# ZYM-PKU/UDiffText

Measured on AMD Instinct MI355X. Metric: 512x512 50-step denoised images/sec (UDiffText hot path: conditioner + 50 CFG Euler steps + VAE decode), higher is better.
Workload: dtype bf16; 1 GPU; 512x512, 50 Euler/DDIM(eta 0) steps, CFG 5.0, 9-char labels, noise_iters 0; global batch 4 per step sharded over 1 GPU(s) = 4 images per GPU in micro-batches of 4: every UNet call runs ONE batch of 4 (8 samples with CFG); 3 such batch(es) in flight per GPU on separate launch streams; BASELINE.json configs[1]; global_batch=4, weights=synthetic (name-keyed recipe), 1361.2 M parameters, launch=hipGraph replay of the sampler steps, in_flight=3, batches_per_unet_call=1

## Files before the change

include/udt_kernels.h:

```cpp
#ifndef UDT_KERNELS_H
#define UDT_KERNELS_H

#include <stddef.h>
#include <stdint.h>

#ifdef __cplusplus
extern "C" {
#endif

typedef enum {
  UDT_OK = 0,
  UDT_ERR_BAD_SHAPE = -1,
  UDT_ERR_BAD_ARG = -2,
  UDT_ERR_WORKSPACE = -3,
  UDT_ERR_HIP = -4,
  UDT_ERR_NO_DEVICE = -5,
  UDT_ERR_ASYNC = -6
} udt_status;

typedef enum {
  UDT_DTYPE_F32 = 0,
  UDT_DTYPE_BF16 = 1,
  UDT_DTYPE_FP8_E4M3 = 2
} udt_dtype;

#define UDT_GEMM_OUT_F32     (1 << 0)
#define UDT_GEMM_GEGLU       (1 << 1)
#define UDT_GEMM_RELU        (1 << 2)
#define UDT_GEMM_TRANSPOSED  (1 << 3)
#define UDT_GEMM_CONV        (1 << 4)
#define UDT_GEMM_SILU_OUT    (1 << 5)
#define UDT_GEMM_MX8         (1 << 7)

typedef struct {
  const void* a;
  const void* a2;
  const void* w;
  const float* bias;
  const void* residual;
  const float* rowvec;
  void* out;
  int32_t M, N, K;
  int32_t lda, ldo, ldr;
  int32_t ldw;
  int32_t batch;
  int64_t stride_a, stride_w, stride_out, stride_res;
  int32_t Hin, Win, C1, C2, Hout, Wout;
  int32_t ksize;
  int32_t stride;
  int32_t pad_t, pad_l;
  int32_t upsample;
  int32_t rows_per_batch;
  int32_t ld_rowvec;
  int32_t flags;
  float alpha;
  const float* colscale;
  const float* in_scsh;
  int32_t in_act;
  float* colstats;
  int32_t cu_share;
  const float* ln_colsum;
  float ln_eps;
  const void* a_scale;
  void* q8_out;
  void* q8_scale;
  int32_t ld_q8;
  int32_t q8_fixed_col;
  float q8_fixed_mul;
  float* rowstat_out;
  const float* rowstat_in;
  int32_t rowstat_in_parts;
} udt_gemm_desc;

size_t udt_gemm_workspace_bytes(const udt_gemm_desc* d);
int udt_gemm(const udt_gemm_desc* d, void* workspace, size_t workspace_bytes, void* stream);
int32_t udt_gemm_colstats_rows(const udt_gemm_desc* d);
int32_t udt_gemm_rowstat_parts(const udt_gemm_desc* d);
int32_t udt_gemm_q8_ok(const udt_gemm_desc* d);
int32_t udt_gemm_colstats_slots(const udt_gemm_desc* d);
int32_t udt_gemm_in_scsh_ok(const udt_gemm_desc* d);
int32_t udt_gemm_up4_ok(const udt_gemm_desc* d);
int udt_gn_silu_conv3x3_fwd(const udt_gemm_desc* d, void* workspace, size_t workspace_bytes, void* stream);
int udt_ln_gemm_fwd(const udt_gemm_desc* d, void* workspace, size_t workspace_bytes, void* stream);
int udt_check_async_error(void* workspace, size_t workspace_bytes, void* stream);

int udt_attn_fwd(const void* q, const void* k, const void* vt, void* o,
                 int32_t batch, int32_t heads, int32_t nq, int32_t nk,
                 int32_t ldq, int32_t ldk, int32_t ldvt, int32_t ldo,
                 int64_t q_bstride, int64_t k_bstride, int64_t vt_bstride, int64_t o_bstride,
                 float scale, void* stream);

int udt_xattn_fwd(const void* q, const void* k, const void* v, void* o, float* probs,
                  int32_t batch, int32_t heads, int32_t head_dim, int32_t nq, int32_t L,
                  int32_t ldq, int32_t ldkv, int32_t ldo, float scale, void* stream);

int udt_attn_rowv_fwd(const void* q, const void* k, const void* v, void* o,
                      int32_t batch, int32_t heads, int32_t nq, int32_t nk,
                      int32_t ldq, int32_t ldk, int32_t ldv, int32_t ldo,
                      int64_t q_bstride, int64_t k_bstride, int64_t v_bstride, int64_t o_bstride,
                      float scale, void* stream);
int udt_attn_rowv_q8_fwd(const void* q, const void* k, const void* v, void* o,
                         int32_t batch, int32_t heads, int32_t nq, int32_t nk,
                         int32_t ldq, int32_t ldk, int32_t ldv, int32_t ldo,
                         int64_t q_bstride, int64_t k_bstride, int64_t v_bstride, int64_t o_bstride,
                         float scale, void* q8_out, void* q8_scale, int32_t ld_q8, void* stream);

int udt_attn_mx8_fwd(const void* qkv8, const void* qkv_scale, void* o, int32_t batch, int32_t heads, int32_t n,
                     int32_t ld8, int32_t ldo, float scale, float v_inv, void* q8_out, void* q8_scale, int32_t ld_q8,
                     void* stream);

int udt_attn512_fwd(const void* q, const void* k, const void* v, void* o,
                    int32_t batch, int32_t nq, int32_t nk,
                    int32_t ldq, int32_t ldk, int32_t ldv, int32_t ldo,
                    int64_t q_bstride, int64_t k_bstride, int64_t v_bstride, int64_t o_bstride,
                    float scale, void* stream);

size_t udt_attn512_workspace_bytes(int32_t batch, int32_t nq, int32_t nk);
int udt_attn512_split_fwd(const void* q, const void* k, const void* v, void* o,
                          int32_t batch, int32_t nq, int32_t nk,
                          int32_t ldq, int32_t ldk, int32_t ldv, int32_t ldo,
                          int64_t q_bstride, int64_t k_bstride, int64_t v_bstride, int64_t o_bstride,
                          float scale, void* workspace, size_t workspace_bytes, void* stream);

int udt_mattn_fwd(const void* q, const void* k, const void* v, void* o, const float* mask, const uint8_t* kpm,
                  int32_t batch, int32_t heads, int32_t head_dim, int32_t nq, int32_t lk,
                  int32_t ldq, int32_t ldk, int32_t ldv, int32_t ldo, int32_t ldmask,
                  int64_t q_bstride, int64_t k_bstride, int64_t v_bstride, int64_t o_bstride, float scale, void* stream);

int32_t udt_tattn_hp(int32_t heads);
int udt_tattn_prepare(const void* kv, int32_t ldkv, const void* wq, int32_t ldwq, const void* wo, int32_t ldwo,
                      const float* gamma, const float* beta, void* A, float* sc, void* BmT, int32_t B, int32_t L,
                      int32_t C, int32_t heads, float scale, void* stream);
int udt_tattn_fused(const void* x, void* out, const void* A, const float* sc, const void* BmT, const float* bias,
                    int32_t B, int32_t n_tok, int32_t C, int32_t heads, int32_t zero_samples, float eps, void* stream);
int32_t udt_tattn_rowstat_parts(int32_t B, int32_t n_tok, int32_t C);
int udt_tattn_fused_q8(const void* x, void* out, const void* A, const float* sc, const void* BmT, const float* bias,
                       int32_t B, int32_t n_tok, int32_t C, int32_t heads, int32_t zero_samples, float eps, void* q8_out,
                       void* q8_scale, float* rowstat_out, void* stream);

int udt_softmax_rows(void* x, int64_t rows, int32_t cols, int32_t ld, void* stream);

int32_t udt_gn_nchunks(int64_t HW, int32_t C);
int udt_gn_stats(const void* x, const void* x2, float* partials, int32_t B, int64_t HW, int32_t C, int32_t C2,
                 int32_t G, void* stream);
int udt_gn_apply(const void* x, const void* x2, void* y, const float* partials, const float* gamma,
                 const float* beta, int32_t B, int64_t HW, int32_t C, int32_t C2, int32_t G, float eps, int32_t act,
                 void* stream);
int32_t udt_gn_strip_ok(int32_t B, int64_t HW, int32_t C1, int32_t C2, int32_t G);
int udt_gn_strip(const void* x, const void* x2, void* y, const float* gamma, const float* beta, int32_t B, int64_t HW,
                 int32_t C1, int32_t C2, int32_t G, float eps, int32_t act, void* stream);

int udt_gn_finalize(const float* stats1, int32_t slots1, int32_t C1, const float* stats2, int32_t slots2, int32_t C2,
                    const float* gamma, const float* beta, float* scsh, int32_t B, int64_t HW, int32_t G, float eps,
                    void* stream);

int udt_gn_apply_scsh(const void* x, const void* x2, void* y, const float* scsh, int32_t B, int64_t HW, int32_t C1,
                      int32_t C2, int32_t act, void* stream);

int udt_gn_strip_stats(const void* x, const void* x2, void* y, const float* stats1, int32_t slots1, const float* stats2,
                       int32_t slots2, const float* gamma, const float* beta, int32_t B, int64_t HW, int32_t C1, int32_t C2,
                       int32_t G, float eps, int32_t act, void* stream);

int udt_layernorm(const void* x, void* y, const float* gamma, const float* beta,
                  int64_t rows, int32_t C, float eps, void* stream);
int udt_unet_input(const float* x, void* xin, int32_t B, int32_t hw, int32_t cpad, float c_in, void* stream);
int udt_unet_input_churn(float* x, const float* noise, void* xin, int32_t B, int32_t hw, int32_t cpad, float c_in, float kn,
                         void* stream);
int udt_cfg_euler_step(float* x, const float* eps, float* denoised_out, int32_t B, int32_t hw, int32_t ld_eps,
                       float c_out, float sigma, float sigma_next, float cfg_scale, void* stream);
typedef struct {
  float kx, kd, ka, kp, kn;
  float c_out, scale;
} udt_sampler_coefs;
int udt_cfg_sampler_step(const float* xin, const float* eps, const float* aux, const float* prev, const float* noise,
                         float* xout, float* denoised_out, int32_t B, int32_t hw, int32_t ld_eps, udt_sampler_coefs k,
                         void* stream);
#define UDT_MULTISTEP_MAX 8
typedef struct {
  float c_out, scale, sigma;
  int32_t n;
  float k[UDT_MULTISTEP_MAX];
  const float* hist[UDT_MULTISTEP_MAX];
} udt_multistep_coefs;
int udt_cfg_multistep_step(const float* xin, const float* eps, float* xout, float* d_out, int32_t B, int32_t hw,
                           int32_t ld_eps, udt_multistep_coefs k, void* stream);
int udt_posterior_sample(const float* moments, const float* noise, float* z, int32_t B, int32_t hw, int32_t ldm,
                         float scale, void* stream);
int udt_nchw_to_nhwc(const float* x, void* y, int32_t B, int32_t C, int64_t HW, int32_t cpad, float scale,
                     void* stream);
int udt_nhwc_to_nchw(const void* x, float* y, int32_t B, int32_t C, int64_t HW, int32_t ld, int32_t src_is_f32,
                     void* stream);
int udt_nhwc_set_channels(const float* src, void* dst, int32_t B, int32_t C, int64_t HW, int32_t cpad, int32_t c0,
                          void* stream);
int udt_embed_tokens(const int32_t* idx, const float* table, const float* pe, void* out, int32_t n_tok, int32_t L,
                     int32_t D, void* stream);
int udt_timestep_embedding(const float* t, void* out, int32_t n, int32_t dim, void* stream);
int udt_mask_downsample(const float* mask, float* out, int32_t B, int32_t H, int32_t W, void* stream);
int udt_local_loss(const float* probs, const float* mask, const float* seg_mask, const float* gkernel9,
                   float* loss_accum, int32_t B, int32_t heads, int32_t size, int32_t L, int32_t seg_l,
                   int32_t Hm, int32_t Wm, void* stream);
int udt_local_loss_tiled(const float* probs, const float* mask, const float* seg_mask, const float* gkernel9,
                         float* loss_accum, int32_t n_samples, int32_t mask_batch, int32_t heads, int32_t size, int32_t L,
                         int32_t seg_l, int32_t Hm, int32_t Wm, void* stream);
int udt_attn_bwd(const void* q, const void* k, const void* v, const void* o, const void* d_o, void* dq, void* dk, void* dv,
                 float* lse_ws, float* dsum_ws, int32_t batch, int32_t heads, int32_t n, int32_t ldq, int32_t ldo, int32_t ldd,
                 float scale, void* stream);
int udt_xattn_bwd(const void* k, const void* v, const float* probs, const float* d_probs, const void* d_o, void* dq, int32_t batch,
                  int32_t heads, int32_t head_dim, int32_t nq, int32_t L, int32_t ldkv, int32_t ldo, int32_t lddq, float scale,
                  void* stream);
int udt_local_loss_bwd(const float* probs, const float* mask, const float* seg_mask, const float* gkernel9, float* d_probs,
                       float* loss_accum, float* scratch , int32_t n_samples,
                       int32_t mask_batch, int32_t heads, int32_t size, int32_t L, int32_t seg_l, int32_t Hm, int32_t Wm, float weight,
                       void* stream);
int udt_local_loss_bwd_hw(const float* probs, const float* mask, const float* seg_mask, const float* gkernel9, float* d_probs,
                          float* loss_accum, float* scratch , int32_t n_samples, int32_t mask_batch,
                          int32_t heads, int32_t h, int32_t w, int32_t L, int32_t seg_l, int32_t Hm, int32_t Wm, float weight,
                          void* stream);
int udt_local_loss_tiled_hw(const float* probs, const float* mask, const float* seg_mask, const float* gkernel9, float* loss_accum,
                            float* scratch , int32_t n_samples, int32_t mask_batch, int32_t heads,
                            int32_t h, int32_t w, int32_t L, int32_t seg_l, int32_t Hm, int32_t Wm, void* stream);
int udt_layernorm_bwd(const void* x, const void* dy, const float* gamma, const void* add, void* dx, int64_t rows, int32_t C, float eps,
                      void* stream);
int udt_gn_bwd(const void* x, const void* dy, const float* gamma, const float* beta, const void* add, void* dx, float* partials, int32_t B,
               int32_t HW, int32_t C, int32_t groups, float eps, int32_t silu, void* stream);
int udt_geglu_fwd(const void* ag, void* out, int64_t rows, int32_t inner, void* stream);
int udt_geglu_bwd(const void* ag, const void* dy, void* dag, int64_t rows, int32_t inner, void* stream);
int udt_sum2x2_bf16(const void* dy, void* dx, int32_t B, int32_t H, int32_t W, int32_t C, void* stream);
int udt_center_tokens(const float* x, void* out, int32_t B, int32_t L, int32_t D, void* stream);
int udt_transpose_bf16(const void* in, void* out, int32_t R, int32_t C, int32_t ld, int32_t Rp, void* stream);
int udt_reduce_rows_f32(const float* in, float* out, int32_t P, int64_t n, int32_t accumulate, void* stream);
int32_t udt_colparts(int64_t rows);
int udt_colsum_bf16(const void* x, float* partials, float* out, int64_t rows, int32_t C, void* stream);
int udt_ln_param_grad(const void* x, const void* dy, float* partials, float* dgamma_dbeta, int64_t rows, int32_t C, float eps, void* stream);
// ... 58 lines not shown
```

udifftext_amd/csrc/common.h:

```cpp
#pragma once
#include <hip/hip_runtime.h>
#include <stdint.h>
#include "../../include/udt_kernels.h"

typedef __attribute__((ext_vector_type(8))) __bf16 bf16x8_t;
typedef __attribute__((ext_vector_type(2))) __bf16 bf16x2_t;
typedef __attribute__((ext_vector_type(2))) float f32x2;
typedef __attribute__((ext_vector_type(4))) float f32x4;
typedef __attribute__((ext_vector_type(16))) float f32x16;
typedef __attribute__((ext_vector_type(2))) uint32_t u32x2;
typedef __attribute__((ext_vector_type(4))) uint32_t u32x4;

#define UDT_DEVINL __device__ __forceinline__

#ifdef UDT_MEASURE
#define UDT_DBG(flags, bit) ((((flags) >> (bit)) & 1) != 0)
#else
#define UDT_DBG(flags, bit) false
#endif

UDT_DEVINL float bf16_bits_to_f32(uint32_t v) { return __uint_as_float(v << 16); }
UDT_DEVINL float bf16_lo(uint32_t packed) { return __uint_as_float(packed << 16); }
UDT_DEVINL float bf16_hi(uint32_t packed) { return __uint_as_float(packed & 0xffff0000u); }

UDT_DEVINL uint32_t pack_bf16x2(float lo, float hi) {
  f32x2 v = {lo, hi};
  bf16x2_t b = __builtin_convertvector(v, bf16x2_t);
  return __builtin_bit_cast(uint32_t, b);
}

UDT_DEVINL float fast_exp2(float x) { return __builtin_amdgcn_exp2f(x); }
UDT_DEVINL float silu_f(float x) {
  return x * __builtin_amdgcn_rcpf(1.0f + __builtin_amdgcn_exp2f(-x * 1.4426950408889634f));
}
UDT_DEVINL float gelu_erf_f(float x) {
  const float z = fabsf(x) * 0.70710678118654752f;
  const float t = __builtin_amdgcn_rcpf(1.0f + 0.3275911f * z);
  float poly = 1.061405429f;
  poly = poly * t - 1.453152027f;
  poly = poly * t + 1.421413741f;
  poly = poly * t - 0.284496736f;
  poly = poly * t + 0.254829592f;
  poly = poly * t;
  const float e = __builtin_amdgcn_exp2f(-z * z * 1.4426950408889634f);
  const float erf_abs = 1.0f - poly * e;
  const float erf = __builtin_copysignf(erf_abs, x);
  return 0.5f * x * (1.0f + erf);
}

constexpr float GEGLU_GS = 0.70710678118654752f * 1.2011224087864498f;
constexpr float GEGLU_XS = 0.5f / GEGLU_GS;
UDT_DEVINL float geglu_scaled(float xs, float gs) {
  const float t = fminf(fabsf(gs), 7.2067347f);
  float P = 5.1346913e-05f;
  P = P * t - 0.001489955f;
  P = P * t + 0.014895574f;
  P = P * t - 0.086436f;
  P = P * t - 0.636406f;
  P = P * t - 1.3553386f;
  P = P * t;
  const float e = __builtin_amdgcn_exp2f(P);
  const float ha = xs * fabsf(gs);
  const float hs = __builtin_fmaf(xs, gs, ha);
  return __builtin_fmaf(-ha, e, hs);
}

UDT_DEVINL void glds16(const void* gsrc, void* lds_wave_base) {
  __builtin_amdgcn_global_load_lds((const __attribute__((address_space(1))) void*)gsrc,
                                   (__attribute__((address_space(3))) void*)lds_wave_base, 16, 0, 0);
}

UDT_DEVINL void store16_sc1(void* p, f32x4 v) {
  asm volatile("global_store_dwordx4 %0, %1, off sc1\n\ts_nop 1" ::"v"(p), "v"(v) : "memory");
}

UDT_DEVINL void wait_vmcnt0() { asm volatile("s_waitcnt vmcnt(0)" ::: "memory"); }

UDT_DEVINL bf16x8_t lds_read_frag(const char* p) { return *reinterpret_cast<const bf16x8_t*>(p); }

UDT_DEVINL f32x16 mfma32(bf16x8_t a, bf16x8_t b, f32x16 c) {
  return __builtin_amdgcn_mfma_f32_32x32x16_bf16(a, b, c, 0, 0, 0);
}

typedef __attribute__((ext_vector_type(8))) int i32x8_t;
UDT_DEVINL i32x8_t lds_read_frag32(const char* p0, const char* p1) {
  const u32x4 a = *reinterpret_cast<const u32x4*>(p0);
  const u32x4 b = *reinterpret_cast<const u32x4*>(p1);
  i32x8_t r = {(int)a[0], (int)a[1], (int)a[2], (int)a[3], (int)b[0], (int)b[1], (int)b[2], (int)b[3]};
  return r;
}

template <int OPSEL>
UDT_DEVINL f32x16 mfma32_mx8(i32x8_t w, i32x8_t x, f32x16 c, int scale) {
  return __builtin_amdgcn_mfma_scale_f32_32x32x64_f8f6f4(w, x, c, 0, 0, 0, 127, OPSEL, scale);
}

UDT_DEVINL uint32_t mx8_scale_byte(float amax) {
  const uint32_t e = (__float_as_uint(amax * 0.57142866f) >> 23) & 0xffu;
  return e > 7u ? e - 7u : 0u;
}
UDT_DEVINL float mx8_inv_scale(uint32_t s) { return __uint_as_float((254u - s) << 23); }
UDT_DEVINL uint32_t mx8_pack4(float a, float b, float c, float d) {
  int r = 0;
  r = __builtin_amdgcn_cvt_pk_fp8_f32(a, b, r, false);
  r = __builtin_amdgcn_cvt_pk_fp8_f32(c, d, r, true);
  return (uint32_t)r;
}
template <int CTRL>
UDT_DEVINL float dpp_max(float v) {
  const int t = __builtin_amdgcn_update_dpp(0, __builtin_bit_cast(int, v), CTRL, 0xF, 0xF, false);
  return fmaxf(v, __builtin_bit_cast(float, t));
}
UDT_DEVINL u32x2 mx8_quant_row8(const float (&o)[8], uint32_t& sbyte) {
  float a = fmaxf(fmaxf(fmaxf(fabsf(o[0]), fabsf(o[1])), fmaxf(fabsf(o[2]), fabsf(o[3]))),
                  fmaxf(fmaxf(fabsf(o[4]), fabsf(o[5])), fmaxf(fabsf(o[6]), fabsf(o[7]))));
  a = dpp_max<0xB1>(a);
  a = dpp_max<0x4E>(a);
  sbyte = mx8_scale_byte(a);
  const float m = mx8_inv_scale(sbyte);
  u32x2 r = {mx8_pack4(o[0] * m, o[1] * m, o[2] * m, o[3] * m), mx8_pack4(o[4] * m, o[5] * m, o[6] * m, o[7] * m)};
  return r;
}
UDT_DEVINL u32x2 e4m3_fixed_row8(const float (&o)[8], float m) {
  float c[8];
#pragma unroll
  for (int j = 0; j < 8; ++j) c[j] = fminf(fmaxf(o[j] * m, -448.f), 448.f);
  u32x2 r = {mx8_pack4(c[0], c[1], c[2], c[3]), mx8_pack4(c[4], c[5], c[6], c[7])};
  return r;
}
UDT_DEVINL void mx8_quant_acc16(const float (&v)[16], uint32_t (&out)[4], uint32_t& sbyte) {
  float a = 0.f;
#pragma unroll
  for (int r = 0; r < 16; ++r) a = fmaxf(a, fabsf(v[r]));
  const auto sw = __builtin_amdgcn_permlane32_swap(__builtin_bit_cast(unsigned, a), __builtin_bit_cast(unsigned, a), false, false);
  a = fmaxf(__builtin_bit_cast(float, (unsigned)sw[0]), __builtin_bit_cast(float, (unsigned)sw[1]));
  sbyte = mx8_scale_byte(a);
  const float m = mx8_inv_scale(sbyte);
#pragma unroll
  for (int q = 0; q < 4; ++q) out[q] = mx8_pack4(v[q * 4] * m, v[q * 4 + 1] * m, v[q * 4 + 2] * m, v[q * 4 + 3] * m);
}

UDT_DEVINL int range_index(int g, int G) {
  if ((G & 7) != 0) return g;
  return (g & 7) * (G >> 3) + (g >> 3);
}

UDT_DEVINL unsigned lds_offset(const void* p) { return (unsigned)(uintptr_t)p; }
UDT_DEVINL u32x2 lds_tr16_b64(unsigned addr, int off) {
  u32x2 r;
  asm volatile("ds_read_b64_tr_b16 %0, %1 offset:%2" : "=v"(r) : "v"(addr), "i"(off) : "memory");
  return r;
}
UDT_DEVINL u32x2 lds_tr8_b64(unsigned addr, int off) {
  u32x2 r;
  asm volatile("ds_read_b64_tr_b8 %0, %1 offset:%2" : "=v"(r) : "v"(addr), "i"(off) : "memory");
  return r;
}
UDT_DEVINL void lds_tr_wait(u32x2& a, u32x2& b) { asm volatile("s_waitcnt lgkmcnt(0)" : "+v"(a), "+v"(b) : : "memory"); }
UDT_DEVINL void lds_tr_wait(u32x2& a, u32x2& b, u32x2& c, u32x2& d) {
  asm volatile("s_waitcnt lgkmcnt(0)" : "+v"(a), "+v"(b), "+v"(c), "+v"(d) : : "memory");
}
UDT_DEVINL float half_swap_max(float v) {
  const auto sw = __builtin_amdgcn_permlane32_swap(__builtin_bit_cast(unsigned, v), __builtin_bit_cast(unsigned, v), false, false);
  return fmaxf(__builtin_bit_cast(float, (unsigned)sw[0]), __builtin_bit_cast(float, (unsigned)sw[1]));
}
UDT_DEVINL float half_swap_sum(float v) {
  const auto sw = __builtin_amdgcn_permlane32_swap(__builtin_bit_cast(unsigned, v), __builtin_bit_cast(unsigned, v), false, false);
  return __builtin_bit_cast(float, (unsigned)sw[0]) + __builtin_bit_cast(float, (unsigned)sw[1]);
}

template <int CTRL>
UDT_DEVINL float dpp_add(float v) {
  const int t = __builtin_amdgcn_update_dpp(0, __builtin_bit_cast(int, v), CTRL, 0xF, 0xF, false);
  return v + __builtin_bit_cast(float, t);
}
UDT_DEVINL float row16_sum(float v) {
  v = dpp_add<0xB1>(v);
  v = dpp_add<0x4E>(v);
  v = dpp_add<0x124>(v);
  v = dpp_add<0x128>(v);
  return v;
}
UDT_DEVINL float xor16_sum(float v) {
  const auto r = __builtin_amdgcn_permlane16_swap(__builtin_bit_cast(unsigned, v), __builtin_bit_cast(unsigned, v), false, false);
  return __builtin_bit_cast(float, (unsigned)r[0]) + __builtin_bit_cast(float, (unsigned)r[1]);
}
// ... 22 lines not shown
```

udifftext_amd/csrc/gemm.hip:

```cpp
#include "common.h"
#include <stdio.h>
#include <stdlib.h>
#include <string.h>
#include <atomic>
#include <cmath>

hipError_t udt_lean_launch_gemm(int cfg, const void* lparams, int smem, int G, int geglu, int ln, hipStream_t s);
hipError_t udt_lean_launch_conv3(const void* c3params, hipStream_t s);

namespace {
#include "tile_common.h"

struct GemmParams {
  const uint16_t* a;
  const uint16_t* a2;
  const uint16_t* w;
  const uint16_t* zero;
  const float* bias;
  const uint16_t* res;
  const float* rowvec;
  void* out;
  const float* colscale;
  const float* in_scsh;
  float* colstats;
// ... 725 lines not shown
  const bool geglu = (d->flags & UDT_GEMM_GEGLU) != 0;
  const bool ln = d->ln_colsum != nullptr;
  if (want_stats && (geglu || ln || !lean_stats_enabled())) return false;
  if (mx8 || emit) {
    if (conv1 || d->rowvec || mode == 0 || (mode > 0 && mode != 1)) return false;
    if (mx8 && (!d->a_scale || d->K % 128 != 0 || d->lda % 16 != 0 || (d->ldw > 0 && d->ldw % 16 != 0))) return false;
    if (mx8 && ln && (!d->rowstat_in || d->rowstat_in_parts <= 0)) return false;
    if (!mx8 && geglu) return false;
    if (mx8 && geglu && !(ln && emit)) return false;
    if (mx8 && !geglu && ln && emit && d->rowstat_out) return false;
    if (emit && (want_stats || !d->q8_scale || d->ld_q8 % 8 != 0 || d->N % (geglu ? 64 : 32) != 0)) return false;
    if (d->rowstat_out && (!emit || geglu)) return false;
    if (d->q8_fixed_col > 0 && (!emit || geglu || d->q8_fixed_col % 32 != 0 || !(d->q8_fixed_mul > 0.f))) return false;
    if ((reinterpret_cast<uintptr_t>(d->q8_out) | reinterpret_cast<uintptr_t>(d->colscale)) & 15) return false;
  } else if (d->rowstat_out || d->rowstat_in) {
    return false;
  }
  const int KT = mx8 ? 128 : BK;
  if (d->N <= 64 || d->N % 8 != 0 || d->K % KT != 0 || (!conv1 && d->lda % 8 != 0) || (d->ldo % 8 != 0 && d->out)) return false;
  if (d->residual && d->ldr % 8 != 0) return false;
  if (geglu && (d->N % 64 != 0 || d->residual || d->rowvec)) return false;
  const long long ldw = d->ldw > 0 ? d->ldw : d->K;
  const long long lda_eff = conv1 ? (d->C1 > d->C2 ? d->C1 : d->C2) : d->lda;
  if ((long long)d->M * lda_eff * 2 >= (1LL << 31) || (long long)d->N * ldw * 2 >= (1LL << 31)) return false;
  if (d->M >= (1 << 28)) return false;
  if ((reinterpret_cast<uintptr_t>(d->out) | reinterpret_cast<uintptr_t>(d->residual) | reinterpret_cast<uintptr_t>(d->bias) |
       reinterpret_cast<uintptr_t>(d->rowvec) | reinterpret_cast<uintptr_t>(d->ln_colsum)) & 15) return false;
  if (d->rowvec && ((d->ld_rowvec > 0 ? d->ld_rowvec : d->N) % 4 != 0)) return false;
  if (mode > 0 && mode != 1 && mode != 6 && mode != 7) return false;
  if (!mx8 && (!emit || (ln && !geglu && !d->rowstat_out)) && (mode == 7 || (mode < 0 && rowres_on()))) {
    const bool emit_fits = !emit || ((d->q8_fixed_col <= 0 || d->q8_fixed_col % 64 == 0) && (long long)d->M * d->ld_q8 < (1LL << 31) &&
                                     (long long)d->M * (d->out ? d->ldo : 0) * 2 < (1LL << 31) && (long long)((d->N + 127) / 128) * d->M * 4 < (1LL << 31));
    if (ln && !want_stats && d->K == 320 && d->N % 64 == 0 && !d->residual && !d->rowvec && !conv1 && emit_fits &&
        (reinterpret_cast<uintptr_t>(d->a) & 15) == 0) {
      const int tiles_m = (d->M + 255) / 256, chunks = d->N / 64;
      int ns = (device_cus() + tiles_m - 1) / tiles_m;
      if (ns > chunks / 4) ns = chunks / 4;
      const int cmax = geglu ? 20 : 16;
      const int ns_min = (chunks + cmax - 1) / cmax;
      if (ns < ns_min) ns = ns_min;
      const long long wgs = (long long)tiles_m * ns;
      if (ns >= 1 && (mode == 7 || emit || (geglu ? wgs * 4 >= 3LL * device_cus() : wgs >= device_cus()))) {
        t.cfg = 7; t.stats_rows = 0; t.nw = 4; t.bm = 256; t.bn = 64; t.smem = 0;
        t.tiles_m = tiles_m; t.kt_per = (chunks + ns - 1) / ns; t.tiles_n = (chunks + t.kt_per - 1) / t.kt_per;
        t.tiles = t.tiles_m * t.tiles_n; t.nkt = d->K / BK; t.splitk = 1; t.n_block = 1;
        t.G = round_workgroups(t.tiles);
        return true;
      }
    }
    if (mode == 7 || (emit && ln)) return false;
  }
  t.cfg = (mode > 0) ? mode : 1;
  if (!mx8 && !emit) {
  if (!geglu && d->N % 160 == 0 && d->N % 128 != 0 && t.cfg == 1) t.cfg = 5;
  if (mode <= 0 && d->N >= 768 && (long long)((d->M + 255) / 256) * ((d->N + 255) / 256) >= 2LL * device_cus() &&
      (d->cu_share <= 1 || lean256_under_lanes())) t.cfg = 6;
  }
  t.stats_rows = 0;
  if (want_stats) {
    if (t.cfg != 1 && t.cfg != 5) {
      if (mode > 0) return false;
      t.cfg = (d->N % 160 == 0 && d->N % 128 != 0) ? 5 : 1;
    }
    if (mx8) t.cfg = 1;
    t.stats_rows = t.cfg == 1 ? 64 : 32;
    const int rpb = d->rows_per_batch > 0 ? d->rows_per_batch : d->M;
    if (rpb % t.stats_rows != 0) return false;
  }
  switch (t.cfg) {
    case 1: t.nw = 4; t.bm = 128; t.bn = 128; t.smem = 2 * (128 + 128) * ROW_BYTES; break;
    case 5: t.nw = 4; t.bm = 128; t.bn = 160; t.smem = 128 * 160 * 4; break;
    case 6: t.nw = 8; t.bm = 256; t.bn = 256; t.smem = 2 * (256 + 256) * ROW_BYTES; break;
    default: return false;
  }
  {
    const int epi = (t.cfg == 6 ? t.bm * t.bn : t.bm * t.bn * 4) + ((ln && t.cfg != 5) ? t.bm * 8 : 0);
    if (t.smem < epi) t.smem = epi;
  }
  t.tiles_m = (d->M + t.bm - 1) / t.bm;
  t.tiles_n = (d->N + t.bn - 1) / t.bn;
  t.tiles = t.tiles_m * t.tiles_n;
  t.nkt = d->K / KT;
  int slots = device_cus() * ((t.cfg == 1 || t.cfg == 5) ? 2 : 1) / share_of(d);
  if (slots < 1) slots = 1;
  int sk = 1;
  const int knob = lean_splitk_knob();
  if (!ln && t.tiles <= 1023) {
    if (knob > 1) sk = knob;
    else if (knob < 0 && t.tiles * 2 <= slots && t.nkt >= (mx8 ? 20 : 40)) { sk = slots / t.tiles; if (sk > t.nkt / (mx8 ? 8 : 16)) sk = t.nkt / (mx8 ? 8 : 16); }
    if (sk > t.nkt / 4) sk = t.nkt / 4;
    while (sk > 1 && (long long)t.tiles * sk * t.bm * t.bn * 4 > (64LL << 20)) --sk;
    if (sk < 1) sk = 1;
  }
  t.kt_per = (t.nkt + sk - 1) / sk;
  t.splitk = (t.nkt + t.kt_per - 1) / t.kt_per;
  const int units = t.tiles * t.splitk;
  t.G = round_workgroups(units);
  int nb = g_n_block.load(std::memory_order_relaxed);
  if (nb <= 0) nb = (t.tiles_m <= 8) ? t.tiles_n : 8;
  if (nb > t.tiles_n) nb = t.tiles_n;
  t.n_block = nb;
  return true;
}

size_t lean_workspace(const LeanPlan& t) {
  return t.splitk > 1 ? G8_HEADER_BYTES + (size_t)t.tiles * t.splitk * t.bm * t.bn * sizeof(float) : 0;
}

std::atomic<int> g_lean_conv{-1};
std::atomic<int> g_wide_conv{-2};
int wide_conv_mode() {
  int v = g_wide_conv.load(std::memory_order_relaxed);
  if (v == -2) {
    const char* e = getenv("UDT_WIDE_CONV");
    v = e ? atoi(e) : -1;
    g_wide_conv.store(v, std::memory_order_relaxed);
  }
  return v;
}
#ifdef UDT_MEASURE
std::atomic<int> g_lconv_dbg{0};
#endif

std::atomic<int> g_wide_lanes_eff{-2};
double wide_lanes_eff() {
  int v = g_wide_lanes_eff.load(std::memory_order_relaxed);
  if (v == -2) {
    const char* e = getenv("UDT_WIDE_LANES_EFF");
    v = e ? atoi(e) : 70;
    g_wide_lanes_eff.store(v, std::memory_order_relaxed);
  }
  return v / 100.0;
}

int conv_chunk_slices(long long tiles, int slots, int chunks, int knob) {
  long long sk = 1;
  if (tiles <= 1023) {
    if (knob > 1) { sk = knob; if (sk > chunks) sk = chunks; }
    else if (knob < 0 && tiles * 2 <= slots && chunks >= 10) { sk = slots / tiles; if (sk > chunks / 4) sk = chunks / 4; }
    if (sk < 1) sk = 1;
  }
  return (int)sk;
}

bool lean_conv_plan(const udt_gemm_desc* d, lg::C3Params& c, bool want_stats) {
  int on = g_lean_conv.load(std::memory_order_relaxed);
  if (on < 0) {
    const char* e = getenv("UDT_LEAN_CONV");
    on = (e && e[0] == '0') ? 0 : 1;
    g_lean_conv.store(on, std::memory_order_relaxed);
  }
  if (!on || lean_mode() == 0) return false;
  if (d->flags != UDT_GEMM_CONV || d->ksize != 3 || d->stride != 1 || d->pad_t != 1 || d->pad_l != 1) return false;
  if (d->C2 != 0 || d->in_scsh || d->colscale || d->batch > 1) return false;
  if (want_stats && !lean_stats_enabled()) return false;
  if (d->N < 128 || d->N % 8 != 0 || d->C1 <= 0 || d->C1 % 64 != 0) return false;
  if (d->upsample != 0 && d->upsample != 1 && d->upsample != 2) return false;
  const bool phase = d->upsample == 2, ups = d->upsample == 1;
  const int nph = phase ? 4 : 1;
  if (d->Hout != (d->Hin << (d->upsample ? 1 : 0)) || d->Wout != (d->Win << (d->upsample ? 1 : 0))) return false;
  if (phase && d->ldw > 0 && d->ldw < 4 * d->C1) return false;
  const int Ht = phase ? d->Hin : d->Hout, Wt = phase ? d->Win : d->Wout;
  c.bn = 128; c.wgm = 2;
  bool wide = false;
  int wide_slots = device_cus();
  {
    const int wm = wide_conv_mode();
    if (wm != 0 && !ups && d->N % 160 == 0 && Wt % 16 == 0 && Ht % 16 == 0) {
      const int cus = device_cus(), share = d->cu_share > 1 ? d->cu_share : 1;
      wide_slots = cus / share > 0 ? cus / share : 1;
      const long long wt = (long long)(d->M / 256) * (d->N / 160);
      const long long sk = conv_chunk_slices(wt, wide_slots, d->C1 / 64, lean_splitk_knob());
      const long long units = wt * sk;
      const long long rounds = (units + cus - 1) / cus;
      const double eff = units > cus ? (double)units / (double)(rounds * cus) : ((double)units * share >= cus ? 1.0 : (double)units * share / cus);
      wide = (wm > 0) || (sk <= 2 && eff >= ((share >= 3 && share_of(d) >= 3) ? wide_lanes_eff() : 0.85));
    }
  }
  if (wide) { c.geo = phase ? 6 : 3; c.tw = 16; c.th = 16; c.bn = 160; c.wgm = 4; }
  else if (Wt % 16 == 0 && Ht % 8 == 0) { c.geo = ups ? 2 : phase ? 4 : 0; c.tw = 16; c.th = 8; }
  else if (!ups && Wt % 8 == 0 && Ht % 8 == 0) { c.geo = phase ? 5 : 1; c.tw = 8; c.th = 8; }
  else return false;
  if (d->ldo % 8 != 0 || (d->residual && d->ldr % 8 != 0)) return false;
  const long long ldw = d->ldw > 0 ? d->ldw : (phase ? 4LL * d->C1 : (long long)d->K);
  if (ldw % 8 != 0) return false;
  c.w_phase = phase ? (d->stride_w > 0 ? d->stride_w : (long long)d->N * ldw) : 0;
  if (phase && (c.w_phase < (long long)d->N * ldw || c.w_phase % 8 != 0)) return false;
  if ((long long)d->M * d->C1 * 2 >= (1LL << 31) || (long long)d->N * ldw * 2 >= (1LL << 31)) return false;
  if ((reinterpret_cast<uintptr_t>(d->out) | reinterpret_cast<uintptr_t>(d->residual) | reinterpret_cast<uintptr_t>(d->bias) |
       reinterpret_cast<uintptr_t>(d->rowvec)) & 15) return false;
  if (d->rowvec && ((d->ld_rowvec > 0 ? d->ld_rowvec : d->N) % 4 != 0)) return false;
  c.dbg = 0;
#ifdef UDT_MEASURE
  c.dbg = g_lconv_dbg.load(std::memory_order_relaxed);
#endif
  c.N = d->N; c.C = d->C1; c.H = d->Hin; c.W = d->Win; c.B = d->M / (d->Hout * d->Wout);
  c.ldw = (int)ldw; c.ldo = d->ldo; c.ldr = d->ldr; c.ldrv = d->ld_rowvec > 0 ? d->ld_rowvec : d->N;
  c.alpha = d->alpha;
  c.tiles_x = Wt / c.tw; c.tiles_y = Ht / c.th;
  c.tiles_m = c.B * c.tiles_x * c.tiles_y;
  c.tiles_n = (d->N + c.bn - 1) / c.bn;
  c.tiles = c.tiles_m * c.tiles_n;
  c.chunks = c.C / 64;
  const int slots = wide ? wide_slots : (2 * device_cus() / share_of(d) > 0 ? 2 * device_cus() / share_of(d) : 1);
  int sk = conv_chunk_slices((long long)c.tiles * nph, slots, c.chunks, lean_splitk_knob());
  while (sk > 1 && (long long)c.tiles * nph * sk * c.tw * c.th * c.bn * 4 > (64LL << 20)) --sk;
  c.ch_per = (c.chunks + sk - 1) / sk;
  c.splitk = (c.chunks + c.ch_per - 1) / c.ch_per;
  c.G = round_workgroups(c.tiles * nph * c.splitk);
  {
    const double patch = (double)((ups ? c.tw / 2 : c.tw) + 2) * ((ups ? c.th / 2 : c.th) + 2) * c.C * 2.0, wtile = (phase ? 4.0 : 9.0) * c.bn * c.C * 2.0;
    int nb = g_n_block.load(std::memory_order_relaxed);
    if (nb <= 0) nb = (int)(std::sqrt(64.0 * patch / wtile) + 0.5);
    if (nb < 1) nb = 1;
    if (nb > c.tiles_n) nb = c.tiles_n;
    c.n_block = nb;
  }
  c.a_bytes = (unsigned)((long long)c.B * d->Hin * d->Win * d->C1 * 2);
  c.w_bytes = (unsigned)((long long)d->N * ldw * 2);
  c.counters = nullptr; c.slabs = nullptr;
  return true;
}

int lean_conv_phases(const lg::C3Params& c) { return c.geo >= 4 ? 4 : 1; }

size_t lean_conv_workspace(const lg::C3Params& c) {
  return c.splitk > 1 ? G8_HEADER_BYTES + (size_t)c.tiles * lean_conv_phases(c) * c.splitk * c.tw * c.th * c.bn * sizeof(float) : 0;
}

bool lean_stats_probe(const udt_gemm_desc* d, int& rows, int& slots) {
  if (d->in_scsh) return false;
  {
    lg::C3Params c3;
    if (lean_conv_plan(d, c3, true)) {
      rows = c3.tw * c3.th / c3.wgm;
      slots = c3.tiles_m * c3.wgm * lean_conv_phases(c3);
      return true;
    }
  }
  if ((d->flags & UDT_GEMM_CONV) && d->ksize == 3) return false;
  LeanPlan lt;
  if (lean_plan(d, lt, true)) {
    rows = lt.stats_rows;
    slots = lt.tiles_m * (lt.bm / lt.stats_rows);
    return true;
  }
  return false;
}
}

extern "C" int udt_debug_set(const char* key, int32_t value) {
  if (!key) return UDT_ERR_BAD_ARG;
  if (!strcmp(key, "n_block")) { g_n_block.store(value); return UDT_OK; }
  if (!strcmp(key, "rows_epi")) { g_rows_epi.store(value ? 1 : 0); return UDT_OK; }
  if (!strcmp(key, "lean")) { g_lean.store(value < 0 ? -2 : value); return UDT_OK; }
  if (!strcmp(key, "rowres")) { g_rowres.store(value < 0 ? 1 : (value ? 1 : 0)); return UDT_OK; }
  if (!strcmp(key, "wide_lanes_eff")) { g_wide_lanes_eff.store(value < 0 ? -2 : value); return UDT_OK; }
  if (!strcmp(key, "conv_n4")) { g_conv_n4.store(value < 0 ? -2 : (value ? 1 : 0)); return UDT_OK; }
  if (!strcmp(key, "lean256_lanes")) { g_lean256_lanes.store(value < 0 ? -2 : (value ? 1 : 0)); return UDT_OK; }
  if (!strcmp(key, "lean_splitk")) { g_lean_splitk.store(value); return UDT_OK; }
  if (!strcmp(key, "share_splitk")) { g_share_splitk.store(value < 0 ? -2 : (value ? 1 : 0)); return UDT_OK; }
  if (!strcmp(key, "lean_conv")) { g_lean_conv.store(value < 0 ? -1 : (value ? 1 : 0)); return UDT_OK; }
  if (!strcmp(key, "wide_conv")) { g_wide_conv.store(value < 0 ? -1 : (value ? 1 : 0)); return UDT_OK; }
#ifdef UDT_MEASURE
  if (!strcmp(key, "lconv_dbg")) { g_lconv_dbg.store(value); return UDT_OK; }
  static const struct { const char* k; int bit; } bits[] = {{"no_xchg", 28}, {"no_epi", 27}, {"no_store", 26}, {"no_res", 25},
                                                            {"no_bias", 24}, {"no_fast", 22}};
  for (const auto& b : bits)
    if (!strcmp(key, b.k)) {
      int cur = g_dbg_bits.load();
      g_dbg_bits.store((cur & ~(1 << b.bit)) | (value ? (1 << b.bit) : 0));
      return UDT_OK;
    }
#endif
  return UDT_ERR_BAD_ARG;
}

extern "C" int udt_check_async_error(void* workspace, size_t workspace_bytes, void* stream) {
  if (!workspace || workspace_bytes < G8_HEADER_BYTES) return UDT_ERR_BAD_ARG;
  hipStream_t s = reinterpret_cast<hipStream_t>(stream);
  int err = 0;
  hipError_t e = hipMemcpyAsync(&err, reinterpret_cast<int*>(workspace) + 1023, sizeof(int), hipMemcpyDeviceToHost, s);
  if (e == hipSuccess) e = hipStreamSynchronize(s);
  if (e != hipSuccess) return udt_set_hip_error(e);
  if (err == 0) return UDT_OK;
  e = hipMemsetAsync(workspace, 0, G8_HEADER_BYTES, s);
  if (e == hipSuccess) e = hipStreamSynchronize(s);
  if (e != hipSuccess) return udt_set_hip_error(e);
  return UDT_ERR_ASYNC;
}

extern "C" int32_t udt_gemm_colstats_rows(const udt_gemm_desc* d) { return d ? colstats_rows(d) : 0; }
extern "C" int32_t udt_gemm_colstats_slots(const udt_gemm_desc* d) { return d ? colstats_slots(d) : 0; }
extern "C" int32_t udt_gemm_q8_ok(const udt_gemm_desc* d) {
  if (!d || !d->q8_out || d->M <= 0 || d->N <= 0 || d->K <= 0) return 0;
  LeanPlan lt;
  return lean_plan(d, lt, d->colstats != nullptr) ? 1 : 0;
}

extern "C" int32_t udt_gemm_rowstat_parts(const udt_gemm_desc* d) {
  if (!d || d->M <= 0 || d->N <= 0 || d->K <= 0) return 0;
  udt_gemm_desc t = *d;
  alignas(16) static const uint64_t probe_dst[2] = {0, 0};
  if (!t.q8_out) { t.q8_out = const_cast<uint64_t*>(probe_dst); t.q8_scale = const_cast<uint64_t*>(probe_dst); if (t.ld_q8 <= 0) t.ld_q8 = (t.N + 15) / 16 * 16; }
  LeanPlan lt;
  if (!lean_plan(&t, lt, false) || lt.cfg != 1 || (d->flags & UDT_GEMM_GEGLU)) return 0;
  return (d->N + 63) / 64;
}
extern "C" int32_t udt_gemm_in_scsh_ok(const udt_gemm_desc* d) {
  if (!d || d->K <= 0 || d->K % BK != 0) return 0;
  c3p::Geo ge;
  return conv3p_geometry(d, ge, true) ? 1 : 0;
}

extern "C" int32_t udt_gemm_up4_ok(const udt_gemm_desc* d) {
  if (!d || d->upsample != 2) return 0;
  lg::C3Params c3;
  return lean_conv_plan(d, c3, d->colstats != nullptr) ? 1 : 0;
}

extern "C" int udt_gn_silu_conv3x3_fwd(const udt_gemm_desc* d, void* workspace, size_t workspace_bytes, void* stream) {
  if (!d || !(d->flags & UDT_GEMM_CONV) || d->ksize != 3 || d->stride != 1 || d->pad_t != 1 || d->pad_l != 1 || !d->in_scsh)
    return UDT_ERR_BAD_ARG;
  return udt_gemm(d, workspace, workspace_bytes, stream);
}

extern "C" int udt_ln_gemm_fwd(const udt_gemm_desc* d, void* workspace, size_t workspace_bytes, void* stream) {
  if (!d || !d->ln_colsum || !d->bias || !(d->ln_eps > 0.f)) return UDT_ERR_BAD_ARG;
  LeanPlan lt;
  if (!lean_plan(d, lt, false)) return UDT_ERR_BAD_SHAPE;
  return udt_gemm(d, workspace, workspace_bytes, stream);
}

extern "C" size_t udt_gemm_workspace_bytes(const udt_gemm_desc* d) {
  if (!d || d->K <= 0 || d->M <= 0 || d->N <= 0 || d->K % k_tile(d) != 0) return 0;
  if (conv_n4_applies(d)) return 0;
  {
    LeanPlan lt;
    if (lean_plan(d, lt, d->colstats != nullptr)) return lean_workspace(lt);
    lg::C3Params c3;
    if (lean_conv_plan(d, c3, d->colstats != nullptr)) return lean_conv_workspace(c3);
  }
  {
    c3p::Geo ge;
    if (conv3p_geometry(d, ge, d->in_scsh != nullptr)) {
      TilePlan t3 = plan_tiles3p(d, ge);
      if (!t3.fixup) return 0;
      return G8_HEADER_BYTES + (size_t)t3.G * t3.bm * t3.bn * sizeof(float);
    }
  }
  if (use_gemm8(d)) {
    TilePlan t8 = plan_tiles8(d);
    if (!t8.fixup) return 0;
    return G8_HEADER_BYTES + (size_t)t8.G * t8.bm * t8.bn * sizeof(float);
  }
  TilePlan t = plan_tiles(d);
  if (t.bm != 256 || !t.fixup) return 0;
  return G8_HEADER_BYTES + (size_t)t.G * 2 * SLAB_FLOATS * sizeof(float);
}

extern "C" int udt_gemm(const udt_gemm_desc* d, void* workspace, size_t workspace_bytes, void* stream) {
  if (!d || !d->a || !d->w) return UDT_ERR_BAD_ARG;
  if (d->M <= 0 || d->N <= 0 || d->K <= 0) return UDT_ERR_BAD_SHAPE;
  if (d->K % k_tile(d) != 0) return UDT_ERR_BAD_SHAPE;
  if (d->N % 4 != 0) return UDT_ERR_BAD_SHAPE;
  const bool mx8 = (d->flags & UDT_GEMM_MX8) != 0;
  if (mx8 || d->q8_out || d->rowstat_out || d->rowstat_in) {
    LeanPlan lt8;
    if (!lean_plan(d, lt8, d->colstats != nullptr)) return UDT_ERR_BAD_ARG;
  } else if (d->colscale) {
    return UDT_ERR_BAD_ARG;
  }
  const bool conv = (d->flags & UDT_GEMM_CONV) != 0;
  const bool trans = (d->flags & UDT_GEMM_TRANSPOSED) != 0;
  const int batch = d->batch > 0 ? d->batch : 1;
  if (conv) {
    if (d->ksize != 1 && d->ksize != 3) return UDT_ERR_BAD_SHAPE;
    if (d->C1 <= 0 || d->C1 % BK != 0 || d->C2 % BK != 0) return UDT_ERR_BAD_SHAPE;
    if (d->C2 > 0 && !d->a2) return UDT_ERR_BAD_ARG;
    if (d->K != d->ksize * d->ksize * (d->C1 + d->C2)) return UDT_ERR_BAD_SHAPE;
    if (d->Hout <= 0 || d->Wout <= 0 || d->M % (d->Hout * d->Wout) != 0) return UDT_ERR_BAD_SHAPE;
    if (d->stride != 1 && d->stride != 2) return UDT_ERR_BAD_SHAPE;
    if (trans || batch != 1) return UDT_ERR_BAD_ARG;
  } else {
    if (d->lda < d->K || d->lda % 8 != 0) return UDT_ERR_BAD_SHAPE;
  }
  if (!d->out && !d->q8_out) return UDT_ERR_BAD_ARG;
  if (trans) {
    if (d->rows_per_batch <= 0 || d->rows_per_batch % 4 != 0 || d->M % d->rows_per_batch != 0)
      return UDT_ERR_BAD_SHAPE;
    if (d->flags & (UDT_GEMM_OUT_F32 | UDT_GEMM_GEGLU | UDT_GEMM_RELU | UDT_GEMM_SILU_OUT)) return UDT_ERR_BAD_ARG;
    if (d->residual || d->rowvec || batch != 1) return UDT_ERR_BAD_ARG;
  } else {
    if (d->ldo % 4 != 0) return UDT_ERR_BAD_SHAPE;
    if (d->residual && d->ldr % 4 != 0) return UDT_ERR_BAD_SHAPE;
  }
  if (d->flags & UDT_GEMM_GEGLU) {
    if (d->N % 64 != 0 || (d->flags & UDT_GEMM_OUT_F32) || d->residual || d->rowvec) return UDT_ERR_BAD_ARG;
  }
  if (d->rowvec && d->rows_per_batch <= 0) return UDT_ERR_BAD_ARG;

  hipStream_t s = reinterpret_cast<hipStream_t>(stream);
  if (conv_n4_applies(d)) {
    cn4::Params cp;
    cp.a = reinterpret_cast<const uint16_t*>(d->a); cp.w = reinterpret_cast<const uint16_t*>(d->w); cp.bias = d->bias;
    cp.out = reinterpret_cast<float*>(d->out);
    cp.B = d->M / (d->Hout * d->Wout); cp.H = d->Hin; cp.W = d->Win; cp.C = d->C1;
    cp.ldw = d->ldw > 0 ? d->ldw : d->K; cp.ldo = d->ldo;
    cp.tiles_x = (d->Win + 7) / 8; cp.tiles_y = (d->Hin + 7) / 8;
    const size_t smem = (size_t)100 * (d->C1 + 8) * 2 + (size_t)4 * 9 * d->C1 * 2;
    static AttrOnce once;
    hipError_t ea = once.ensure(reinterpret_cast<const void*>(cn4::conv3x3_n4_kernel), 100 * (512 + 8) * 2 + 4 * 9 * 512 * 2);
    if (ea != hipSuccess) return udt_set_hip_error(ea);
    UdtProfScope profn(0, s);
    if (profn.rec) {
      char tag[96];
      snprintf(tag, sizeof(tag), "conv_n4 M=%d N=%d K=%d %dx%d", d->M, d->N, d->K, d->Hin, d->Win);
      udt_prof_tag(profn.rec, tag);
    }
    hipLaunchKernelGGL(cn4::conv3x3_n4_kernel, dim3((unsigned)(cp.B * cp.tiles_x * cp.tiles_y)), dim3(256), smem, s, cp);
    UDT_CHECK_LAUNCH();
    return UDT_OK;
  }
  TilePlan t = plan_tiles(d);

  GemmParams p;
  p.a = reinterpret_cast<const uint16_t*>(d->a);
  p.a2 = reinterpret_cast<const uint16_t*>(d->a2);
  p.w = reinterpret_cast<const uint16_t*>(d->w);
  p.zero = udt_zero_page();
  if (!p.zero) return UDT_ERR_HIP;
  p.bias = d->bias;
  p.res = reinterpret_cast<const uint16_t*>(d->residual);
  p.rowvec = d->rowvec;
  p.out = d->out;
  p.colscale = d->colscale;
  p.in_scsh = d->in_scsh;
  p.in_act = d->in_act;
  p.colstats = d->colstats;
  p.slabs = nullptr;
  if (d->colstats && colstats_rows(d) == 0) return UDT_ERR_BAD_ARG;
  if (d->in_scsh && !udt_gemm_in_scsh_ok(d)) return UDT_ERR_BAD_ARG;
  if (d->in_act != 0 && d->in_act != 1) return UDT_ERR_BAD_ARG;
  p.M = d->M; p.N = d->N; p.K = d->K;
  p.lda = d->lda; p.ldo = d->ldo; p.ldr = d->ldr;
  p.ldw = d->ldw > 0 ? d->ldw : d->K;
  if (d->upsample == 2) {
    if (!udt_gemm_up4_ok(d)) return UDT_ERR_BAD_SHAPE;
  } else if (p.ldw < d->K || p.ldw % 8 != 0) return UDT_ERR_BAD_SHAPE;
  if (mx8 && d->lda < d->K) return UDT_ERR_BAD_SHAPE;
  p.sA = d->stride_a; p.sW = d->stride_w; p.sO = d->stride_out; p.sR = d->stride_res;
  p.Hin = d->Hin; p.Win = d->Win; p.C1 = d->C1; p.C2 = d->C2; p.Hout = d->Hout; p.Wout = d->Wout;
  p.ksz = d->ksize; p.stride = d->stride; p.pad_t = d->pad_t; p.pad_l = d->pad_l; p.ups = d->upsample ? 1 : 0;
  p.rows_per_batch = d->rows_per_batch > 0 ? d->rows_per_batch : d->M;
  p.ldrv = d->ld_rowvec > 0 ? d->ld_rowvec : d->N;
  if (d->flags & ~PUBLIC_FLAGS) return UDT_ERR_BAD_ARG;
  p.flags = d->flags | (g_rows_epi.load(std::memory_order_relaxed) ? 0 : INTERNAL_DIRECT_EPI);
#ifdef UDT_MEASURE
  p.flags |= g_dbg_bits.load(std::memory_order_relaxed);
#endif
  p.n_block = 1;
  p.alpha = d->alpha;
  const int cls = (conv && d->ksize == 3) ? 0 : 1;
  {
    LeanPlan lt;
    if (lean_plan(d, lt, d->colstats != nullptr)) {
      lg::LParams lp;
      lp.colstats = d->colstats;
      const bool conv1 = (d->flags & UDT_GEMM_CONV) != 0;
      lp.a = p.a; lp.a2 = (conv1 && d->C2 > 0) ? p.a2 : nullptr; lp.w = p.w; lp.bias = p.bias; lp.res = p.res; lp.rowvec = p.rowvec;
      lp.ln_s = d->ln_colsum;
      lp.out = reinterpret_cast<uint16_t*>(d->out);
      lp.M = d->M; lp.N = d->N; lp.K = d->K;
      lp.lda = conv1 ? d->C1 : p.lda; lp.ldw = p.ldw; lp.ldo = p.ldo; lp.ldr = p.ldr; lp.ldrv = p.ldrv; lp.rows_per_batch = p.rows_per_batch;
      lp.lda2 = conv1 ? d->C2 : 0;
      lp.kt_split = (conv1 && d->C2 > 0) ? d->C1 / BK : lt.nkt;
      lp.a2_bytes = (unsigned)((long long)d->M * (conv1 ? d->C2 : 0) * 2);
      lp.alpha = d->alpha; lp.ln_eps = d->ln_eps;
      lp.tiles_m = lt.tiles_m; lp.tiles_n = lt.tiles_n; lp.n_block = lt.n_block; lp.tiles = lt.tiles;
      lp.nkt = lt.nkt; lp.splitk = lt.splitk; lp.kt_per = lt.kt_per;
      lp.a_bytes = (unsigned)((long long)d->M * lp.lda * elem_bytes(d));
      lp.w_bytes = (unsigned)((long long)d->N * p.ldw * elem_bytes(d));
      lp.a_scale = mx8 ? reinterpret_cast<const uint32_t*>(d->a_scale) : nullptr;
      lp.colscale = d->colscale;
      lp.rowstat_in = d->rowstat_in; lp.rowstat_in_parts = d->rowstat_in_parts;
      lp.q8_out = reinterpret_cast<uint8_t*>(d->q8_out); lp.q8_scale = reinterpret_cast<uint32_t*>(d->q8_scale); lp.ld_q8 = d->ld_q8;
      lp.rowstat_out = d->rowstat_out;
      lp.q8_fixed_col = d->q8_fixed_col > 0 ? d->q8_fixed_col : 0x7fffffff;
      lp.q8_fixed_mul = d->q8_fixed_mul;
      lp.G = lt.G;
      lp.counters = nullptr; lp.slabs = nullptr;
      if (lt.splitk > 1) {
        if (!workspace || workspace_bytes < lean_workspace(lt)) return UDT_ERR_WORKSPACE;
        lp.counters = reinterpret_cast<int*>(workspace);
        lp.slabs = reinterpret_cast<float*>(reinterpret_cast<char*>(workspace) + G8_HEADER_BYTES);
      }
      UdtProfScope profl(cls, s);
      if (profl.rec) {
        char tag[96];
        snprintf(tag, sizeof(tag), "lean%d%s%s M=%d N=%d K=%d fl=0x%x ln=%d tile=%dx%d units=%d splitk=%d", lt.cfg, mx8 ? "-mx8" : "", d->q8_out ? "+q8" : "",
                 d->M, d->N, d->K, d->flags, d->ln_colsum ? 1 : 0, lt.bm, lt.bn, lt.tiles * lt.splitk, lt.splitk);
        udt_prof_tag(profl.rec, tag);
      }
      const bool geglu = (d->flags & UDT_GEMM_GEGLU) != 0, ln = d->ln_colsum != nullptr;
      hipError_t el;
      el = udt_lean_launch_gemm(lt.cfg, &lp, lt.smem, lt.G, geglu ? 1 : 0, ln ? 1 : 0, s);
      if (el != hipSuccess) return udt_set_hip_error(el);
      return UDT_OK;
    }
  }
  if (d->ln_colsum) return UDT_ERR_BAD_ARG;
  {
    lg::C3Params c3;
    if (lean_conv_plan(d, c3, d->colstats != nullptr)) {
      c3.colstats = d->colstats;
      c3.a = p.a; c3.w = p.w; c3.bias = p.bias; c3.res = p.res; c3.rowvec = p.rowvec; c3.out = reinterpret_cast<uint16_t*>(d->out);
      if (c3.splitk > 1) {
        if (!workspace || workspace_bytes < lean_conv_workspace(c3)) return UDT_ERR_WORKSPACE;
        c3.counters = reinterpret_cast<int*>(workspace);
        c3.slabs = reinterpret_cast<float*>(reinterpret_cast<char*>(workspace) + G8_HEADER_BYTES);
      }
      UdtProfScope profc(cls, s);
      if (profc.rec) {
        char tag[96];
        snprintf(tag, sizeof(tag), "%s%s M=%d N=%d K=%d %dx%d tile=%dx%d units=%d splitk=%d nb=%d%s", (c3.geo == 3 || c3.geo == 6) ? "wconv3" : "lconv3",
                 (d->upsample && c3.geo != 6) ? "+up" : "", d->M, d->N, d->K,
                 d->Hin, d->Win, c3.tw, c3.th, c3.tiles * lean_conv_phases(c3) * c3.splitk, c3.splitk, c3.n_block,
                 d->upsample == 2 ? " up4" : "");
        udt_prof_tag(profc.rec, tag);
      }
      const hipError_t ec = udt_lean_launch_conv3(&c3, s);
      if (ec != hipSuccess) return udt_set_hip_error(ec);
      return UDT_OK;
    }
  }
  {
    c3p::CParams cp;
    if (conv3p_geometry(d, cp.geo, d->in_scsh != nullptr)) {
      const TilePlan t3 = plan_tiles3p(d, cp.geo);
      p.tiles_m = t3.tiles_m; p.tiles_n = t3.tiles_n; p.tiles_per_batch = t3.tiles_m * t3.tiles_n;
      {
        const double patch = (double)cp.geo.prows_img * cp.geo.NI * cp.geo.C * 2.0;
        const double wtile = 9.0 * t3.bn * cp.geo.C * 2.0;
        const double S = (double)(t3.tiles < t3.G ? t3.tiles : t3.G) / 8.0;
        int nb = (int)(std::sqrt((S < 1.0 ? 1.0 : S) * patch / wtile) + 0.5);
        if (nb < 1) nb = 1;
        if (nb > t3.tiles_n) nb = t3.tiles_n;
        p.n_block = nb;
      }
      p.n_ktiles = t3.nkt;
      p.total_iters = t3.total;
      p.iters_per_wg = t3.ipw;
      p.G = t3.G;
      const long long in_px = (long long)cp.geo.B * d->Hin * d->Win;
      cp.base.a_bytes = (unsigned)(in_px * d->C1 * 2);
      cp.a2_bytes = (unsigned)((long long)d->M * d->C2 * 2);
      cp.scsh_bytes = (unsigned)((long long)cp.geo.B * cp.geo.chunks * 512);
      cp.base.w_bytes = (unsigned)((long long)d->N * p.ldw * 2);
      cp.base.g = p;
      cp.base.flags = nullptr; cp.base.err = nullptr; cp.base.slab_base = nullptr;
      if (t3.fixup) {
        const size_t need = G8_HEADER_BYTES + (size_t)t3.G * t3.bm * t3.bn * sizeof(float);
        if (!workspace || workspace_bytes < need) return UDT_ERR_WORKSPACE;
        cp.base.flags = reinterpret_cast<int*>(workspace);
        cp.base.err = cp.base.flags + 1023;
        cp.base.slab_base = reinterpret_cast<float*>(reinterpret_cast<char*>(workspace) + G8_HEADER_BYTES);
      }
      UdtProfScope prof3(cls, s);
      if (prof3.rec) {
        char tag[96];
        snprintf(tag, sizeof(tag), "conv3p%s%s M=%d N=%d K=%d %dx%d tile=%dx%dx%d bn=%d G=%d ipw=%d", d->in_scsh ? "+gn" : "", d->upsample ? "+up" : "", d->M,
                 d->N, d->K, d->Hin, d->Win, cp.geo.TW, cp.geo.TH, cp.geo.NI, t3.bn, t3.G, t3.ipw);
        udt_prof_tag(prof3.rec, tag);
      }
      hipError_t e3;
      const bool st3 = d->colstats != nullptr;
      if (t3.bn == 160) e3 = st3 ? launch3p<8, 1, 1, 5, true, true>(cp, t3, s) : launch3p<8, 1, 1, 5, true, false>(cp, t3, s);
      else e3 = st3 ? launch3p<4, 2, 2, 2, true, true>(cp, t3, s) : launch3p<4, 2, 2, 2, true, false>(cp, t3, s);
      if (e3 != hipSuccess) return udt_set_hip_error(e3);
      return UDT_OK;
    }
  }
  if (use_gemm8(d)) {
    const TilePlan t8 = plan_tiles8(d);
    p.tiles_m = t8.tiles_m; p.tiles_n = t8.tiles_n; p.tiles_per_batch = t8.tiles_m * t8.tiles_n;
    const int n_block_knob = g_n_block.load(std::memory_order_relaxed);
    if (n_block_knob != 0 && !conv) {
      const long long wt = (long long)t8.bn * d->K * elem_bytes(d);
      long long nb = 1;
      if (n_block_knob > 0) nb = n_block_knob;
      else if (t8.tiles_m <= 8 || trans) nb = t8.tiles_n;
      else if (t8.tiles_n >= 8) nb = (4LL << 20) / (wt > 0 ? wt : 1);
      if (nb < 1) nb = 1;
      if (nb > t8.tiles_n) nb = t8.tiles_n;
      p.n_block = (int)nb;
    }
    p.n_ktiles = t8.nkt;
    p.total_iters = t8.total;
    p.iters_per_wg = t8.ipw;
    p.G = t8.G;
    g8::Params pp;
    pp.g = p;
    pp.flags = nullptr; pp.err = nullptr; pp.slab_base = nullptr;
    pp.a_bytes = conv ? 0u : (unsigned)((long long)d->M * d->lda * elem_bytes(d));
    pp.w_bytes = (unsigned)((long long)d->N * p.ldw * elem_bytes(d));
    if (t8.fixup) {
      const size_t need = G8_HEADER_BYTES + (size_t)t8.G * t8.bm * t8.bn * sizeof(float);
      if (!workspace || workspace_bytes < need) return UDT_ERR_WORKSPACE;
      pp.flags = reinterpret_cast<int*>(workspace);
      pp.err = pp.flags + 1023;
      pp.slab_base = reinterpret_cast<float*>(reinterpret_cast<char*>(workspace) + G8_HEADER_BYTES);
    }
    UdtProfScope prof8(cls, s);
    if (prof8.rec) {
      char tag[96];
      snprintf(tag, sizeof(tag), "gemm8 M=%d N=%d K=%d conv=%d ks=%d fl=0x%x tile=%dx%d G=%d ipw=%d b=%d",
               d->M, d->N, d->K, conv ? 1 : 0, d->ksize, d->flags, t8.bm, t8.bn, t8.G, t8.ipw, batch);
      udt_prof_tag(prof8.rec, tag);
    }
    hipError_t e8;
    const bool st = d->colstats != nullptr;
    if (t8.bn == 160) {
      if (st) e8 = conv ? launch8<8, 1, 1, 5, true, false, true>(pp, t8, s) : launch8<8, 1, 1, 5, false, false, true>(pp, t8, s);
      else e8 = conv ? launch8<8, 1, 1, 5, true, false>(pp, t8, s) : launch8<8, 1, 1, 5, false, false>(pp, t8, s);
    } else if (trans) {
      e8 = launch8<4, 2, 2, 2, false, true>(pp, t8, s);
    } else if (st) {
      e8 = conv ? launch8<4, 2, 2, 2, true, false, true>(pp, t8, s) : launch8<4, 2, 2, 2, false, false, true>(pp, t8, s);
    } else {
      e8 = conv ? launch8<4, 2, 2, 2, true, false>(pp, t8, s) : launch8<4, 2, 2, 2, false, false>(pp, t8, s);
    }
    if (e8 != hipSuccess) return udt_set_hip_error(e8);
    return UDT_OK;
  }

  p.tiles_m = t.tiles_m; p.tiles_n = t.tiles_n; p.tiles_per_batch = t.tiles_m * t.tiles_n;
  p.n_ktiles = t.nkt;
  p.total_iters = t.total;
  p.iters_per_wg = t.ipw;
  p.G = t.G;

  if (t.fixup) {
    const size_t need = G8_HEADER_BYTES + (size_t)t.G * 2 * SLAB_FLOATS * sizeof(float);
    if (!workspace || workspace_bytes < need) return UDT_ERR_WORKSPACE;
    p.slabs = reinterpret_cast<float*>(reinterpret_cast<char*>(workspace) + G8_HEADER_BYTES);
  }

  UdtProfScope prof(cls, s);
  if (prof.rec) {
    char tag[96];
    snprintf(tag, sizeof(tag), "gemm M=%d N=%d K=%d conv=%d ks=%d fl=0x%x tile=%dx%d G=%d ipw=%d b=%d", d->M, d->N, d->K,
             conv ? 1 : 0, d->ksize, d->flags, t.bm, t.bn, t.G, t.ipw, batch);
    udt_prof_tag(prof.rec, tag);
  }

  if (t.bm != 256) return UDT_ERR_BAD_SHAPE;
  const hipError_t e = conv ? launch_cfg<256, 64, 4, 1, true, false>(p, t, s) : launch_cfg<256, 64, 4, 1, false, false>(p, t, s);
  if (e != hipSuccess) return udt_set_hip_error(e);
  return UDT_OK;
}
```

udifftext_amd/csrc/lean.hip:

```cpp
#include "common.h"
#include <stdio.h>
#include <stdlib.h>
#include <atomic>

namespace {
#include "tile_common.h"
#include "lean_params.h"
#include "lean.h"
#include "wide.h"
#include "rowres.h"

template <int NW, int WGM, int WGN, int TM, int TN, int NST, int TMB = TM>
hipError_t launch_lean(const lg::LParams& lp, int smem, int G, bool geglu, bool ln, hipStream_t s) {
  static AttrOnce once[5];
  const void* fn;
  const bool stats = lp.colstats != nullptr;
  if constexpr (NW == 4 && NST == 2) {
    if (stats) {
      fn = (const void*)lg::lgemm_kernel<NW, WGM, WGN, TM, TN, NST, false, false, TMB, true>;
      hipError_t e = once[4].ensure(fn, smem);
      if (e != hipSuccess) return e;
      void* args[] = {const_cast<lg::LParams*>(&lp)};
      return hipLaunchKernel(fn, dim3(G), dim3(NW * 64), args, smem, s);
    }
  }
  if (stats) return hipErrorInvalidValue;
  if constexpr (TN == 2) {
    fn = geglu ? (ln ? (const void*)lg::lgemm_kernel<NW, WGM, WGN, TM, TN, NST, true, true, TMB> : (const void*)lg::lgemm_kernel<NW, WGM, WGN, TM, TN, NST, true, false, TMB>)
               : (ln ? (const void*)lg::lgemm_kernel<NW, WGM, WGN, TM, TN, NST, false, true, TMB> : (const void*)lg::lgemm_kernel<NW, WGM, WGN, TM, TN, NST, false, false, TMB>);
  } else {
    fn = ln ? (const void*)lg::lgemm_kernel<NW, WGM, WGN, TM, TN, NST, false, true, TMB> : (const void*)lg::lgemm_kernel<NW, WGM, WGN, TM, TN, NST, false, false, TMB>;
  }
  hipError_t e = once[(geglu ? 2 : 0) + (ln ? 1 : 0)].ensure(fn, smem);
  if (e != hipSuccess) return e;
  void* args[] = {const_cast<lg::LParams*>(&lp)};
  return hipLaunchKernel(fn, dim3(G), dim3(NW * 64), args, smem, s);
}

template <bool GEGLU, bool LN, bool STATS, bool FP8, bool EMIT>
hipError_t launch_lean_mx8_k(const lg::LParams& lp, int smem, int G, hipStream_t s) {
  static AttrOnce once;
  const void* fn = (const void*)lg::lgemm_kernel<4, 2, 2, 2, 2, 2, GEGLU, LN, 2, STATS, FP8, EMIT>;
  hipError_t e = once.ensure(fn, smem);
  if (e != hipSuccess) return e;
  void* args[] = {const_cast<lg::LParams*>(&lp)};
  return hipLaunchKernel(fn, dim3(G), dim3(256), args, smem, s);
}
hipError_t launch_lean_mx8(const lg::LParams& lp, int smem, int G, bool geglu, bool ln, bool fp8, bool emit, hipStream_t s) {
  const bool stats = lp.colstats != nullptr;
  if (!fp8) {
    if (emit && !geglu && !ln && !stats) return launch_lean_mx8_k<false, false, false, false, true>(lp, smem, G, s);
    return hipErrorInvalidValue;
  }
  if (geglu) return (ln && emit && !stats) ? launch_lean_mx8_k<true, true, false, true, true>(lp, smem, G, s) : hipErrorInvalidValue;
  if (ln) return stats ? hipErrorInvalidValue
                 : emit ? launch_lean_mx8_k<false, true, false, true, true>(lp, smem, G, s)
                        : launch_lean_mx8_k<false, true, false, true, false>(lp, smem, G, s);
  if (stats) return emit ? hipErrorInvalidValue : launch_lean_mx8_k<false, false, true, true, false>(lp, smem, G, s);
  return emit ? launch_lean_mx8_k<false, false, false, true, true>(lp, smem, G, s) : launch_lean_mx8_k<false, false, false, true, false>(lp, smem, G, s);
}

template <int TW, int TH, bool UPS, bool STATS, bool PHASE>
hipError_t launch_lconv3s(const lg::C3Params& c3, hipStream_t s) {
  static AttrOnce once;
  constexpr int smem = lg::C3Geo<TW, TH, UPS>::SMEM;
  hipError_t e = once.ensure(reinterpret_cast<const void*>(lg::lconv3_kernel<TW, TH, UPS, STATS, PHASE>), smem);
  if (e != hipSuccess) return e;
  hipLaunchKernelGGL((lg::lconv3_kernel<TW, TH, UPS, STATS, PHASE>), dim3(c3.G), dim3(256), smem, s, c3);
  return hipGetLastError();
}
template <int TW, int TH, bool UPS, bool PHASE = false>
hipError_t launch_lconv3(const lg::C3Params& c3, hipStream_t s) {
  return c3.colstats ? launch_lconv3s<TW, TH, UPS, true, PHASE>(c3, s) : launch_lconv3s<TW, TH, UPS, false, PHASE>(c3, s);
}

template <bool STATS, bool PHASE>
hipError_t launch_wconv3s(const lg::C3Params& c3, hipStream_t s) {
  static AttrOnce once;
  constexpr int smem = wd::WGeo::SMEM;
  hipError_t e = once.ensure(reinterpret_cast<const void*>(wd::wconv3_kernel<STATS, PHASE>), smem);
  if (e != hipSuccess) return e;
  hipLaunchKernelGGL((wd::wconv3_kernel<STATS, PHASE>), dim3(c3.G), dim3(256), smem, s, c3);
  return hipGetLastError();
}
template <int KT, bool GEGLU, bool EMIT = false>
hipError_t launch_rowres(const lg::LParams& lp, int G, hipStream_t s) {
  static AttrOnce once;
  constexpr int smem = rr::RGeo<KT, GEGLU>::SMEM;
  hipError_t e = once.ensure(reinterpret_cast<const void*>(rr::rgemm_kernel<KT, GEGLU, EMIT>), smem);
  if (e != hipSuccess) return e;
  hipLaunchKernelGGL((rr::rgemm_kernel<KT, GEGLU, EMIT>), dim3(G), dim3(256), smem, s, lp);
  return hipGetLastError();
}

template <bool PHASE>
hipError_t launch_wconv3(const lg::C3Params& c3, hipStream_t s) {
  return c3.colstats ? launch_wconv3s<true, PHASE>(c3, s) : launch_wconv3s<false, PHASE>(c3, s);
}

}

hipError_t udt_lean_launch_gemm(int cfg, const void* lparams, int smem, int G, int geglu, int ln, hipStream_t s) {
  const lg::LParams& lp = *static_cast<const lg::LParams*>(lparams);
  const bool fp8 = lp.a_scale != nullptr, emit = lp.q8_out != nullptr;
  if (cfg == 7 && emit && !fp8 && !geglu && ln && lp.K == 320) return launch_rowres<5, false, true>(lp, G, s);
  if (fp8 || emit) return cfg == 1 ? launch_lean_mx8(lp, smem, G, geglu != 0, ln != 0, fp8, emit, s) : hipErrorInvalidValue;
  switch (cfg) {
    case 1: return launch_lean<4, 2, 2, 2, 2, 2>(lp, smem, G, geglu != 0, ln != 0, s);
    case 6: return launch_lean<8, 2, 4, 4, 2, 2, 1>(lp, smem, G, geglu != 0, ln != 0, s);
    case 5: return geglu ? hipErrorInvalidValue : launch_lean<4, 4, 1, 1, 5, 2>(lp, smem, G, false, ln != 0, s);
    case 7:
      if (!ln || lp.K != 320) return hipErrorInvalidValue;
      return geglu ? launch_rowres<5, true>(lp, G, s) : launch_rowres<5, false>(lp, G, s);
    default: return hipErrorInvalidValue;
  }
}

hipError_t udt_lean_launch_conv3(const void* c3params, hipStream_t s) {
  const lg::C3Params& c3 = *static_cast<const lg::C3Params*>(c3params);
  return c3.geo == 3 ? launch_wconv3<false>(c3, s) : c3.geo == 6 ? launch_wconv3<true>(c3, s) : c3.geo == 2 ? launch_lconv3<16, 8, true>(c3, s)
         : c3.geo == 4 ? launch_lconv3<16, 8, false, true>(c3, s) : c3.geo == 5 ? launch_lconv3<8, 8, false, true>(c3, s)
         : c3.geo == 1 ? launch_lconv3<8, 8, false>(c3, s) : launch_lconv3<16, 8, false>(c3, s);
}
```

udifftext_amd/csrc/lean_params.h:

```cpp
#pragma once

namespace lg {

struct LParams {
  const uint16_t* a;
  const uint16_t* a2;
  const uint16_t* w;
  const float* bias;
  const uint16_t* res;
  const float* rowvec;
  const float* ln_s;
  uint16_t* out;
  int M, N, K;
  int lda, ldw, ldo, ldr, ldrv, rows_per_batch;
  float alpha, ln_eps;
  int tiles_m, tiles_n, n_block, tiles;
  int nkt;
  int splitk, kt_per;
  unsigned a_bytes, w_bytes;
  int kt_split, lda2;
  unsigned a2_bytes;
  int G;
  int* counters;
  float* slabs;
  float* colstats;
  const uint32_t* a_scale;
  const float* colscale;
  const float* rowstat_in;
  int rowstat_in_parts;
  uint8_t* q8_out;
  uint32_t* q8_scale;
  int ld_q8;
  int q8_fixed_col;
  float q8_fixed_mul;
  float* rowstat_out;
};

struct C3Params {
  const uint16_t* a;
  const uint16_t* w;
  const float* bias;
  const uint16_t* res;
  const float* rowvec;
  uint16_t* out;
  int N, C;
  int B, H, W;
  int ldw, ldo, ldr, ldrv;
  float alpha;
  int tiles_x, tiles_y, tiles_m, tiles_n, n_block, tiles;
  int chunks, splitk, ch_per;
  unsigned a_bytes, w_bytes;
  int G;
  int* counters;
  float* slabs;
  float* colstats;
  int geo, tw, th;
  int bn, wgm;
  long long w_phase;
  int dbg;
};

}
```

udifftext_amd/csrc/norm.hip:

```cpp
#include "common.h"
#include <stdio.h>
#include <stdlib.h>

namespace {

constexpr int GN_MAX_C = 4096;

__global__ void __launch_bounds__(256) gn_stats_kernel(const uint16_t* __restrict__ x, const uint16_t* __restrict__ x2,
                                                       float* __restrict__ partials, long long HW, int C1, int C2,
                                                       int G, int nchunks) {
  const int C = C1 + C2;
  extern __shared__ __attribute__((aligned(16))) float gsm[];
  const int t = threadIdx.x;
  const int c8 = C >> 3;
  const int chunk = blockIdx.x;
  const int b = blockIdx.y;
  const long long rows_per_chunk = (HW + nchunks - 1) / nchunks;
  const long long p0 = chunk * rows_per_chunk;
  long long p1 = p0 + rows_per_chunk;
  if (p1 > HW) p1 = HW;

  int R, rg, cc0, cstep;
  if (c8 <= 256) {
    R = 256 / c8;
    rg = t / c8;
    cc0 = t - rg * c8;
    cstep = c8;
    if (rg >= R) cc0 = c8;
  } else {
    R = 1; rg = 0; cc0 = t; cstep = 256;
  }
  float* ssum = gsm;
  float* ssq = gsm + R * C;
  for (int cc = cc0; cc < c8; cc += cstep) {
    float s[8], q[8];
#pragma unroll
    for (int j = 0; j < 8; ++j) s[j] = q[j] = 0.f;
    const bool second = cc * 8 >= C1;
    const int cs = second ? C2 : C1;
    const uint16_t* xb = (second ? x2 : x) + (long long)b * HW * cs + (second ? cc * 8 - C1 : cc * 8);
    auto acc8 = [&](const u32x4 v) {
#pragma unroll
      for (int j = 0; j < 4; ++j) {
        const float a = bf16_lo(v[j]), bb = bf16_hi(v[j]);
        s[2 * j] += a; q[2 * j] += a * a;
        s[2 * j + 1] += bb; q[2 * j + 1] += bb * bb;
      }
    };
    long long pix = p0 + rg;
    for (; pix + 3LL * R < p1; pix += 4LL * R) {
      const u32x4 v0 = *reinterpret_cast<const u32x4*>(xb + pix * cs);
      const u32x4 v1 = *reinterpret_cast<const u32x4*>(xb + (pix + R) * cs);
      const u32x4 v2 = *reinterpret_cast<const u32x4*>(xb + (pix + 2LL * R) * cs);
      const u32x4 v3 = *reinterpret_cast<const u32x4*>(xb + (pix + 3LL * R) * cs);
      acc8(v0); acc8(v1); acc8(v2); acc8(v3);
    }
    for (; pix < p1; pix += R) acc8(*reinterpret_cast<const u32x4*>(xb + pix * cs));
#pragma unroll
    for (int j = 0; j < 8; ++j) {
      ssum[rg * C + cc * 8 + j] = s[j];
      ssq[rg * C + cc * 8 + j] = q[j];
    }
  }
  __syncthreads();
  if (t < G) {
    const int cpg = C / G;
    float a = 0.f, q = 0.f;
    for (int r = 0; r < R; ++r)
      for (int c = t * cpg; c < (t + 1) * cpg; ++c) {
        a += ssum[r * C + c];
        q += ssq[r * C + c];
      }
    float* dst = partials + (((long long)b * nchunks + chunk) * G + t) * 2;
    dst[0] = a;
    dst[1] = q;
  }
}

__global__ void __launch_bounds__(256) gn_apply_kernel(const uint16_t* __restrict__ x, const uint16_t* __restrict__ x2,
                                                       uint16_t* __restrict__ y, const float* __restrict__ partials,
                                                       const float* __restrict__ gamma,
                                                       const float* __restrict__ beta, long long HW, int C1, int C2,
                                                       int G, int nchunks, float eps, int act,
                                                       long long chunks_per_wg, const float* __restrict__ scsh) {
  const int C = C1 + C2;
  extern __shared__ __attribute__((aligned(16))) float asm_[];
  float* sc = asm_;
  float* sh = asm_ + C;
  float* gm = asm_ + 2 * C;
  float* gr = gm + G;
  const int t = threadIdx.x;
  const int b = blockIdx.y;
  const int cpg = C / G;
  const int c8 = C >> 3;
  const long long total = HW * c8;
  const long long begin = (long long)blockIdx.x * chunks_per_wg;
  long long end = begin + chunks_per_wg;
  if (end > total) end = total;
  const uint16_t* xb1 = x + (long long)b * HW * C1;
  const uint16_t* xb2 = x2 ? (x2 + (long long)b * HW * C2) : nullptr;
  uint16_t* yb = y + (long long)b * HW * C;
  auto src_of = [&](long long i, int& cc) -> const uint16_t* {
    const long long pix = i / c8;
    cc = (int)(i - pix * c8);
    return (cc * 8 < C1) ? (xb1 + pix * C1 + cc * 8) : (xb2 + pix * C2 + (cc * 8 - C1));
  };
  long long i = begin + t;
  u32x4 v0 = {0u, 0u, 0u, 0u}, v1 = v0, v2 = v0, v3 = v0;
  int c0 = 0, c1 = 0, c2 = 0, c3 = 0;
  const bool full = i + 768 < end;
  if (full) {
    v0 = *reinterpret_cast<const u32x4*>(src_of(i, c0));
    v1 = *reinterpret_cast<const u32x4*>(src_of(i + 256, c1));
    v2 = *reinterpret_cast<const u32x4*>(src_of(i + 512, c2));
    v3 = *reinterpret_cast<const u32x4*>(src_of(i + 768, c3));
  }
  if (scsh) {
    for (int c = t; c < C; c += 256) {
      const float* src = scsh + (((long long)b * (C >> 6) + (c >> 6)) * 2) * 64 + (c & 63);
      sc[c] = src[0];
      sh[c] = src[64];
    }
  } else {
    double* red = reinterpret_cast<double*>(gr + G);
    const int lanes = 256 / G;
    const int g = t % G, ln = t / G;
    double a = 0.0, q = 0.0;
    if (ln < lanes)
      for (int k = ln; k < nchunks; k += lanes) {
        const float* src = partials + (((long long)b * nchunks + k) * G + g) * 2;
        a += (double)src[0];
        q += (double)src[1];
      }
    red[t] = a;
    red[256 + t] = q;
    __syncthreads();
    if (t < G) {
      a = 0.0; q = 0.0;
      for (int l = 0; l < lanes; ++l) { a += red[l * G + t]; q += red[256 + l * G + t]; }
      const double n = (double)HW * (double)cpg;
      const double mean = a / n;
      double var = q / n - mean * mean;
      if (var < 0.0) var = 0.0;
      gm[t] = (float)mean;
      gr[t] = (float)(1.0 / sqrt(var + (double)eps));
    }
    __syncthreads();
    for (int c = t; c < C; c += 256) {
      const int g = c / cpg;
      const float a = gr[g] * gamma[c];
      sc[c] = a;
      sh[c] = beta[c] - gm[g] * a;
    }
  }
  __syncthreads();
  auto norm8 = [&](const u32x4 v, int cc) {
    u32x4 o;
#pragma unroll
    for (int j = 0; j < 4; ++j) {
      const int c = cc * 8 + 2 * j;
      float a = bf16_lo(v[j]) * sc[c] + sh[c];
      float bb = bf16_hi(v[j]) * sc[c + 1] + sh[c + 1];
      if (act == 1) {
        a = silu_f(a);
        bb = silu_f(bb);
      }
      o[j] = pack_bf16x2(a, bb);
    }
    return o;
  };
  if (full) {
    *reinterpret_cast<u32x4*>(yb + i * 8) = norm8(v0, c0);
    *reinterpret_cast<u32x4*>(yb + (i + 256) * 8) = norm8(v1, c1);
    *reinterpret_cast<u32x4*>(yb + (i + 512) * 8) = norm8(v2, c2);
    *reinterpret_cast<u32x4*>(yb + (i + 768) * 8) = norm8(v3, c3);
    i += 1024;
  }
  for (; i + 768 < end; i += 1024) {
    v0 = *reinterpret_cast<const u32x4*>(src_of(i, c0));
    v1 = *reinterpret_cast<const u32x4*>(src_of(i + 256, c1));
    v2 = *reinterpret_cast<const u32x4*>(src_of(i + 512, c2));
    v3 = *reinterpret_cast<const u32x4*>(src_of(i + 768, c3));
    *reinterpret_cast<u32x4*>(yb + i * 8) = norm8(v0, c0);
    *reinterpret_cast<u32x4*>(yb + (i + 256) * 8) = norm8(v1, c1);
    *reinterpret_cast<u32x4*>(yb + (i + 512) * 8) = norm8(v2, c2);
    *reinterpret_cast<u32x4*>(yb + (i + 768) * 8) = norm8(v3, c3);
  }
  for (; i < end; i += 256) {
    int cc;
    const u32x4 v = *reinterpret_cast<const u32x4*>(src_of(i, cc));
    *reinterpret_cast<u32x4*>(yb + i * 8) = norm8(v, cc);
  }
}

template <int NCH>
__global__ void __launch_bounds__(256) layernorm_kernel(const uint16_t* __restrict__ x, uint16_t* __restrict__ y,
                                                        const float* __restrict__ gamma,
                                                        const float* __restrict__ beta, long long rows, int C,
                                                        float eps) {
  const int lane = threadIdx.x & 63;
  const long long row = (long long)blockIdx.x * 4 + (threadIdx.x >> 6);
  if (row >= rows) return;
  const int c8 = C >> 3;
  const uint16_t* xr = x + row * C;
  float v[NCH][8];
  float s = 0.f;
#pragma unroll
  for (int i = 0; i < NCH; ++i) {
    const int ch = lane + i * 64;
    if (ch < c8) {
      const u32x4 u = *reinterpret_cast<const u32x4*>(xr + ch * 8);
#pragma unroll
      for (int j = 0; j < 4; ++j) {
        v[i][2 * j] = bf16_lo(u[j]);
        v[i][2 * j + 1] = bf16_hi(u[j]);
      }
    } else {
#pragma unroll
      for (int j = 0; j < 8; ++j) v[i][j] = 0.f;
    }
#pragma unroll
    for (int j = 0; j < 8; ++j) s += v[i][j];
  }
#pragma unroll
  for (int off = 32; off > 0; off >>= 1) s += __shfl_xor(s, off);
  const float mean = s / (float)C;
  float q = 0.f;
#pragma unroll
  for (int i = 0; i < NCH; ++i) {
    const int ch = lane + i * 64;
    if (ch < c8) {
#pragma unroll
      for (int j = 0; j < 8; ++j) {
        const float d = v[i][j] - mean;
        q += d * d;
      }
    }
  }
#pragma unroll
  for (int off = 32; off > 0; off >>= 1) q += __shfl_xor(q, off);
  const float rstd = rsqrtf(q / (float)C + eps);
  uint16_t* yr = y + row * C;
#pragma unroll
  for (int i = 0; i < NCH; ++i) {
    const int ch = lane + i * 64;
    if (ch < c8) {
      const f32x4 g0 = *reinterpret_cast<const f32x4*>(gamma + ch * 8);
      const f32x4 g1 = *reinterpret_cast<const f32x4*>(gamma + ch * 8 + 4);
      const f32x4 b0 = *reinterpret_cast<const f32x4*>(beta + ch * 8);
      const f32x4 b1 = *reinterpret_cast<const f32x4*>(beta + ch * 8 + 4);
      float o[8];
#pragma unroll
      for (int j = 0; j < 4; ++j) {
        o[j] = (v[i][j] - mean) * rstd * g0[j] + b0[j];
        o[4 + j] = (v[i][4 + j] - mean) * rstd * g1[j] + b1[j];
      }
      u32x4 pk = {pack_bf16x2(o[0], o[1]), pack_bf16x2(o[2], o[3]), pack_bf16x2(o[4], o[5]),
                  pack_bf16x2(o[6], o[7])};
      *reinterpret_cast<u32x4*>(yr + ch * 8) = pk;
    }
  }
}


constexpr int GNS_THREADS = 512;

__global__ void __launch_bounds__(GNS_THREADS) gn_strip_kernel(const uint16_t* __restrict__ x, const uint16_t* __restrict__ x2,
                                                               uint16_t* __restrict__ y, const float* __restrict__ gamma,
                                                               const float* __restrict__ beta, long long HW, int C1, int C2, int G,
                                                               int gw, float eps, int act, const float* __restrict__ st1,
                                                               int slots1, const float* __restrict__ st2, int slots2) {
  extern __shared__ __attribute__((aligned(16))) float gss[];
  const int C = C1 + C2;
  const int cpg = C / G;
  const int cw = gw * cpg;
  const int nch = cw >> 3;
  const int pstep = GNS_THREADS / nch;
  float* psum = gss;
  float* psq = gss + pstep * cw;
  float* scl = psq + pstep * cw;
  float* shf = scl + cw;
  double* csum = reinterpret_cast<double*>(shf + cw + (cw & 1));
  double* csq = csum + cw;
  const int t = threadIdx.x;
  const int b = blockIdx.y;
  const int c_base = blockIdx.x * cw;
  const int j = t % nch, pl = t / nch;
  const bool active = pl < pstep;
  const int c = c_base + 8 * j;
  const bool second = c >= C1;
  const int cs = second ? C2 : C1;
  const uint16_t* src = (second ? x2 : x) + (long long)b * HW * cs + (second ? c - C1 : c);
  if (st1) {
    if (t < cw) {
      const int cc = c_base + t;
      const bool sec = cc >= C1;
      const float* sp = sec ? st2 + ((long long)b * slots2 * C2 + (cc - C1)) * 2 : st1 + ((long long)b * slots1 * C1 + cc) * 2;
      const int n = sec ? slots2 : slots1;
      const long long stride = (long long)(sec ? C2 : C1) * 2;
      double a = 0.0, qq = 0.0;
      for (int k = 0; k < n; ++k) {
        const f32x2 v = *reinterpret_cast<const f32x2*>(sp + k * stride);
        a += (double)v[0];
        qq += (double)v[1];
      }
      csum[t] = a;
      csq[t] = qq;
    }
  }
  float s[8], q[8];
#pragma unroll
  for (int i = 0; i < 8; ++i) s[i] = q[i] = 0.f;
  auto acc8 = [&](const u32x4 v) {
#pragma unroll
    for (int i = 0; i < 4; ++i) {
      const float a = bf16_lo(v[i]), bb = bf16_hi(v[i]);
      s[2 * i] += a; q[2 * i] += a * a;
      s[2 * i + 1] += bb; q[2 * i + 1] += bb * bb;
    }
  };
  if (active && !st1) {
    long long p = pl;
    for (; p + 3LL * pstep < HW; p += 4LL * pstep) {
// ... 321 lines not shown
```

udifftext_amd/csrc/wide.h:

```cpp
#pragma once
#include <type_traits>

namespace wd {

using g8::buf_lds16;
using g8::OOB;
using g8::wait_vm;
using lg::C3Params;
using lg::raw_barrier;
using lg::wait_vm_upto;
using lg::wave_colstats;

struct WGeo {
  static constexpr int TW = 16, TH = 16, NW = 4;
  static constexpr int TM = 2, TN = 5, BN = TN * 32;
  static constexpr int PW = TW + 2, PH = TH + 2, PROWS = PW * PH;
  static constexpr int PIECES = (PROWS + 7) / 8;
  static constexpr int PATCH_BYTES = PIECES * 1024;
  static constexpr int W_BYTES = BN * ROW_BYTES;
  static constexpr int NRING = 3;
  static constexpr int RING = NRING * W_BYTES + 2 * PATCH_BYTES;
  static constexpr int EROW = BN * 4;
  static constexpr int STAGING = NW * 32 * EROW;
  static constexpr int SMEM = RING > STAGING ? RING : STAGING;
  static_assert(SMEM <= 160 * 1024, "one workgroup per CU");
};

template <bool STATS, bool PHASE = false>
__global__ void __launch_bounds__(256, 1) wconv3_kernel(const C3Params p) {
  using G = WGeo;
  constexpr int NT = PHASE ? 4 : 9;
  constexpr int NW = G::NW, TM = G::TM, TN = G::TN, BN = G::BN, PW = G::PW, NR = G::NRING;
  constexpr int WP = (BN / 8) / NW;
  constexpr int PP = (G::PIECES + NW - 1) / NW;
  constexpr int EROW = G::EROW;
  static_assert((BN / 8) % NW == 0, "weight pieces split evenly over the waves");
  extern __shared__ __attribute__((aligned(16))) char smem[];
  char* const wring = smem;
  char* const patches = smem + NR * G::W_BYTES;

  const int tid = threadIdx.x;
  const int wave = __builtin_amdgcn_readfirstlane(tid >> 6);
  const int lane = tid & 63;
  const int l31 = lane & 31;
  const int hi = lane >> 5;
  const int l3 = lane >> 3;
  const int pslot = lane & 7;
  const int row0 = wave * (TM * 32);
  const int swz_w = (l31 >> 1) & 7;
  const int w_frag_row = l31 * ROW_BYTES;

  const int unit = range_index(blockIdx.x, p.G);
  if (unit >= p.tiles * p.splitk * (PHASE ? 4 : 1)) return;
  const int phase = PHASE ? unit / (p.tiles * p.splitk) : 0;
  const int pha = phase >> 1, phb = phase & 1;
  const int ptile = unit / p.splitk;
  const int slice = unit - ptile * p.splitk;
  const int tile = ptile - phase * p.tiles;
  int tile_m, n0;
  {
    const int per_block = p.tiles_m * p.n_block;
    const int blk = tile / per_block;
    const int r = tile - blk * per_block;
    int nbw = p.tiles_n - blk * p.n_block;
    if (nbw > p.n_block) nbw = p.n_block;
    tile_m = r / nbw;
    n0 = (blk * p.n_block + (r - tile_m * nbw)) * BN;
  }
  const int per_img = p.tiles_x * p.tiles_y;
  const int b = tile_m / per_img;
  const int rt = tile_m - b * per_img;
  const int ty = rt / p.tiles_x;
  const int y0 = ty * G::TH, x0 = (rt - ty * p.tiles_x) * G::TW;
  const int c0 = slice * p.ch_per;
  int c1 = c0 + p.ch_per;
  if (c1 > p.chunks) c1 = p.chunks;

  const __amdgpu_buffer_rsrc_t rsrc_a = __builtin_amdgcn_make_buffer_rsrc(const_cast<uint16_t*>(p.a), 0, p.a_bytes, 0x00020000);
  const __amdgpu_buffer_rsrc_t rsrc_w =
      __builtin_amdgcn_make_buffer_rsrc(const_cast<uint16_t*>(p.w) + (PHASE ? (long long)phase * p.w_phase : 0LL), 0, p.w_bytes, 0x00020000);
  auto patch_swz = [](int prow, int yy) { return ((prow - 2 * yy) >> 1) & 7; };
  unsigned w_voff[WP], p_voff[PP];
  int p_piece[PP];
#pragma unroll
  for (int i = 0; i < WP; ++i) {
    const int row = (wave + NW * i) * 8 + l3;
    const int kw = (pslot ^ ((row >> 1) & 7)) * 8;
    const int n = n0 + row;
    w_voff[i] = (n < p.N) ? (unsigned)(((long long)n * p.ldw + kw) * 2) : OOB;
  }
#pragma unroll
  for (int i = 0; i < PP; ++i) {
    int idx = wave + NW * i;
    while (idx >= G::PIECES) idx -= NW;
    p_piece[i] = idx;
    const int prow = idx * 8 + l3;
    const int yy = prow / PW;
    const int xx = prow - yy * PW;
    const int gy = y0 + yy - 1, gx = x0 + xx - 1;
    const bool ok = (prow < G::PROWS) && ((unsigned)gy < (unsigned)p.H) && ((unsigned)gx < (unsigned)p.W);
    const int koff = (pslot ^ patch_swz(prow, yy)) * 8;
    p_voff[i] = ok ? (unsigned)(((((long long)b * p.H + gy) * p.W + gx) * p.C + koff) * 2) : OOB;
  }
  int a_prow[TM], a_py[TM];
#pragma unroll
  for (int tm = 0; tm < TM; ++tm) {
    const int ml = row0 + tm * 32 + l31;
    const int py = ml / G::TW, px = ml - py * G::TW;
    a_py[tm] = PHASE ? py + pha : py;
    a_prow[tm] = PHASE ? (py + pha) * PW + px + phb : py * PW + px;
  }
  auto issue_w = [&](int st, int c, int tap) {
    const int soff = (tap * p.C + c * 64) * 2;
    char* wbuf = wring + st * G::W_BYTES;
#pragma unroll
    for (int i = 0; i < WP; ++i) buf_lds16(rsrc_w, wbuf + (wave + NW * i) * 1024, w_voff[i], soff);
  };
  auto issue_patch = [&](int buf, int c) {
    char* pbuf = patches + buf * G::PATCH_BYTES;
#pragma unroll
    for (int i = 0; i < PP; ++i) buf_lds16(rsrc_a, pbuf + p_piece[i] * 1024, p_voff[i], c * 128);
  };

  f32x16 acc[TM][TN];
#pragma unroll
  for (int i = 0; i < TM; ++i)
#pragma unroll
    for (int j = 0; j < TN; ++j)
#pragma unroll
      for (int r = 0; r < 16; ++r) acc[i][j][r] = 0.f;

  constexpr int PPT = PHASE ? 6 : 2, PTAPS = (PP + PPT - 1) / PPT;
  static_assert(PTAPS <= NT - 2, "the next patch is complete two taps before its chunk starts");
  static_assert(NR - 1 < NT, "the ring's prologue stays inside the first chunk");
  auto issue_patch_part = [&](int buf, int c, int part) {
    char* pbuf = patches + buf * G::PATCH_BYTES;
#pragma unroll
    for (int j = 0; j < PPT; ++j) {
      const int i = part * PPT + j;
      if (i < PP) buf_lds16(rsrc_a, pbuf + p_piece[i] * 1024, p_voff[i], c * 128);
    }
  };
  issue_patch(c0 & 1, c0);
#pragma unroll
  for (int j = 0; j < NR - 1; ++j) issue_w(j, c0, j);
  int st = 0;
  for (int c = c0; c < c1; ++c) {
    const int cn = (c + 1 < c1) ? c + 1 : c;
    const char* pbuf = patches + (c & 1) * G::PATCH_BYTES;
    auto tap_body = [&](auto tap_c) {
      constexpr int tap = decltype(tap_c)::value;
      constexpr auto pcount = [](int t) { const int tt = (t + NT) % NT; return tt < PTAPS ? ((tt + 1) * PPT <= PP ? PPT : PP - tt * PPT) : 0; };
      wait_vm<pcount(tap - 2) + WP + pcount(tap - 1)>();
      raw_barrier();
      const int dy = PHASE ? tap >> 1 : tap / 3, dx = PHASE ? tap & 1 : tap - dy * 3;
      const char* wbuf = wring + st * G::W_BYTES;
      int arow[TM], aswz[TM];
#pragma unroll
      for (int t = 0; t < TM; ++t) {
        const int prow = a_prow[t] + dy * PW + dx;
        arow[t] = prow * ROW_BYTES;
        aswz[t] = patch_swz(prow, a_py[t] + dy);
      }
      bf16x8_t fx[2][TM], fw[2][TN];
      auto read_ks = [&](int ks, int slot2) {
        if (UDT_DBG(p.dbg, 3)) return;
#pragma unroll
        for (int t = 0; t < TM; ++t) fx[slot2][t] = lds_read_frag(pbuf + arow[t] + (((ks * 2 + hi) ^ aswz[t]) << 4));
        const int slot = ((ks * 2 + hi) ^ swz_w) << 4;
#pragma unroll
        for (int t = 0; t < TN; ++t) fw[slot2][t] = lds_read_frag(wbuf + w_frag_row + t * 32 * ROW_BYTES + slot);
      };
      read_ks(0, 0);
#pragma unroll
      for (int ks = 0; ks < 4; ++ks) {
        if (ks + 1 < 4) read_ks(ks + 1, (ks + 1) & 1);
        if (ks == 3) {
          const int ahead = tap + NR - 1;
          int s2 = st + NR - 1;
          if (s2 >= NR) s2 -= NR;
          if (!UDT_DBG(p.dbg, 0)) {
            if (ahead < NT) issue_w(s2, c, ahead);
            else issue_w(s2, cn, ahead - NT);
          }
          if constexpr (tap < PTAPS) {
            if (!UDT_DBG(p.dbg, 1)) issue_patch_part((c + 1) & 1, cn, tap);
          }
        }
        if (UDT_DBG(p.dbg, 2)) {
#pragma unroll
          for (int tm = 0; tm < TM; ++tm) asm volatile("" ::"v"(fx[ks & 1][tm]));
#pragma unroll
          for (int tn = 0; tn < TN; ++tn) asm volatile("" ::"v"(fw[ks & 1][tn]));
        } else {
#pragma unroll
          for (int tm = 0; tm < TM; ++tm)
#pragma unroll
            for (int tn = 0; tn < TN; ++tn) acc[tm][tn] = mfma32(fw[ks & 1][tn], fx[ks & 1][tm], acc[tm][tn]);
        }
      }
      __builtin_amdgcn_sched_group_barrier(0x100, TM + TN, 0);
#pragma unroll
      for (int ks = 0; ks < 3; ++ks) {
#pragma unroll
        for (int i = 0; i < TM + TN; ++i) {
          __builtin_amdgcn_sched_group_barrier(0x008, 1, 0);
          __builtin_amdgcn_sched_group_barrier(0x100, 1, 0);
        }
        __builtin_amdgcn_sched_group_barrier(0x008, TM * TN - (TM + TN), 0);
      }
      constexpr int NV = WP + pcount(tap), NVI = NV < TM * TN ? NV : TM * TN;
#pragma unroll
      for (int i = 0; i < NVI; ++i) {
        __builtin_amdgcn_sched_group_barrier(0x008, 1, 0);
        __builtin_amdgcn_sched_group_barrier(0x020, 1, 0);
      }
      if constexpr (NV > NVI) __builtin_amdgcn_sched_group_barrier(0x020, NV - NVI, 0);
      else __builtin_amdgcn_sched_group_barrier(0x008, TM * TN - NV, 0);
      st = (st + 1 == NR) ? 0 : st + 1;
    };
    tap_body(std::integral_constant<int, 0>{}); tap_body(std::integral_constant<int, 1>{}); tap_body(std::integral_constant<int, 2>{});
    tap_body(std::integral_constant<int, 3>{});
    if constexpr (!PHASE) {
      tap_body(std::integral_constant<int, 4>{}); tap_body(std::integral_constant<int, 5>{});
      tap_body(std::integral_constant<int, 6>{}); tap_body(std::integral_constant<int, 7>{}); tap_body(std::integral_constant<int, 8>{});
    }
  }
  constexpr int CPR = TN * 4;
  constexpr int RPI = 64 / CPR;
  constexpr int NIT = (32 + RPI - 1) / RPI;
  const int rl = lane / CPR;
  const int c8 = lane - rl * CPR;
  const int n = n0 + c8 * 8;
  const bool col_ok = (rl < RPI) && (n < p.N);
  long long mrow[TM][NIT];
  bool rok[TM][NIT];
  u32x4 rv[TM][NIT];
#pragma unroll
  for (int tm = 0; tm < TM; ++tm)
#pragma unroll
    for (int i = 0; i < NIT; ++i) {
      const int row = i * RPI + rl;
      rok[tm][i] = col_ok && row < 32;
      const int ml = row0 + tm * 32 + (row < 32 ? row : 0);
      const int py = ml / G::TW, px = ml - py * G::TW;
      mrow[tm][i] = PHASE ? ((long long)b * (2 * p.H) + (2 * (y0 + py) + pha)) * (2 * p.W) + (2 * (x0 + px) + phb)
                          : ((long long)b * p.H + (y0 + py)) * p.W + (x0 + px);
      u32x4 z = {0u, 0u, 0u, 0u};
      rv[tm][i] = z;
      if (p.res && rok[tm][i]) rv[tm][i] = *reinterpret_cast<const u32x4*>(p.res + mrow[tm][i] * p.ldr + n);
    }
  wait_vm<0>();
  raw_barrier();

  if (p.splitk > 1) {
    f32x4* slab = reinterpret_cast<f32x4*>(p.slabs + (long long)unit * (G::TW * G::TH * BN));
#pragma unroll
    for (int tm = 0; tm < TM; ++tm)
#pragma unroll
      for (int tn = 0; tn < TN; ++tn)
#pragma unroll
        for (int q = 0; q < 4; ++q) {
          f32x4 v = {acc[tm][tn][q * 4 + 0], acc[tm][tn][q * 4 + 1], acc[tm][tn][q * 4 + 2], acc[tm][tn][q * 4 + 3]};
          store16_sc1(slab + ((tm * TN + tn) * 4 + q) * 256 + tid, v);
        }
    asm volatile("s_waitcnt vmcnt(0)" ::: "memory");
    __syncthreads();
    int* const bcast = reinterpret_cast<int*>(smem);
    if (tid == 0) {
      const int t = __hip_atomic_fetch_add(p.counters + ptile, 1, __ATOMIC_RELAXED, __HIP_MEMORY_SCOPE_AGENT);
      const int last = (t == p.splitk - 1) ? 1 : 0;
      if (last) {
        __builtin_amdgcn_fence(__ATOMIC_ACQUIRE, "agent");
        __hip_atomic_store(p.counters + ptile, 0, __ATOMIC_RELAXED, __HIP_MEMORY_SCOPE_AGENT);
      }
      *bcast = last;
    }
    __syncthreads();
    const bool last = *bcast != 0;
    __syncthreads();
    if (!last) return;
#pragma unroll
    for (int i = 0; i < TM; ++i)
#pragma unroll
      for (int j = 0; j < TN; ++j)
#pragma unroll
        for (int r = 0; r < 16; ++r) acc[i][j][r] = 0.f;
    for (int s = 0; s < p.splitk; ++s) {
      const f32x4* sl = reinterpret_cast<const f32x4*>(p.slabs + ((long long)ptile * p.splitk + s) * (G::TW * G::TH * BN));
#pragma unroll
      for (int tm = 0; tm < TM; ++tm)
#pragma unroll
        for (int tn = 0; tn < TN; ++tn)
#pragma unroll
          for (int q = 0; q < 4; ++q) {
            const f32x4 v = sl[((tm * TN + tn) * 4 + q) * 256 + tid];
#pragma unroll
            for (int r = 0; r < 4; ++r) acc[tm][tn][q * 4 + r] += v[r];
          }
    }
  }

  char* const wl = smem + wave * (32 * EROW);
  f32x4 b0 = {0.f, 0.f, 0.f, 0.f}, b1 = b0;
  if (col_ok) {
    if (p.bias) {
      b0 = *reinterpret_cast<const f32x4*>(p.bias + n);
      b1 = *reinterpret_cast<const f32x4*>(p.bias + n + 4);
    }
    if (p.rowvec) {
      const float* rvp = p.rowvec + (long long)b * p.ldrv + n;
      const f32x4 r0 = *reinterpret_cast<const f32x4*>(rvp), r1 = *reinterpret_cast<const f32x4*>(rvp + 4);
#pragma unroll
      for (int j = 0; j < 4; ++j) b0[j] += r0[j], b1[j] += r1[j];
    }
  }
  float cs[8], cq[8];
#pragma unroll
  for (int j = 0; j < 8; ++j) cs[j] = cq[j] = 0.f;
#pragma unroll
  for (int tm = 0; tm < TM; ++tm) {
    {
      const int row = l31;
#pragma unroll
      for (int tn = 0; tn < TN; ++tn)
#pragma unroll
        for (int q = 0; q < 4; ++q) {
          const int chunk = (tn * 8 + q * 2 + hi) ^ (row & 7);
          f32x4 v = {acc[tm][tn][q * 4 + 0], acc[tm][tn][q * 4 + 1], acc[tm][tn][q * 4 + 2], acc[tm][tn][q * 4 + 3]};
          *reinterpret_cast<f32x4*>(wl + row * EROW + chunk * 16) = v;
        }
    }
#pragma unroll
    for (int i = 0; i < NIT; ++i) {
      const int row = i * RPI + rl;
      const int rr = row < 32 ? row : 0;
      const char* rp = wl + rr * EROW;
      const int sw = rr & 7;
      const f32x4 v0 = *reinterpret_cast<const f32x4*>(rp + (((2 * c8) ^ sw) << 4));
      const f32x4 v1 = *reinterpret_cast<const f32x4*>(rp + (((2 * c8 + 1) ^ sw) << 4));
      float o[8];
#pragma unroll
      for (int j = 0; j < 4; ++j) {
        o[j] = v0[j] * p.alpha + b0[j];
        o[4 + j] = v1[j] * p.alpha + b1[j];
      }
      if (p.res) {
#pragma unroll
        for (int j = 0; j < 4; ++j) {
          o[2 * j] += bf16_lo(rv[tm][i][j]);
          o[2 * j + 1] += bf16_hi(rv[tm][i][j]);
        }
      }
      if (rok[tm][i]) {
        u32x4 pk = {pack_bf16x2(o[0], o[1]), pack_bf16x2(o[2], o[3]), pack_bf16x2(o[4], o[5]), pack_bf16x2(o[6], o[7])};
        *reinterpret_cast<u32x4*>(p.out + mrow[tm][i] * p.ldo + n) = pk;
        if constexpr (STATS) {
#pragma unroll
          for (int j = 0; j < 4; ++j) {
            const float a = bf16_lo(pk[j]), bb = bf16_hi(pk[j]);
            cs[2 * j] += a; cq[2 * j] += a * a;
            cs[2 * j + 1] += bb; cq[2 * j + 1] += bb * bb;
          }
        }
// ... 11 lines not shown
```

udifftext_amd/lib.py:

```python
from __future__ import annotations

import ctypes as C
import os

_HERE = os.path.dirname(os.path.abspath(__file__))
LIB_PATH = os.path.join(_HERE, "libudt_kernels.so")

GEMM_OUT_F32 = 1 << 0
DTYPE_F32, DTYPE_BF16, DTYPE_FP8_E4M3 = 0, 1, 2
GEMM_GEGLU = 1 << 1
GEMM_RELU = 1 << 2
GEMM_TRANSPOSED = 1 << 3
GEMM_CONV = 1 << 4
GEMM_SILU_OUT = 1 << 5
GEMM_MX8 = 1 << 7

PROF_CONV3X3, PROF_GEMM, PROF_ATTN, PROF_XATTN, PROF_NORM, PROF_ELEMENTWISE = range(6)


class GemmDesc(C.Structure):
    _fields_ = [
        ("a", C.c_void_p), ("a2", C.c_void_p), ("w", C.c_void_p), ("bias", C.c_void_p),
        ("residual", C.c_void_p), ("rowvec", C.c_void_p), ("out", C.c_void_p),
        ("M", C.c_int32), ("N", C.c_int32), ("K", C.c_int32),
        ("lda", C.c_int32), ("ldo", C.c_int32), ("ldr", C.c_int32), ("ldw", C.c_int32),
        ("batch", C.c_int32),
        ("stride_a", C.c_int64), ("stride_w", C.c_int64), ("stride_out", C.c_int64), ("stride_res", C.c_int64),
        ("Hin", C.c_int32), ("Win", C.c_int32), ("C1", C.c_int32), ("C2", C.c_int32),
        ("Hout", C.c_int32), ("Wout", C.c_int32),
        ("ksize", C.c_int32), ("stride", C.c_int32), ("pad_t", C.c_int32), ("pad_l", C.c_int32),
        ("upsample", C.c_int32), ("rows_per_batch", C.c_int32), ("ld_rowvec", C.c_int32), ("flags", C.c_int32),
        ("alpha", C.c_float), ("colscale", C.c_void_p), ("in_scsh", C.c_void_p), ("in_act", C.c_int32), ("colstats", C.c_void_p),
        ("cu_share", C.c_int32), ("ln_colsum", C.c_void_p), ("ln_eps", C.c_float),
        ("a_scale", C.c_void_p), ("q8_out", C.c_void_p), ("q8_scale", C.c_void_p), ("ld_q8", C.c_int32),
        ("q8_fixed_col", C.c_int32), ("q8_fixed_mul", C.c_float),
        ("rowstat_out", C.c_void_p), ("rowstat_in", C.c_void_p), ("rowstat_in_parts", C.c_int32),
    ]


class SamplerCoefs(C.Structure):
    _fields_ = [("kx", C.c_float), ("kd", C.c_float), ("ka", C.c_float), ("kp", C.c_float), ("kn", C.c_float),
                ("c_out", C.c_float), ("scale", C.c_float)]


MULTISTEP_MAX = 8


class MultistepCoefs(C.Structure):
    _fields_ = [("c_out", C.c_float), ("scale", C.c_float), ("sigma", C.c_float), ("n", C.c_int32),
                ("k", C.c_float * MULTISTEP_MAX), ("hist", C.c_void_p * MULTISTEP_MAX)]


_vp, _i32, _i64, _f32, _fp = C.c_void_p, C.c_int32, C.c_int64, C.c_float, C.c_void_p
SYMBOLS = {
    "udt_gemm_workspace_bytes": (C.c_size_t, [C.POINTER(GemmDesc)]),
    "udt_gemm": (C.c_int, [C.POINTER(GemmDesc), _vp, C.c_size_t, _vp]),
    "udt_gemm_fwd": (C.c_int, [C.POINTER(GemmDesc), _vp, C.c_size_t, _vp]),
    "udt_conv1x1_fwd": (C.c_int, [C.POINTER(GemmDesc), _vp, C.c_size_t, _vp]),
    "udt_workspace_bytes": (C.c_size_t, [C.POINTER(GemmDesc)]),
    "udt_pack_linear": (C.c_int, [_fp, _fp, _i32, _i32, _i32, _i32, C.POINTER(_vp), _vp]),
    "udt_pack_conv": (C.c_int, [_fp, _fp, _i32, _i32, _i32, _i32, C.POINTER(_i32), _i32, _i32, C.POINTER(_vp), _vp]),
    "udt_packed_weight": (_vp, [_vp]),
    "udt_packed_bias": (_vp, [_vp]),
    "udt_packed_colscale": (_vp, [_vp]),
    "udt_packed_dim": (_i32, [_vp, _i32]),
    "udt_free_packed": (C.c_int, [_vp]),
    "udt_check_async_error": (C.c_int, [_vp, C.c_size_t, _vp]),
    "udt_gemm_colstats_rows": (_i32, [C.POINTER(GemmDesc)]),
    "udt_gemm_colstats_slots": (_i32, [C.POINTER(GemmDesc)]),
    "udt_gemm_rowstat_parts": (_i32, [C.POINTER(GemmDesc)]),
    "udt_gemm_q8_ok": (_i32, [C.POINTER(GemmDesc)]),
    "udt_gemm_in_scsh_ok": (_i32, [C.POINTER(GemmDesc)]),
    "udt_gemm_up4_ok": (_i32, [C.POINTER(GemmDesc)]),
    "udt_gn_silu_conv3x3_fwd": (C.c_int, [C.POINTER(GemmDesc), _vp, C.c_size_t, _vp]),
    "udt_ln_gemm_fwd": (C.c_int, [C.POINTER(GemmDesc), _vp, C.c_size_t, _vp]),
    "udt_gn_finalize": (C.c_int, [_fp, _i32, _i32, _fp, _i32, _i32, _fp, _fp, _fp, _i32, _i64, _i32, _f32, _vp]),
    "udt_gn_apply_scsh": (C.c_int, [_vp, _vp, _vp, _fp, _i32, _i64, _i32, _i32, _i32, _vp]),
    "udt_gn_strip_stats": (C.c_int, [_vp, _vp, _vp, _fp, _i32, _fp, _i32, _fp, _fp, _i32, _i64, _i32, _i32, _i32, _f32, _i32, _vp]),
    "udt_attn_fwd": (C.c_int, [_vp, _vp, _vp, _vp, _i32, _i32, _i32, _i32, _i32, _i32, _i32, _i32,
                               _i64, _i64, _i64, _i64, _f32, _vp]),
    "udt_attn_rowv_fwd": (C.c_int, [_vp, _vp, _vp, _vp, _i32, _i32, _i32, _i32, _i32, _i32, _i32, _i32,
                                    _i64, _i64, _i64, _i64, _f32, _vp]),
    "udt_attn_rowv_q8_fwd": (C.c_int, [_vp, _vp, _vp, _vp, _i32, _i32, _i32, _i32, _i32, _i32, _i32, _i32,
                                       _i64, _i64, _i64, _i64, _f32, _vp, _vp, _i32, _vp]),
    "udt_attn_mx8_fwd": (C.c_int, [_vp, _vp, _vp, _i32, _i32, _i32, _i32, _i32, _f32, _f32, _vp, _vp, _i32, _vp]),
    "udt_attn512_fwd": (C.c_int, [_vp, _vp, _vp, _vp, _i32, _i32, _i32, _i32, _i32, _i32, _i32, _i64, _i64, _i64, _i64, _f32, _vp]),
    "udt_attn512_workspace_bytes": (C.c_size_t, [_i32, _i32, _i32]),
    "udt_attn512_split_fwd": (C.c_int, [_vp, _vp, _vp, _vp, _i32, _i32, _i32, _i32, _i32, _i32, _i32, _i64, _i64, _i64, _i64, _f32,
                                        _vp, C.c_size_t, _vp]),
    "udt_xattn_fwd": (C.c_int, [_vp, _vp, _vp, _vp, _fp, _i32, _i32, _i32, _i32, _i32, _i32, _i32, _i32, _f32, _vp]),
    "udt_mattn_fwd": (C.c_int, [_vp, _vp, _vp, _vp, _fp, _vp, _i32, _i32, _i32, _i32, _i32, _i32, _i32, _i32, _i32, _i32,
                                _i64, _i64, _i64, _i64, _f32, _vp]),
    "udt_softmax_rows": (C.c_int, [_vp, _i64, _i32, _i32, _vp]),
    "udt_tattn_hp": (_i32, [_i32]),
    "udt_tattn_prepare": (C.c_int, [_vp, _i32, _vp, _i32, _vp, _i32, _fp, _fp, _vp, _fp, _vp, _i32, _i32, _i32, _i32, _f32, _vp]),
    "udt_tattn_fused": (C.c_int, [_vp, _vp, _vp, _fp, _vp, _fp, _i32, _i32, _i32, _i32, _i32, _f32, _vp]),
    "udt_tattn_rowstat_parts": (_i32, [_i32, _i32, _i32]),
    "udt_tattn_fused_q8": (C.c_int, [_vp, _vp, _vp, _fp, _vp, _fp, _i32, _i32, _i32, _i32, _i32, _f32, _vp, _vp, _fp, _vp]),
    "udt_gn_nchunks": (_i32, [_i64, _i32]),
    "udt_gn_stats": (C.c_int, [_vp, _vp, _fp, _i32, _i64, _i32, _i32, _i32, _vp]),
    "udt_gn_apply": (C.c_int, [_vp, _vp, _vp, _fp, _fp, _fp, _i32, _i64, _i32, _i32, _i32, _f32, _i32, _vp]),
    "udt_gn_strip_ok": (_i32, [_i32, _i64, _i32, _i32, _i32]),
    "udt_gn_strip": (C.c_int, [_vp, _vp, _vp, _fp, _fp, _i32, _i64, _i32, _i32, _i32, _f32, _i32, _vp]),
    "udt_layernorm": (C.c_int, [_vp, _vp, _fp, _fp, _i64, _i32, _f32, _vp]),
    "udt_unet_input": (C.c_int, [_fp, _vp, _i32, _i32, _i32, _f32, _vp]),
    "udt_unet_input_churn": (C.c_int, [_fp, _fp, _vp, _i32, _i32, _i32, _f32, _f32, _vp]),
    "udt_cfg_euler_step": (C.c_int, [_fp, _fp, _fp, _i32, _i32, _i32, _f32, _f32, _f32, _f32, _vp]),
    "udt_cfg_sampler_step": (C.c_int, [_fp, _fp, _fp, _fp, _fp, _fp, _fp, _i32, _i32, _i32, SamplerCoefs, _vp]),
    "udt_cfg_multistep_step": (C.c_int, [_fp, _fp, _fp, _fp, _i32, _i32, _i32, MultistepCoefs, _vp]),
    "udt_sampler_step": (C.c_int, [_fp, _fp, _fp, _i32, _i32, _i32, _f32, _f32, _f32, _f32, _vp]),
    "udt_posterior_sample": (C.c_int, [_fp, _fp, _fp, _i32, _i32, _i32, _f32, _vp]),
    "udt_nchw_to_nhwc": (C.c_int, [_fp, _vp, _i32, _i32, _i64, _i32, _f32, _vp]),
    "udt_nhwc_to_nchw": (C.c_int, [_vp, _fp, _i32, _i32, _i64, _i32, _i32, _vp]),
    "udt_nhwc_set_channels": (C.c_int, [_fp, _vp, _i32, _i32, _i64, _i32, _i32, _vp]),
    "udt_embed_tokens": (C.c_int, [_vp, _fp, _fp, _vp, _i32, _i32, _i32, _vp]),
    "udt_timestep_embedding": (C.c_int, [_fp, _vp, _i32, _i32, _vp]),
    "udt_mask_downsample": (C.c_int, [_fp, _fp, _i32, _i32, _i32, _vp]),
    "udt_local_loss": (C.c_int, [_fp, _fp, _fp, _fp, _fp, _i32, _i32, _i32, _i32, _i32, _i32, _i32, _vp]),
    "udt_local_loss_tiled": (C.c_int, [_fp, _fp, _fp, _fp, _fp, _i32, _i32, _i32, _i32, _i32, _i32, _i32, _i32, _vp]),
    "udt_attn_bwd": (C.c_int, [_vp, _vp, _vp, _vp, _vp, _vp, _vp, _vp, _fp, _fp, _i32, _i32, _i32, _i32, _i32, _i32, _f32, _vp]),
    "udt_xattn_bwd": (C.c_int, [_vp, _vp, _fp, _fp, _vp, _vp, _i32, _i32, _i32, _i32, _i32, _i32, _i32, _i32, _f32, _vp]),
    "udt_local_loss_bwd": (C.c_int, [_fp, _fp, _fp, _fp, _fp, _fp, _fp, _i32, _i32, _i32, _i32, _i32, _i32, _i32, _i32, _f32, _vp]),
    "udt_local_loss_bwd_hw": (C.c_int, [_fp, _fp, _fp, _fp, _fp, _fp, _fp, _i32, _i32, _i32, _i32, _i32, _i32, _i32, _i32, _i32, _f32,
                                        _vp]),
    "udt_local_loss_tiled_hw": (C.c_int, [_fp, _fp, _fp, _fp, _fp, _fp, _i32, _i32, _i32, _i32, _i32, _i32, _i32, _i32, _i32, _vp]),
    "udt_layernorm_bwd": (C.c_int, [_vp, _vp, _fp, _vp, _vp, _i64, _i32, _f32, _vp]),
    "udt_gn_bwd": (C.c_int, [_vp, _vp, _fp, _fp, _vp, _vp, _fp, _i32, _i32, _i32, _i32, _f32, _i32, _vp]),
    "udt_geglu_fwd": (C.c_int, [_vp, _vp, _i64, _i32, _vp]),
    "udt_geglu_bwd": (C.c_int, [_vp, _vp, _vp, _i64, _i32, _vp]),
    "udt_sum2x2_bf16": (C.c_int, [_vp, _vp, _i32, _i32, _i32, _i32, _vp]),
    "udt_axpy_f32": (C.c_int, [_fp, _fp, _f32, _i64, _vp]),
    "udt_center_tokens": (C.c_int, [_fp, _vp, _i32, _i32, _i32, _vp]),
    "udt_transpose_bf16": (C.c_int, [_vp, _vp, _i32, _i32, _i32, _i32, _vp]),
    "udt_reduce_rows_f32": (C.c_int, [_fp, _fp, _i32, _i64, _i32, _vp]),
    "udt_colparts": (_i32, [_i64]),
    "udt_colsum_bf16": (C.c_int, [_vp, _fp, _fp, _i64, _i32, _vp]),
    "udt_ln_param_grad": (C.c_int, [_vp, _vp, _fp, _fp, _i64, _i32, _f32, _vp]),
    "udt_xattn_bwd_kv": (C.c_int, [_vp, _vp, _fp, _fp, _vp, _vp, _vp, _fp, _i32, _i32, _i32, _i32, _i32, _i32, _i32, _i32, _i32, _f32, _vp]),
    "udt_xattn_kv_splits": (_i32, [_i32]),
    "udt_wgrad_splits": (_i32, [_i64, _i32, _i32]),
    "udt_wgrad_bf16": (C.c_int, [_vp, _vp, _fp, _fp, _i64, _i32, _i32, _i32, _i32, _vp]),
    "udt_local_loss_seg_bwd": (C.c_int, [_fp, _fp, _fp, _fp, _fp, _fp, _fp, _i32, _i32, _i32, _i32, _i32, _i32, _i32, _f32, _vp]),
    "udt_local_loss_seg_bwd_hw": (C.c_int, [_fp, _fp, _fp, _fp, _fp, _fp, _fp, _i32, _i32, _i32, _i32, _i32, _i32, _i32, _i32, _f32,
                                            _vp]),
    "udt_diff_loss_grad": (C.c_int, [_fp, _fp, _fp, _fp, _vp, _fp, _i32, _i32, _i32, _i32, _vp]),
    "udt_adamw_f32": (C.c_int, [_fp, _fp, _fp, _fp, _i64, _f32, _f32, _f32, _f32, _f32, _i32, _f32, _vp]),
    "udt_add_bf16": (C.c_int, [_vp, _vp, _i64, _vp]),
    "udt_debug_set": (C.c_int, [C.c_char_p, _i32]),
    "udt_bias_add_bf16": (C.c_int, [_vp, _vp, _vp, _i64, _i32, _vp]),
    "udt_version": (C.c_char_p, []),
    "udt_status_string": (C.c_char_p, [C.c_int]),
    "udt_last_hip_error": (C.c_int, []),
    "udt_device_arch_ok": (C.c_int, []),
    "udt_prof_enable": (C.c_int, [C.c_uint32]),
    "udt_prof_reset": (C.c_int, []),
    "udt_prof_trace": (C.c_int, [_i32]),
    "udt_prof_dump": (C.c_int, [C.c_char_p]),
    "udt_prof_get": (C.c_int, [_i32, C.POINTER(C.c_double), C.POINTER(C.c_int64)]),
}

_lib = None


class UdtError(RuntimeError):
    pass


def load() -> C.CDLL:
    global _lib
    if _lib is not None:
        return _lib
    if not os.path.exists(LIB_PATH):
        raise UdtError(
            f"{LIB_PATH} not found: the HIP extension is not built. Run `python -m udifftext_amd.build` "
            "(or __graft_entry__.build()). There is no CPU fallback for the product path.")
    lib = C.CDLL(LIB_PATH)
    for name, (res, args) in SYMBOLS.items():
        fn = getattr(lib, name)
        fn.restype = res
        fn.argtypes = args
    _lib = lib
    return lib


def check(status: int, what: str = "") -> None:
    if status == 0:
        return
    lib = load()
    msg = lib.udt_status_string(status).decode()
    if status == -4:
        msg += f" [hipError {lib.udt_last_hip_error()}]"
    if status in (-1, -2):
        raise ValueError(f"{what}: {msg}")
    raise UdtError(f"{what}: {msg}")
```

udifftext_amd/ops.py:

```python
from __future__ import annotations

import contextlib
import ctypes as C
import os
import threading
from typing import NamedTuple, Optional, Sequence

import torch

from . import lib as L

WORKSPACE_BYTES = 96 << 20


class Workspace:

    def __init__(self, device, nbytes: int = WORKSPACE_BYTES):
        if torch.device(device).type != "cuda":
            raise L.UdtError("udifftext_amd workspaces live on the GPU (no CPU fallback)")
        self.buf = torch.zeros(nbytes, dtype=torch.uint8, device=device)

    def check(self, stream: Optional[int] = None) -> None:
        L.check(L.load().udt_check_async_error(self.buf.data_ptr(), self.buf.numel(), _stream() if stream is None else stream),
                "udt_check_async_error")


class _Ctx(threading.local):
    cu_share = 1
    workspace: Optional[Workspace] = None


_ctx = _Ctx()
_default_ws: dict = {}


@contextlib.contextmanager
def launch_context(cu_share: Optional[int] = None, workspace: Optional[Workspace] = None):
    prev = (_ctx.cu_share, _ctx.workspace)
    if cu_share is not None:
        _ctx.cu_share = max(1, int(cu_share))
    if workspace is not None:
        _ctx.workspace = workspace
    try:
        yield
    finally:
        _ctx.cu_share, _ctx.workspace = prev


def _stream() -> int:
    return torch.cuda.current_stream().cuda_stream


def _ptr(t: Optional[torch.Tensor]) -> Optional[int]:
    if t is None:
        return None
    if not t.is_cuda:
        raise L.UdtError("udifftext_amd ops need device tensors (no CPU fallback)")
    return t.data_ptr()


def _ws(nbytes: int, device) -> torch.Tensor:
    ws = _ctx.workspace
    if ws is None:
        key = (device.type, device.index, _stream())
        ws = _default_ws.get(key)
        if ws is None:
            ws = _default_ws[key] = Workspace(device)
    if ws.buf.numel() < nbytes:
        raise L.UdtError(f"stream-K workspace of {ws.buf.numel()} bytes is too small for this launch ({nbytes})")
    return ws.buf


def check_async_errors() -> None:
    for (_, _, stream), ws in list(_default_ws.items()):
        ws.check(stream)


WORK_COUNTER: Optional[dict] = None


def count_work(kind: str, amount: float) -> None:
    if WORK_COUNTER is not None:
        WORK_COUNTER[kind] = WORK_COUNTER.get(kind, 0.0) + amount


def _bf16(t: torch.Tensor) -> None:
    if t.dtype != torch.bfloat16:
        raise ValueError(f"expected bf16 tensor, got {t.dtype}")


def gemm_desc(**kw) -> L.GemmDesc:
    d = L.GemmDesc()
    d.batch = 1
    d.alpha = 1.0
    d.cu_share = _ctx.cu_share
    for k, v in kw.items():
        setattr(d, k, v)
    return d


def run_gemm(d: L.GemmDesc, device, fused_gn: bool = False) -> None:
    lib = L.load()
    need = lib.udt_gemm_workspace_bytes(C.byref(d))
    ws_ptr, ws_bytes = None, 0
    if need:
        ws = _ws(need, device)
        ws_ptr, ws_bytes = ws.data_ptr(), ws.numel()
    if fused_gn:
        L.check(lib.udt_gn_silu_conv3x3_fwd(C.byref(d), ws_ptr, ws_bytes, _stream()), "udt_gn_silu_conv3x3_fwd")
    else:
        L.check(lib.udt_gemm(C.byref(d), ws_ptr, ws_bytes, _stream()), "udt_gemm")


GN_STRIP = True


class GnStats(NamedTuple):
    data: torch.Tensor
    slots_per_sample: int


def gn_stats_of(t: Optional[torch.Tensor]) -> Optional[GnStats]:
    return getattr(t, "gn_stats", None) if t is not None else None


def _attach_colstats(d: L.GemmDesc, out: torch.Tensor, n_cols: int, rows_per_batch: int) -> bool:
    lib = L.load()
    rows = lib.udt_gemm_colstats_rows(C.byref(d))
    if rows <= 0:
        return False
    slots = lib.udt_gemm_colstats_slots(C.byref(d))
    st = torch.empty((slots, n_cols, 2), dtype=torch.float32, device=out.device)
    d.colstats = st.data_ptr()
    out.gn_stats = GnStats(st, rows_per_batch // rows)
    return True


def _drop_stale_stats(out: Optional[torch.Tensor]) -> None:
    if out is not None and getattr(out, "gn_stats", None) is not None:
        del out.gn_stats


class Mx8Act(NamedTuple):
    data: torch.Tensor
    scale: torch.Tensor
    stats: Optional[torch.Tensor] = None


def mx8_of(t: Optional[torch.Tensor]) -> Optional[Mx8Act]:
    return getattr(t, "mx8", None) if t is not None else None


def _mx8_alloc(M: int, cols: int, device) -> Mx8Act:
    return Mx8Act(torch.empty((M, cols), dtype=torch.uint8, device=device),
                  torch.empty(((cols + 127) // 128, M), dtype=torch.int32, device=device))


def _attach_q8(d: L.GemmDesc, M: int, cols: int, device, rowstats: bool, fixed: Optional[tuple] = None) -> Optional[Mx8Act]:
    q = _mx8_alloc(M, cols, device)
    d.q8_out, d.q8_scale, d.ld_q8 = q.data.data_ptr(), q.scale.data_ptr(), cols
    if fixed is not None:
        d.q8_fixed_col, d.q8_fixed_mul = int(fixed[0]), float(fixed[1])
    lib = L.load()
    parts = lib.udt_gemm_rowstat_parts(C.byref(d)) if rowstats else 0
    if not lib.udt_gemm_q8_ok(C.byref(d)) or (rowstats and parts <= 0):
        d.q8_out, d.q8_scale, d.ld_q8, d.q8_fixed_col = None, None, 0, 0
        return None
    if rowstats:
        st = torch.empty((parts, M, 2), dtype=torch.float32, device=device)
        d.rowstat_out = st.data_ptr()
        q = Mx8Act(q.data, q.scale, st)
    return q


def linear(x: torch.Tensor, w: torch.Tensor, bias: Optional[torch.Tensor] = None, *, out: Optional[torch.Tensor] = None,
           residual: Optional[torch.Tensor] = None, rowvec: Optional[torch.Tensor] = None, rows_per_batch: int = 0,
           flags: int = 0, alpha: float = 1.0, n_out: Optional[int] = None, colstats: bool = False,
           emit_q8: bool = False, emit_rowstats: bool = False) -> torch.Tensor:
    _bf16(x); _bf16(w)
    K = x.shape[-1]
    x2 = x.reshape(-1, K) if x.is_contiguous() else x
    assert x2.dim() == 2 and x2.stride(1) == 1
    M = x2.shape[0]
    N = w.shape[0] if n_out is None else n_out
    assert w.shape[1] == K and w.is_contiguous()
    n_cols = N // 2 if (flags & L.GEMM_GEGLU) else N
    if out is None:
        dt = torch.float32 if (flags & L.GEMM_OUT_F32) else torch.bfloat16
        if flags & L.GEMM_TRANSPOSED:
            assert rows_per_batch > 0
            out = torch.empty((M // rows_per_batch, N, rows_per_batch), dtype=dt, device=x.device)
        else:
            out = torch.empty((M, n_cols), dtype=dt, device=x.device)
    ldo = out.stride(0) if not (flags & L.GEMM_TRANSPOSED) else 0
    d = gemm_desc(a=_ptr(x2), w=_ptr(w), bias=_ptr(bias), residual=_ptr(residual), rowvec=_ptr(rowvec), out=_ptr(out),
                  M=M, N=N, K=K, lda=x2.stride(0), ldo=ldo, ldr=(residual.stride(0) if residual is not None else 0),
                  rows_per_batch=rows_per_batch, ld_rowvec=(rowvec.stride(0) if rowvec is not None else 0), flags=flags,
                  alpha=alpha)
    if not (colstats and rows_per_batch > 0 and out.is_contiguous() and _attach_colstats(d, out, n_cols, rows_per_batch)):
        _drop_stale_stats(out)
    q8 = None
    if emit_q8 and not (flags & (L.GEMM_OUT_F32 | L.GEMM_TRANSPOSED | L.GEMM_GEGLU)) and d.colstats is None and rowvec is None:
        q8 = _attach_q8(d, M, n_cols, x.device, emit_rowstats)
    run_gemm(d, x.device)
    if getattr(out, "mx8", None) is not None:
        del out.mx8
    if q8 is not None:
        out.mx8 = q8
    if WORK_COUNTER is not None:
        count_work("gemm", 2.0 * M * N * K)
        count_work("gemm_bytes", 2.0 * (M * K + N * K) + out.numel() * out.element_size()
                   + (2.0 * M * n_cols if residual is not None else 0.0))
        count_work("gemm_launches", 1.0)
    return out


def linear_mx8(x: Mx8Act, wq: torch.Tensor, colscale: torch.Tensor, bias: Optional[torch.Tensor] = None, *,
               out: Optional[torch.Tensor] = None, residual: Optional[torch.Tensor] = None, rows_per_batch: int = 0,
               flags: int = 0, n_out: Optional[int] = None, colstats: bool = False, emit_q8: bool = False,
               emit_rowstats: bool = False, ln_c: Optional[torch.Tensor] = None, ln_s: Optional[torch.Tensor] = None,
               eps: float = 1e-5, want_bf16: bool = True, q8_fixed: Optional[tuple] = None):
    xq = x.data
    assert xq.dtype == torch.uint8 and wq.dtype == torch.uint8 and xq.is_contiguous() and wq.is_contiguous()
    M, K = xq.shape
    N = wq.shape[0] if n_out is None else n_out
    assert wq.shape[1] == K and K % 128 == 0 and colscale.dtype == torch.float32 and colscale.numel() >= N
    assert x.scale.dtype == torch.int32 and x.scale.shape == (K // 128, M) and x.scale.is_contiguous()
    geglu = bool(flags & L.GEMM_GEGLU)
    n_cols = N // 2 if geglu else N
    only_q8 = emit_q8 and not want_bf16
    if out is None and not only_q8:
        out = torch.empty((M, n_cols), dtype=torch.bfloat16, device=xq.device)
    d = gemm_desc(a=_ptr(xq), w=_ptr(wq), bias=_ptr(ln_c if ln_c is not None else bias), residual=_ptr(residual),
                  out=_ptr(out), M=M, N=N, K=K, lda=K, ldo=(out.stride(0) if out is not None else 0),
                  ldr=(residual.stride(0) if residual is not None else 0), rows_per_batch=rows_per_batch,
                  flags=flags | L.GEMM_MX8, colscale=_ptr(colscale), a_scale=_ptr(x.scale))
    if ln_s is not None:
        if x.stats is None:
            raise L.UdtError("linear_mx8: a LayerNorm-folded MX8 GEMM needs the row statistics of its input (Mx8Act.stats)")
        assert x.stats.dtype == torch.float32 and x.stats.is_contiguous() and x.stats.shape[1:] == (M, 2)
        d.ln_colsum, d.ln_eps = _ptr(ln_s), eps
        d.rowstat_in, d.rowstat_in_parts = _ptr(x.stats), x.stats.shape[0]
    if out is not None and not (colstats and rows_per_batch > 0 and out.is_contiguous()
                                and _attach_colstats(d, out, n_cols, rows_per_batch)):
        _drop_stale_stats(out)
    q8 = None
    if emit_q8:
        q8 = _attach_q8(d, M, n_cols, xq.device, emit_rowstats and not geglu, fixed=q8_fixed)
        if q8 is None:
            raise L.UdtError(f"udt_gemm has no MX8-emitting plan for M={M} N={N} K={K} flags={flags:#x}")
    run_gemm(d, xq.device)
    if out is not None and getattr(out, "mx8", None) is not None:
        del out.mx8
    if WORK_COUNTER is not None:
        count_work("gemm_fp8", 2.0 * M * N * K)
        count_work("gemm_fp8_launches", 1.0)
    if only_q8:
        return q8
    if q8 is not None:
        out.mx8 = q8
    return out


def ln_linear(x: torch.Tensor, w_folded: torch.Tensor, c: torch.Tensor, s: torch.Tensor, *, eps: float = 1e-5,
              out: Optional[torch.Tensor] = None, residual: Optional[torch.Tensor] = None, flags: int = 0,
              n_out: Optional[int] = None, emit_q8: bool = False, want_bf16: bool = True, q8_fixed: Optional[tuple] = None,
              q8_or_none: bool = False):
    _bf16(x); _bf16(w_folded)
    K = x.shape[-1]
    x2 = x.reshape(-1, K) if x.is_contiguous() else x
    assert x2.dim() == 2 and x2.stride(1) == 1 and w_folded.shape[1] == K and w_folded.is_contiguous()
    M = x2.shape[0]
    N = w_folded.shape[0] if n_out is None else n_out
    n_cols = N // 2 if (flags & L.GEMM_GEGLU) else N
    only_q8 = emit_q8 and not want_bf16
    if out is None and not only_q8:
        out = torch.empty((M, n_cols), dtype=torch.bfloat16, device=x.device)
    d = gemm_desc(a=_ptr(x2), w=_ptr(w_folded), bias=_ptr(c), residual=_ptr(residual), out=_ptr(out), M=M, N=N, K=K,
                  lda=x2.stride(0), ldo=(out.stride(0) if out is not None else 0),
                  ldr=(residual.stride(0) if residual is not None else 0), flags=flags, ln_colsum=_ptr(s), ln_eps=eps)
    q8 = None
    if emit_q8:
        q8 = _attach_q8(d, M, n_cols, x.device, False, fixed=q8_fixed)
        if q8 is None:
            if q8_or_none:
                return None
            raise L.UdtError(f"udt_ln_gemm_fwd has no MX8-emitting plan for M={M} N={N} K={K}")
    lib = L.load()
    need = lib.udt_gemm_workspace_bytes(C.byref(d))
    ws_ptr, ws_bytes = None, 0
    if need:
        ws = _ws(need, x.device)
        ws_ptr, ws_bytes = ws.data_ptr(), ws.numel()
    rc = lib.udt_ln_gemm_fwd(C.byref(d), ws_ptr, ws_bytes, _stream())
    if rc in (-1, -2) and x.is_cuda:
        raise L.UdtError(f"udt_ln_gemm_fwd declined M={M} N={N} K={K} flags={flags:#x} (status {rc}): the LayerNorm-folded GEMM "
                         "needs the lean kernel family (UDT_LEAN / udt_debug_set('lean') != 0) and 16-byte aligned operands; "
                         "set UDT_LN_GEMM=0 to run layernorm + GEMM instead")
    L.check(rc, "udt_ln_gemm_fwd")
    if WORK_COUNTER is not None:
        count_work("gemm", 2.0 * M * N * K)
        count_work("gemm_bytes", 2.0 * (M * K + N * K) + (2.0 if out is not None else 0.0) * M * n_cols
                   + (1.0 * M * n_cols if q8 is not None else 0.0) + (2.0 * M * n_cols if residual is not None else 0.0))
        count_work("gemm_launches", 1.0)
    if only_q8:
        return q8
    if q8 is not None:
        out.mx8 = q8
    return out


def bmm_nt(a: torch.Tensor, w: torch.Tensor, *, out: Optional[torch.Tensor] = None, alpha: float = 1.0) -> torch.Tensor:
    _bf16(a); _bf16(w)
    B, M, K = a.shape
    N = w.shape[1]
    assert a.stride(2) == 1 and w.stride(2) == 1 and w.shape[0] == B and w.shape[2] == K
    if out is None:
        out = torch.empty((B, M, N), dtype=torch.bfloat16, device=a.device)
    d = gemm_desc(a=_ptr(a), w=_ptr(w), out=_ptr(out), M=M, N=N, K=K, lda=a.stride(1), ldw=w.stride(1),
                  ldo=out.stride(1), batch=B, stride_a=a.stride(0), stride_w=w.stride(0), stride_out=out.stride(0),
                  alpha=alpha)
    run_gemm(d, a.device)
    if WORK_COUNTER is not None:
        count_work("gemm", 2.0 * B * M * N * K)
        count_work("gemm_bytes", 2.0 * B * (M * K + N * K + M * N))
        count_work("gemm_launches", 1.0)
    return out


def conv2d(x: torch.Tensor, w: torch.Tensor, bias: Optional[torch.Tensor] = None, *, ksize: int = 3, stride: int = 1,
           pad: Optional[tuple] = None, upsample: bool = False, x2: Optional[torch.Tensor] = None,
           out_hw: Optional[tuple] = None, residual: Optional[torch.Tensor] = None,
           rowvec: Optional[torch.Tensor] = None, flags: int = 0, n_out: Optional[int] = None,
           out: Optional[torch.Tensor] = None, colstats: bool = False, in_scsh: Optional[torch.Tensor] = None,
           in_act: int = 0, probe_in_scsh: bool = False, w_up4: Optional[torch.Tensor] = None):
    _bf16(x); _bf16(w)
    assert x.is_contiguous() and w.is_contiguous()
    B, H, W_, C1 = x.shape
    C2 = 0
    if x2 is not None:
        _bf16(x2)
        assert x2.is_contiguous() and x2.shape[:3] == x.shape[:3]
        C2 = x2.shape[3]
    Hv, Wv = (H * 2, W_ * 2) if upsample else (H, W_)
    if pad is None:
        pad = (ksize // 2, ksize // 2)
    if out_hw is None:
        out_hw = ((Hv + 2 * pad[0] - ksize) // stride + 1, (Wv + 2 * pad[1] - ksize) // stride + 1)
    Ho, Wo = out_hw
    N = w.shape[0] if n_out is None else n_out
    K = ksize * ksize * (C1 + C2)
    assert w.shape[1] == K, (w.shape, K)
    M = B * Ho * Wo
    if out is None and not probe_in_scsh:
        dt = torch.float32 if (flags & L.GEMM_OUT_F32) else torch.bfloat16
        out = torch.empty((B, Ho, Wo, N), dtype=dt, device=x.device)
    d = gemm_desc(a=_ptr(x), a2=_ptr(x2), w=_ptr(w), bias=_ptr(bias), residual=_ptr(residual), rowvec=_ptr(rowvec),
                  out=_ptr(out), M=M, N=N, K=K, lda=0, ldo=(out.stride(2) if out is not None else N),
                  ldr=(residual.stride(2) if residual is not None else 0),
                  Hin=H, Win=W_, C1=C1, C2=C2, Hout=Ho, Wout=Wo, ksize=ksize, stride=stride, pad_t=pad[0], pad_l=pad[1],
                  upsample=1 if upsample else 0, rows_per_batch=Ho * Wo,
                  ld_rowvec=(rowvec.stride(0) if rowvec is not None else 0), flags=flags | L.GEMM_CONV)
    if probe_in_scsh:
        return bool(L.load().udt_gemm_in_scsh_ok(C.byref(d)))
    if w_up4 is not None and upsample and ksize == 3 and x2 is None and in_scsh is None:
        _bf16(w_up4)
        assert w_up4.is_contiguous() and w_up4.dim() == 3 and w_up4.shape[0] == 4 and w_up4.shape[1] >= N and w_up4.shape[2] == 4 * C1, \
            (w_up4.shape, N, C1)
        d.upsample, d.w, d.ldw, d.stride_w = 2, _ptr(w_up4), w_up4.shape[2], w_up4.stride(0)
        if not L.load().udt_gemm_up4_ok(C.byref(d)):
            d.upsample, d.w, d.ldw, d.stride_w = 1, _ptr(w), 0, 0
    if in_scsh is not None:
        assert in_scsh.dtype == torch.float32 and in_scsh.is_contiguous() and in_scsh.numel() == B * (C1 + C2) * 2
        d.in_scsh = in_scsh.data_ptr()
        d.in_act = int(in_act)
    if not (colstats and _attach_colstats(d, out, N, Ho * Wo)):
        _drop_stale_stats(out)
    if in_scsh is not None:
        run_gemm(d, x.device, fused_gn=True)
    else:
        run_gemm(d, x.device)
    return out


def attention(q: torch.Tensor, k: torch.Tensor, vt: torch.Tensor, heads: int, scale: float,
              out: Optional[torch.Tensor] = None) -> torch.Tensor:
    _bf16(q); _bf16(k); _bf16(vt)
    B, Nq = q.shape[0], q.shape[1]
    Nk = k.shape[1]
    assert q.stride(2) == 1 and k.stride(2) == 1 and vt.stride(2) == 1
    if out is None:
        out = torch.empty((B, Nq, heads * 64), dtype=torch.bfloat16, device=q.device)
    L.check(L.load().udt_attn_fwd(_ptr(q), _ptr(k), _ptr(vt), _ptr(out), B, heads, Nq, Nk,
                                  q.stride(1), k.stride(1), vt.stride(1), out.stride(1),
                                  q.stride(0), k.stride(0), vt.stride(0), out.stride(0), scale, _stream()),
            "udt_attn_fwd")
    if WORK_COUNTER is not None:
        count_work("attn", 4.0 * B * heads * Nq * Nk * 64)
        count_work("attn_bytes", 2.0 * B * heads * 64 * (2 * Nq + 2 * Nk))
        count_work("attn_launches", 1.0)
    return out


def attention_rowv(q: torch.Tensor, k: torch.Tensor, v: torch.Tensor, heads: int, scale: float,
                   out: Optional[torch.Tensor] = None, emit_q8: bool = False) -> torch.Tensor:
    _bf16(q); _bf16(k); _bf16(v)
    B, Nq = q.shape[0], q.shape[1]
    Nk = k.shape[1]
    assert q.stride(2) == 1 and k.stride(2) == 1 and v.stride(2) == 1 and v.shape[1] == Nk
    if out is None:
        out = torch.empty((B, Nq, heads * 64), dtype=torch.bfloat16, device=q.device)
    if getattr(out, "mx8", None) is not None:
        del out.mx8
    if emit_q8 and heads % 2 == 0 and out.is_contiguous():
        q8 = _mx8_alloc(B * Nq, heads * 64, q.device)
        L.check(L.load().udt_attn_rowv_q8_fwd(_ptr(q), _ptr(k), _ptr(v), _ptr(out), B, heads, Nq, Nk,
                                              q.stride(1), k.stride(1), v.stride(1), out.stride(1),
                                              q.stride(0), k.stride(0), v.stride(0), out.stride(0), scale,
                                              _ptr(q8.data), _ptr(q8.scale), heads * 64, _stream()), "udt_attn_rowv_q8_fwd")
        out.mx8 = q8
    else:
        L.check(L.load().udt_attn_rowv_fwd(_ptr(q), _ptr(k), _ptr(v), _ptr(out), B, heads, Nq, Nk,
                                           q.stride(1), k.stride(1), v.stride(1), out.stride(1),
                                           q.stride(0), k.stride(0), v.stride(0), out.stride(0), scale, _stream()),
                "udt_attn_rowv_fwd")
    if WORK_COUNTER is not None:
        count_work("attn", 4.0 * B * heads * Nq * Nk * 64)
        count_work("attn_bytes", 2.0 * B * heads * 64 * (2 * Nq + 2 * Nk))
        count_work("attn_launches", 1.0)
    return out


def attention_mx8(qkv: Mx8Act, batch: int, heads: int, scale: float, v_mul: float, out: Optional[torch.Tensor] = None,
                  emit_q8: bool = False) -> torch.Tensor:
    C_ = heads * 64
    M, ld8 = qkv.data.shape
    assert qkv.data.dtype == torch.uint8 and qkv.data.is_contiguous() and ld8 >= 3 * C_ and M % batch == 0
    assert qkv.scale.dtype == torch.int32 and qkv.scale.is_contiguous() and qkv.scale.shape == ((ld8 + 127) // 128, M)
    N = M // batch
    if out is None:
        out = torch.empty((batch, N, C_), dtype=torch.bfloat16, device=qkv.data.device)
    assert out.is_contiguous()
    if getattr(out, "mx8", None) is not None:
        del out.mx8
    q8 = _mx8_alloc(M, C_, qkv.data.device) if emit_q8 else None
    L.check(L.load().udt_attn_mx8_fwd(_ptr(qkv.data), _ptr(qkv.scale), _ptr(out), batch, heads, N, ld8, out.stride(1), scale,
                                      1.0 / v_mul, _ptr(q8.data) if q8 else None, _ptr(q8.scale) if q8 else None, C_, _stream()),
            "udt_attn_mx8_fwd")
    if q8 is not None:
        out.mx8 = q8
    if WORK_COUNTER is not None:
        count_work("attn_fp8", 4.0 * batch * heads * N * N * 64)
        count_work("attn_fp8_bytes", 1.0 * batch * heads * 64 * 3 * N + 2.0 * batch * heads * 64 * N)
        count_work("attn_fp8_launches", 1.0)
    return out


def attention_d512(q: torch.Tensor, k: torch.Tensor, v: torch.Tensor, scale: float,
                   out: Optional[torch.Tensor] = None, key_split: bool = True) -> torch.Tensor:
    _bf16(q); _bf16(k); _bf16(v)
    B, Nq = q.shape[0], q.shape[1]
    Nk = k.shape[1]
    assert q.shape[2] == 512 and k.shape[2] == 512 and v.shape[2] == 512 and v.shape[1] == Nk
    assert q.stride(2) == 1 and k.stride(2) == 1 and v.stride(2) == 1
    if out is None:
        out = torch.empty((B, Nq, 512), dtype=torch.bfloat16, device=q.device)
    lib = L.load()
    need = int(lib.udt_attn512_workspace_bytes(B, Nq, Nk)) if key_split else 0
    if need:
        scratch = torch.empty((need,), dtype=torch.uint8, device=q.device)
        L.check(lib.udt_attn512_split_fwd(_ptr(q), _ptr(k), _ptr(v), _ptr(out), B, Nq, Nk,
                                          q.stride(1), k.stride(1), v.stride(1), out.stride(1),
                                          q.stride(0), k.stride(0), v.stride(0), out.stride(0), scale, _ptr(scratch), need, _stream()),
                "udt_attn512_split_fwd")
    else:
        L.check(lib.udt_attn512_fwd(_ptr(q), _ptr(k), _ptr(v), _ptr(out), B, Nq, Nk,
                                    q.stride(1), k.stride(1), v.stride(1), out.stride(1),
                                    q.stride(0), k.stride(0), v.stride(0), out.stride(0), scale, _stream()),
                "udt_attn512_fwd")
    if WORK_COUNTER is not None:
        count_work("attn", 4.0 * B * Nq * Nk * 512)
        count_work("attn_bytes", 2.0 * B * 512 * (2 * Nq + 2 * Nk))
        count_work("attn_launches", 1.0)
    return out


def xattention(q: torch.Tensor, k: torch.Tensor, v: torch.Tensor, heads: int, head_dim: int, scale: float,
               probs: Optional[torch.Tensor] = None, out: Optional[torch.Tensor] = None) -> torch.Tensor:
    _bf16(q); _bf16(k); _bf16(v)
    B, Nq = q.shape[0], q.shape[1]
    Lc = k.shape[1]
    assert q.is_contiguous() or (q.stride(2) == 1 and q.stride(0) == Nq * q.stride(1))
    assert k.stride(2) == 1 and v.stride(2) == 1 and k.stride(1) == v.stride(1)
    assert k.stride(0) == Lc * k.stride(1) and v.stride(0) == Lc * v.stride(1)
    if out is None:
        out = torch.empty((B, Nq, heads * head_dim), dtype=torch.bfloat16, device=q.device)
    if probs is not None:
        assert probs.dtype == torch.float32 and probs.is_contiguous() and probs.numel() == B * heads * Nq * Lc
    L.check(L.load().udt_xattn_fwd(_ptr(q), _ptr(k), _ptr(v), _ptr(out), _ptr(probs), B, heads, head_dim, Nq, Lc,
                                   q.stride(1), k.stride(1), out.stride(1), scale, _stream()), "udt_xattn_fwd")
    return out


def masked_attention(q: torch.Tensor, k: torch.Tensor, v: torch.Tensor, heads: int, scale: float,
                     mask: Optional[torch.Tensor] = None, key_padding_mask: Optional[torch.Tensor] = None,
                     out: Optional[torch.Tensor] = None) -> torch.Tensor:
    _bf16(q); _bf16(k); _bf16(v)
    B, Nq, Cq = q.shape
    Lk = k.shape[1]
    D = Cq // heads
    assert q.stride(2) == 1 and k.stride(2) == 1 and v.stride(2) == 1
    if out is None:
        out = torch.empty((B, Nq, heads * D), dtype=torch.bfloat16, device=q.device)
    if mask is not None:
        mask = mask.float().contiguous()
        assert mask.shape == (Nq, Lk)
# ... 561 lines not shown
```

udifftext_amd/sgm/modules/hipnn.py:

```python
from __future__ import annotations

import math
import os
from typing import Optional

import torch
import torch.nn as nn

from udifftext_amd import lib as L
from udifftext_amd import ops, packing

from ..util import init_skipped


def count_flops(kind: str, flops: float) -> None:
    ops.count_work(kind, flops)


FUSE_GN = os.environ.get("UDT_FUSE_GN", "0") != "0"

GN_EPI = os.environ.get("UDT_GN_EPI", "1") != "0" and os.environ.get("UDT_LEAN", "") != "0"
EMIT_STATS = FUSE_GN or GN_EPI


def want_stats(B: int, HW: int, C: int) -> bool:
    return FUSE_GN or (GN_EPI and C % 8 == 0)


FP8_LINEARS = os.environ.get("UDT_FP8", "0") != "0"


FP8_ATTENTION = os.environ.get("UDT_FP8_ATTN", "1") != "0"


def fp8_attention() -> bool:
    return FP8_LINEARS and LN_GEMM and FP8_ATTENTION


def v_fixed_mul(w_v: torch.Tensor, c_v: torch.Tensor) -> float:
    bound = 12.0 * float(w_v.float().norm(dim=1).max()) + float(c_v.float().abs().max())
    return float(2.0 ** math.floor(math.log2(448.0 / max(bound, 1e-20))))


def mx8_width(c: int) -> bool:
    return FP8_LINEARS and LN_GEMM and c % 128 == 0

LN_GEMM = os.environ.get("UDT_LN_GEMM", "1") != "0" and os.environ.get("UDT_LEAN", "") != "0"


def carry_stats(dst: torch.Tensor, src: torch.Tensor) -> torch.Tensor:
    st = ops.gn_stats_of(src)
    if st is not None:
        dst.gn_stats = st
    return dst


def carry_mx8(dst: torch.Tensor, src: torch.Tensor) -> torch.Tensor:
    q = ops.mx8_of(src)
    if q is not None:
        dst.mx8 = q
    return dst


def _init_uniform_(p: torch.Tensor, fan_in: int) -> None:
    if init_skipped():
        return
    bound = 1.0 / math.sqrt(max(fan_in, 1))
    with torch.no_grad():
        p.uniform_(-bound, bound)


class _Layouts(dict):
    frozen = False


def _layouts(mod: nn.Module) -> _Layouts:
    store = mod.__dict__.get("_layouts")
    if store is None:
        store = mod.__dict__["_layouts"] = _Layouts()
    return store


def layout(mod: nn.Module, tag: str, build, *inputs):
    store = _layouts(mod)
    hit = store.get(tag)
    if store.frozen:
        if hit is None:
            raise L.UdtError(f"{type(mod).__name__}: layout {tag!r} was not built before prepare(free_masters=True) released the "
                             "fp32 masters; reload the checkpoint into a fresh engine to change the launch path")
        return hit[1]
    key = [(t.data_ptr(), t._version, t.device) if isinstance(t, torch.Tensor) else t for t in (*mod._sources(), *inputs)]
    if hit is None or hit[0] != key:
        with torch.no_grad():
            hit = store[tag] = (key, build())
    return hit[1]


def has_layout(mod: nn.Module, tag: str) -> bool:
    return tag in mod.__dict__.get("_layouts", ())


def freeze_layouts(mod: nn.Module) -> None:
    _layouts(mod).frozen = True


def drop_layouts(root: nn.Module) -> None:
    for m in root.modules():
        store = m.__dict__.get("_layouts")
        if store is not None and not store.frozen:
            store.clear()


def nbytes(*layouts) -> int:
    ts = [t for pk in layouts for t in (pk if isinstance(pk, (tuple, list)) else (pk,))]
    return sum(t.numel() * t.element_size() for t in ts if isinstance(t, torch.Tensor))


class _Packed(nn.Module):

    def _sources(self):
        return self._parameters.values()

    def fused_children(self):
        return []

    def packed(self):
        return layout(self, "plain", self._pack)

    def packed_fp8(self):
        return layout(self, "fp8", self._pack_fp8)

    def packed_ln(self, norm):
        return layout(self, "ln", lambda: self._pack_ln(norm.weight, norm.bias), norm.weight, norm.bias)

    def packed_ln_mx8(self, norm):
        return layout(self, "ln_mx8", lambda: self._pack_ln_mx8(norm.weight, norm.bias), norm.weight, norm.bias)


class Linear(_Packed):
    def __init__(self, in_features: int, out_features: int, bias: bool = True):
        super().__init__()
        self.in_features, self.out_features = in_features, out_features
        self.weight = nn.Parameter(torch.empty(out_features, in_features))
        _init_uniform_(self.weight, in_features)
        if bias:
            self.bias = nn.Parameter(torch.empty(out_features))
            _init_uniform_(self.bias, in_features)
        else:
            self.register_parameter("bias", None)

    def _pack(self):
        return packing.pack_linear(self.weight), packing.pad_bias(self.bias)

    def _pack_fp8(self):
        wq, cs = packing.pack_linear_fp8(self.weight)
        return wq, cs, packing.pad_bias(self.bias)

    def forward(self, x, residual=None, flags: int = 0, out=None, rowvec=None, rows_per_batch: int = 0,
                colstats: bool = False, x8=None, emit_q8: bool = False, emit_rowstats: bool = False):
        if x8 is not None:
            wq, cs, b = self.packed_fp8()
            M = x8.data.shape[0]
            if colstats:
                rpb = rows_per_batch if rows_per_batch > 0 else M
                colstats = want_stats(M // rpb, rpb, wq.shape[0])
            return ops.linear_mx8(x8, wq, cs, b, residual=residual, flags=flags, out=out, rows_per_batch=rows_per_batch,
                                  colstats=bool(colstats), emit_q8=emit_q8, emit_rowstats=emit_rowstats)
        w, b = self.packed()
        if colstats:
            rpb = rows_per_batch if rows_per_batch > 0 else x.shape[0]
            colstats = want_stats(x.shape[0] // rpb, rpb, w.shape[0])
        return ops.linear(x, w, b, residual=residual, flags=flags, out=out, rowvec=rowvec, rows_per_batch=rows_per_batch,
                          colstats=bool(colstats), emit_q8=emit_q8, emit_rowstats=emit_rowstats)


class Conv2d(_Packed):

    def __init__(self, in_channels: int, out_channels: int, kernel_size: int, stride: int = 1, padding: int = 0):
        super().__init__()
        self.in_channels, self.out_channels = in_channels, out_channels
        self.kernel_size, self.stride, self.padding = kernel_size, stride, padding
        self.weight = nn.Parameter(torch.empty(out_channels, in_channels, kernel_size, kernel_size))
        self.bias = nn.Parameter(torch.empty(out_channels))
        fan_in = in_channels * kernel_size * kernel_size
        _init_uniform_(self.weight, fan_in)
        _init_uniform_(self.bias, fan_in)
        self.segments = None
        self.n_pad = 4
        self.emit_colstats = False

    def _pack(self):
        return packing.pack_conv(self.weight, self.segments, self.n_pad), packing.pad_bias(self.bias, self.n_pad)

    def packed(self):
        return layout(self, "plain", self._pack, self.segments, self.n_pad)

    def packed_up4(self):
        return layout(self, "up4", lambda: packing.pack_conv_up4(self.weight, self.n_pad), self.n_pad)

    def forward(self, x, x2=None, residual=None, rowvec=None, upsample: bool = False, flags: int = 0,
                pad: Optional[tuple] = None, out_hw: Optional[tuple] = None, norm: Optional["GroupNorm"] = None,
                norm_silu: bool = False, colstats: Optional[bool] = None):
        if x2 is not None and self.segments is None and (x.shape[-1] % 64 != 0 or x2.shape[-1] % 64 != 0):
            self.segments = (x.shape[-1], x2.shape[-1])
        w, b = self.packed()
        if pad is None:
            pad = (self.padding, self.padding)
        if colstats is None:
            colstats = self.emit_colstats
        if colstats:
            oh, ow = out_hw if out_hw is not None else ((x.shape[1] * (2 if upsample else 1) + 2 * pad[0] - self.kernel_size) // self.stride + 1,
                                                        (x.shape[2] * (2 if upsample else 1) + 2 * pad[1] - self.kernel_size) // self.stride + 1)
            colstats = want_stats(x.shape[0], oh * ow, w.shape[0])
        colstats = bool(colstats)
        kw = dict(ksize=self.kernel_size, stride=self.stride, pad=pad, upsample=upsample, out_hw=out_hw, residual=residual,
                  rowvec=rowvec, flags=flags, n_out=w.shape[0], colstats=colstats)
        if upsample and norm is None and x2 is None and self.kernel_size == 3 and self.stride == 1:
            kw["w_up4"] = self.packed_up4()
        in_scsh = None
        if norm is not None:
            st1, st2 = ops.gn_stats_of(x), ops.gn_stats_of(x2)
            if (FUSE_GN and st1 is not None and (x2 is None or st2 is not None)
                    and ops.conv2d(x, w, b, x2=x2, probe_in_scsh=True, **kw)):
                B = x.shape[0]
                in_scsh = ops.gn_finalize(st1, x.shape[-1], st2, x2.shape[-1] if x2 is not None else 0, norm.weight,
                                          norm.bias, B, x.shape[1] * x.shape[2], norm.num_groups, norm.eps)
                count_flops("fused_gn_convs", 1)
            else:
                x, x2 = norm(x, x2=x2, silu=norm_silu), None
        out = ops.conv2d(x, w, b, x2=x2, in_scsh=in_scsh, in_act=1 if norm_silu else 0, **kw)
        if ops.WORK_COUNTER is not None:
            k = self.kernel_size
            kind = "conv3x3" if k == 3 else "conv1x1"
            npix_out = out.shape[0] * out.shape[1] * out.shape[2]
            count_flops(kind, 2.0 * npix_out * self.out_channels * self.in_channels * k * k)
            nbytes = 2.0 * x.numel() / x.shape[-1] * self.in_channels + 2.0 * self.weight.numel() \
                + npix_out * self.out_channels * (4.0 if (flags & L.GEMM_OUT_F32) else 2.0)
            if residual is not None:
                nbytes += 2.0 * npix_out * self.out_channels
            count_flops(kind + "_bytes", nbytes)
            Hh, Ww = x.shape[1], x.shape[2]
            if (k == 3 and self.stride == 1 and not upsample and tuple(pad) == (1, 1)
                    and self.out_channels > 64 and not (flags & L.GEMM_OUT_F32)
                    and ((Ww % 32 == 0 and Hh % 8 == 0) or (Ww % 16 == 0 and Hh % 16 == 0) or (Ww == 8 and Hh == 8))):
                count_flops("conv3p_bytes", nbytes)
                count_flops("conv3p_launches", 1.0)
        return out


class GroupNorm(nn.Module):
    def __init__(self, num_groups: int, num_channels: int, eps: float = 1e-5):
        super().__init__()
        self.num_groups, self.num_channels, self.eps = num_groups, num_channels, eps
        self.weight = nn.Parameter(torch.ones(num_channels))
        self.bias = nn.Parameter(torch.zeros(num_channels))

    def forward(self, x, x2=None, silu: bool = False):
        if GN_EPI:
            st1, st2 = ops.gn_stats_of(x), ops.gn_stats_of(x2)
            C1, C2 = x.shape[-1], (x2.shape[-1] if x2 is not None else 0)
            HW = x.numel() // (x.shape[0] * C1)
            if (st1 is not None and (x2 is None or st2 is not None)
                    and (ops.gn_strip_ok(x.shape[0], HW, C1, C2, self.num_groups)
                         or ((C1 + C2) % 64 == 0 and (C1 + C2) // self.num_groups <= 128))):
                count_flops("gn_from_epilogue_stats", 1)
                return ops.group_norm_from_stats(x, st1, self.weight, self.bias, self.num_groups, self.eps, silu, x2=x2, st2=st2)
        return ops.group_norm(x, self.weight, self.bias, self.num_groups, self.eps, silu, x2=x2)


class LayerNorm(nn.Module):
    def __init__(self, dim: int, eps: float = 1e-5):
        super().__init__()
        self.dim, self.eps = dim, eps
        self.weight = nn.Parameter(torch.ones(dim))
        self.bias = nn.Parameter(torch.zeros(dim))

    def forward(self, x):
        return ops.layer_norm(x, self.weight, self.bias, self.eps)


def fuse_rows(*weights: torch.Tensor) -> torch.Tensor:
    return packing.pack_linear(torch.cat(list(weights), dim=0))


GEMM_GEGLU = L.GEMM_GEGLU
GEMM_OUT_F32 = L.GEMM_OUT_F32
GEMM_RELU = L.GEMM_RELU
GEMM_TRANSPOSED = L.GEMM_TRANSPOSED
GEMM_SILU_OUT = L.GEMM_SILU_OUT
```

Before: 10.74 images/s.

## Fuse GroupNorm+SiLU prologue into wide lean conv3x3 kernel and enable by default

Adds a GNIN variant of the wide conv3x3 kernel that loads input patches into registers, applies the GroupNorm scale/shift and optional SiLU, and stores the result to LDS. It also supports concatenated skip inputs (C2). This removes the standalone GroupNorm pass and its activation round-trip through memory. UDT_FUSE_GN now defaults to 'wide', so the fused path is used only where the wide plan applies and fills the CUs. The cost is register-staged patch loads in place of direct LDS DMA, plus extra VALU work interleaved with the MFMA schedule.

```diff
diff --git a/include/udt_kernels.h b/include/udt_kernels.h
--- a/include/udt_kernels.h
+++ b/include/udt_kernels.h
@@ -79,6 +79,7 @@
 int32_t udt_gemm_q8_ok(const udt_gemm_desc* d);
 int32_t udt_gemm_colstats_slots(const udt_gemm_desc* d);
 int32_t udt_gemm_in_scsh_ok(const udt_gemm_desc* d);
+int32_t udt_gemm_in_scsh_wide_ok(const udt_gemm_desc* d);
 int32_t udt_gemm_up4_ok(const udt_gemm_desc* d);
 int udt_gn_silu_conv3x3_fwd(const udt_gemm_desc* d, void* workspace, size_t workspace_bytes, void* stream);
 int udt_ln_gemm_fwd(const udt_gemm_desc* d, void* workspace, size_t workspace_bytes, void* stream);
diff --git a/udifftext_amd/csrc/common.h b/udifftext_amd/csrc/common.h
--- a/udifftext_amd/csrc/common.h
+++ b/udifftext_amd/csrc/common.h
@@ -32,6 +32,36 @@
 UDT_DEVINL float fast_exp2(float x) { return __builtin_amdgcn_exp2f(x); }
 UDT_DEVINL float silu_f(float x) {
   return x * __builtin_amdgcn_rcpf(1.0f + __builtin_amdgcn_exp2f(-x * 1.4426950408889634f));
+}
+UDT_DEVINL u32x4 gn_norm8(const u32x4 v, const float* sc, const float* sh, int act) {
+  u32x4 o;
+#pragma unroll
+  for (int j = 0; j < 4; ++j) {
+    float a = __builtin_fmaf(bf16_lo(v[j]), sc[2 * j], sh[2 * j]);
+    float bb = __builtin_fmaf(bf16_hi(v[j]), sc[2 * j + 1], sh[2 * j + 1]);
+    if (act == 1) {
+      a = silu_f(a);
+      bb = silu_f(bb);
+    }
+    o[j] = pack_bf16x2(a, bb);
+  }
+  return o;
+}
+UDT_DEVINL void gn_act_consts(int act, float& k, float& off) {
+  k = act == 1 ? -1.4426950408889634f : 0.0f;
+  off = act == 1 ? 0.0f : -200.0f;
+}
+UDT_DEVINL u32x4 gn_norm8_sel(const u32x4 v, const float* sc, const float* sh, float k, float off) {
+  u32x4 o;
+#pragma unroll
+  for (int j = 0; j < 4; ++j) {
+    float a = __builtin_fmaf(bf16_lo(v[j]), sc[2 * j], sh[2 * j]);
+    float bb = __builtin_fmaf(bf16_hi(v[j]), sc[2 * j + 1], sh[2 * j + 1]);
+    a = a * __builtin_amdgcn_rcpf(1.0f + __builtin_amdgcn_exp2f(__builtin_fmaf(a, k, off)));
+    bb = bb * __builtin_amdgcn_rcpf(1.0f + __builtin_amdgcn_exp2f(__builtin_fmaf(bb, k, off)));
+    o[j] = pack_bf16x2(a, bb);
+  }
+  return o;
 }
 UDT_DEVINL float gelu_erf_f(float x) {
   const float z = fabsf(x) * 0.70710678118654752f;
diff --git a/udifftext_amd/csrc/gemm.hip b/udifftext_amd/csrc/gemm.hip
--- a/udifftext_amd/csrc/gemm.hip
+++ b/udifftext_amd/csrc/gemm.hip
@@ -901,7 +901,10 @@
   }
   if (!on || lean_mode() == 0) return false;
   if (d->flags != UDT_GEMM_CONV || d->ksize != 3 || d->stride != 1 || d->pad_t != 1 || d->pad_l != 1) return false;
-  if (d->C2 != 0 || d->in_scsh || d->colscale || d->batch > 1) return false;
+  const bool gnin = d->in_scsh != nullptr;
+  if ((d->C2 != 0 && !gnin) || d->C2 < 0 || d->C2 % 64 != 0 || d->colscale || d->batch > 1) return false;
+  if (gnin && (d->upsample != 0 || (d->C2 > 0 && !d->a2) || (d->in_act != 0 && d->in_act != 1))) return false;
+  const int Ct = d->C1 + d->C2;
   if (want_stats && !lean_stats_enabled()) return false;
   if (d->N < 128 || d->N % 8 != 0 || d->C1 <= 0 || d->C1 % 64 != 0) return false;
   if (d->upsample != 0 && d->upsample != 1 && d->upsample != 2) return false;
@@ -919,23 +922,26 @@
       const int cus = device_cus(), share = d->cu_share > 1 ? d->cu_share : 1;
       wide_slots = cus / share > 0 ? cus / share : 1;
       const long long wt = (long long)(d->M / 256) * (d->N / 160);
-      const long long sk = conv_chunk_slices(wt, wide_slots, d->C1 / 64, lean_splitk_knob());
+      const long long sk = conv_chunk_slices(wt, wide_slots, Ct / 64, lean_splitk_knob());
       const long long units = wt * sk;
       const long long rounds = (units + cus - 1) / cus;
       const double eff = units > cus ? (double)units / (double)(rounds * cus) : ((double)units * share >= cus ? 1.0 : (double)units * share / cus);
       wide = (wm > 0) || (sk <= 2 && eff >= ((share >= 3 && share_of(d) >= 3) ? wide_lanes_eff() : 0.85));
     }
   }
+  if (gnin && !wide) return false;
   if (wide) { c.geo = phase ? 6 : 3; c.tw = 16; c.th = 16; c.bn = 160; c.wgm = 4; }
   else if (Wt % 16 == 0 && Ht % 8 == 0) { c.geo = ups ? 2 : phase ? 4 : 0; c.tw = 16; c.th = 8; }
   else if (!ups && Wt % 8 == 0 && Ht % 8 == 0) { c.geo = phase ? 5 : 1; c.tw = 8; c.th = 8; }
   else return false;
   if (d->ldo % 8 != 0 || (d->residual && d->ldr % 8 != 0)) return false;
   const long long ldw = d->ldw > 0 ? d->ldw : (phase ? 4LL * d->C1 : (long long)d->K);
+  if (gnin && ((reinterpret_cast<uintptr_t>(d->in_scsh) & 15) || (long long)d->M * d->C2 * 2 >= (1LL << 31))) return false;
   if (ldw % 8 != 0) return false;
   c.w_phase = phase ? (d->stride_w > 0 ? d->stride_w : (long long)d->N * ldw) : 0;
   if (phase && (c.w_phase < (long long)d->N * ldw || c.w_phase % 8 != 0)) return false;
   if ((long long)d->M * d->C1 * 2 >= (1LL << 31) || (long long)d->N * ldw * 2 >= (1LL << 31)) return false;
+  if (gnin && (long long)ldw < 9LL * Ct) return false;
   if ((reinterpret_cast<uintptr_t>(d->out) | reinterpret_cast<uintptr_t>(d->residual) | reinterpret_cast<uintptr_t>(d->bias) |
        reinterpret_cast<uintptr_t>(d->rowvec)) & 15) return false;
   if (d->rowvec && ((d->ld_rowvec > 0 ? d->ld_rowvec : d->N) % 4 != 0)) return false;
@@ -943,7 +949,7 @@
 #ifdef UDT_MEASURE
   c.dbg = g_lconv_dbg.load(std::memory_order_relaxed);
 #endif
-  c.N = d->N; c.C = d->C1; c.H = d->Hin; c.W = d->Win; c.B = d->M / (d->Hout * d->Wout);
+  c.N = d->N; c.C = Ct; c.H = d->Hin; c.W = d->Win; c.B = d->M / (d->Hout * d->Wout);
   c.ldw = (int)ldw; c.ldo = d->ldo; c.ldr = d->ldr; c.ldrv = d->ld_rowvec > 0 ? d->ld_rowvec : d->N;
   c.alpha = d->alpha;
   c.tiles_x = Wt / c.tw; c.tiles_y = Ht / c.th;
@@ -968,17 +974,23 @@
   c.a_bytes = (unsigned)((long long)c.B * d->Hin * d->Win * d->C1 * 2);
   c.w_bytes = (unsigned)((long long)d->N * ldw * 2);
   c.counters = nullptr; c.slabs = nullptr;
+  c.in_scsh = d->in_scsh; c.in_act = d->in_act; c.a2 = nullptr; c.C1 = d->C1; c.C2 = d->C2;
+  c.a2_bytes = (unsigned)((long long)c.B * d->Hin * d->Win * d->C2 * 2);
   return true;
 }
 
 int lean_conv_phases(const lg::C3Params& c) { return c.geo >= 4 ? 4 : 1; }
+
+bool wide_gn_pays(const udt_gemm_desc* d, const lg::C3Params& c) {
+  (void)d;
+  return wide_conv_mode() > 0 || (long long)c.tiles >= device_cus();
+}
 
 size_t lean_conv_workspace(const lg::C3Params& c) {
   return c.splitk > 1 ? G8_HEADER_BYTES + (size_t)c.tiles * lean_conv_phases(c) * c.splitk * c.tw * c.th * c.bn * sizeof(float) : 0;
 }
 
 bool lean_stats_probe(const udt_gemm_desc* d, int& rows, int& slots) {
-  if (d->in_scsh) return false;
   {
     lg::C3Params c3;
     if (lean_conv_plan(d, c3, true)) {
@@ -1056,10 +1068,23 @@
   if (!lean_plan(&t, lt, false) || lt.cfg != 1 || (d->flags & UDT_GEMM_GEGLU)) return 0;
   return (d->N + 63) / 64;
 }
+bool wide_gn_plan(const udt_gemm_desc* d, lg::C3Params& c3) {
+  alignas(16) static const float probe_table[4] = {0.f, 0.f, 0.f, 0.f};
+  udt_gemm_desc t = *d;
+  if (!t.in_scsh) { t.in_scsh = probe_table; if (t.in_act != 1) t.in_act = 0; }
+  return lean_conv_plan(&t, c3, t.colstats != nullptr) && c3.geo == 3;
+}
 extern "C" int32_t udt_gemm_in_scsh_ok(const udt_gemm_desc* d) {
   if (!d || d->K <= 0 || d->K % BK != 0) return 0;
+  lg::C3Params c3;
+  if (wide_gn_plan(d, c3)) return 1;
   c3p::Geo ge;
   return conv3p_geometry(d, ge, true) ? 1 : 0;
+}
+extern "C" int32_t udt_gemm_in_scsh_wide_ok(const udt_gemm_desc* d) {
+  if (!d || d->K <= 0 || d->K % BK != 0) return 0;
+  lg::C3Params c3;
+  return (wide_gn_plan(d, c3) && wide_gn_pays(d, c3)) ? 1 : 0;
 }
 
 extern "C" int32_t udt_gemm_up4_ok(const udt_gemm_desc* d) {
@@ -1263,7 +1288,7 @@
     lg::C3Params c3;
     if (lean_conv_plan(d, c3, d->colstats != nullptr)) {
       c3.colstats = d->colstats;
-      c3.a = p.a; c3.w = p.w; c3.bias = p.bias; c3.res = p.res; c3.rowvec = p.rowvec; c3.out = reinterpret_cast<uint16_t*>(d->out);
+      c3.a = p.a; c3.a2 = d->C2 > 0 ? p.a2 : nullptr; c3.w = p.w; c3.bias = p.bias; c3.res = p.res; c3.rowvec = p.rowvec; c3.out = reinterpret_cast<uint16_t*>(d->out);
       if (c3.splitk > 1) {
         if (!workspace || workspace_bytes < lean_conv_workspace(c3)) return UDT_ERR_WORKSPACE;
         c3.counters = reinterpret_cast<int*>(workspace);
@@ -1275,7 +1300,7 @@
         snprintf(tag, sizeof(tag), "%s%s M=%d N=%d K=%d %dx%d tile=%dx%d units=%d splitk=%d nb=%d%s", (c3.geo == 3 || c3.geo == 6) ? "wconv3" : "lconv3",
                  (d->upsample && c3.geo != 6) ? "+up" : "", d->M, d->N, d->K,
                  d->Hin, d->Win, c3.tw, c3.th, c3.tiles * lean_conv_phases(c3) * c3.splitk, c3.splitk, c3.n_block,
-                 d->upsample == 2 ? " up4" : "");
+                 d->upsample == 2 ? " up4" : d->in_scsh ? " gn" : "");
         udt_prof_tag(profc.rec, tag);
       }
       const hipError_t ec = udt_lean_launch_conv3(&c3, s);
diff --git a/udifftext_amd/csrc/lean.hip b/udifftext_amd/csrc/lean.hip
--- a/udifftext_amd/csrc/lean.hip
+++ b/udifftext_amd/csrc/lean.hip
@@ -74,13 +74,13 @@
   return c3.colstats ? launch_lconv3s<TW, TH, UPS, true, PHASE>(c3, s) : launch_lconv3s<TW, TH, UPS, false, PHASE>(c3, s);
 }
 
-template <bool STATS, bool PHASE>
+template <bool STATS, bool PHASE, bool GNIN = false>
 hipError_t launch_wconv3s(const lg::C3Params& c3, hipStream_t s) {
   static AttrOnce once;
   constexpr int smem = wd::WGeo::SMEM;
-  hipError_t e = once.ensure(reinterpret_cast<const void*>(wd::wconv3_kernel<STATS, PHASE>), smem);
+  hipError_t e = once.ensure(reinterpret_cast<const void*>(wd::wconv3_kernel<STATS, PHASE, GNIN>), smem);
   if (e != hipSuccess) return e;
-  hipLaunchKernelGGL((wd::wconv3_kernel<STATS, PHASE>), dim3(c3.G), dim3(256), smem, s, c3);
+  hipLaunchKernelGGL((wd::wconv3_kernel<STATS, PHASE, GNIN>), dim3(c3.G), dim3(256), smem, s, c3);
   return hipGetLastError();
 }
 template <int KT, bool GEGLU, bool EMIT = false>
@@ -95,6 +95,11 @@
 
 template <bool PHASE>
 hipError_t launch_wconv3(const lg::C3Params& c3, hipStream_t s) {
+  if constexpr (!PHASE) {
+    if (c3.in_scsh) return c3.colstats ? launch_wconv3s<true, false, true>(c3, s) : launch_wconv3s<false, false, true>(c3, s);
+  } else if (c3.in_scsh) {
+    return hipErrorInvalidValue;
+  }
   return c3.colstats ? launch_wconv3s<true, PHASE>(c3, s) : launch_wconv3s<false, PHASE>(c3, s);
 }
 
@@ -118,6 +123,7 @@
 
 hipError_t udt_lean_launch_conv3(const void* c3params, hipStream_t s) {
   const lg::C3Params& c3 = *static_cast<const lg::C3Params*>(c3params);
+  if (c3.in_scsh && c3.geo != 3) return hipErrorInvalidValue;
   return c3.geo == 3 ? launch_wconv3<false>(c3, s) : c3.geo == 6 ? launch_wconv3<true>(c3, s) : c3.geo == 2 ? launch_lconv3<16, 8, true>(c3, s)
          : c3.geo == 4 ? launch_lconv3<16, 8, false, true>(c3, s) : c3.geo == 5 ? launch_lconv3<8, 8, false, true>(c3, s)
          : c3.geo == 1 ? launch_lconv3<8, 8, false>(c3, s) : launch_lconv3<16, 8, false>(c3, s);
diff --git a/udifftext_amd/csrc/lean_params.h b/udifftext_amd/csrc/lean_params.h
--- a/udifftext_amd/csrc/lean_params.h
+++ b/udifftext_amd/csrc/lean_params.h
@@ -58,6 +58,11 @@
   int bn, wgm;
   long long w_phase;
   int dbg;
+  const float* in_scsh;
+  const uint16_t* a2;
+  int C1, C2;
+  unsigned a2_bytes;
+  int in_act;
 };
 
 }
diff --git a/udifftext_amd/csrc/norm.hip b/udifftext_amd/csrc/norm.hip
--- a/udifftext_amd/csrc/norm.hip
+++ b/udifftext_amd/csrc/norm.hip
@@ -154,21 +154,7 @@
     }
   }
   __syncthreads();
-  auto norm8 = [&](const u32x4 v, int cc) {
-    u32x4 o;
-#pragma unroll
-    for (int j = 0; j < 4; ++j) {
-      const int c = cc * 8 + 2 * j;
-      float a = bf16_lo(v[j]) * sc[c] + sh[c];
-      float bb = bf16_hi(v[j]) * sc[c + 1] + sh[c + 1];
-      if (act == 1) {
-        a = silu_f(a);
-        bb = silu_f(bb);
-      }
-      o[j] = pack_bf16x2(a, bb);
-    }
-    return o;
-  };
+  auto norm8 = [&](const u32x4 v, int cc) { return gn_norm8(v, sc + cc * 8, sh + cc * 8, act); };
   if (full) {
     *reinterpret_cast<u32x4*>(yb + i * 8) = norm8(v0, c0);
     *reinterpret_cast<u32x4*>(yb + (i + 256) * 8) = norm8(v1, c1);
diff --git a/udifftext_amd/csrc/wide.h b/udifftext_amd/csrc/wide.h
--- a/udifftext_amd/csrc/wide.h
+++ b/udifftext_amd/csrc/wide.h
@@ -26,8 +26,9 @@
   static_assert(SMEM <= 160 * 1024, "one workgroup per CU");
 };
 
-template <bool STATS, bool PHASE = false>
+template <bool STATS, bool PHASE = false, bool GNIN = false>
 __global__ void __launch_bounds__(256, 1) wconv3_kernel(const C3Params p) {
+  static_assert(!(GNIN && PHASE), "no norm sits in front of an upsampling convolution");
   using G = WGeo;
   constexpr int NT = PHASE ? 4 : 9;
   constexpr int NW = G::NW, TM = G::TM, TN = G::TN, BN = G::BN, PW = G::PW, NR = G::NRING;
@@ -82,6 +83,8 @@
   auto patch_swz = [](int prow, int yy) { return ((prow - 2 * yy) >> 1) & 7; };
   unsigned w_voff[WP], p_voff[PP];
   int p_piece[PP];
+  unsigned p_voff2[GNIN ? PP : 1];
+  int p_lds[GNIN ? PP : 1];
 #pragma unroll
   for (int i = 0; i < WP; ++i) {
     const int row = (wave + NW * i) * 8 + l3;
@@ -99,8 +102,15 @@
     const int xx = prow - yy * PW;
     const int gy = y0 + yy - 1, gx = x0 + xx - 1;
     const bool ok = (prow < G::PROWS) && ((unsigned)gy < (unsigned)p.H) && ((unsigned)gx < (unsigned)p.W);
-    const int koff = (pslot ^ patch_swz(prow, yy)) * 8;
-    p_voff[i] = ok ? (unsigned)(((((long long)b * p.H + gy) * p.W + gx) * p.C + koff) * 2) : OOB;
+    if constexpr (GNIN) {
+      const long long pix = ((long long)b * p.H + gy) * p.W + gx;
+      p_voff[i] = ok ? (unsigned)((pix * p.C1 + pslot * 8) * 2) : OOB;
+      p_voff2[i] = ok ? (unsigned)((pix * p.C2 + pslot * 8) * 2) : OOB;
+      p_lds[i] = idx * 1024 + l3 * ROW_BYTES + ((pslot ^ patch_swz(prow, yy)) << 4);
+    } else {
+      const int koff = (pslot ^ patch_swz(prow, yy)) * 8;
+      p_voff[i] = ok ? (unsigned)(((((long long)b * p.H + gy) * p.W + gx) * p.C + koff) * 2) : OOB;
+    }
   }
   int a_prow[TM], a_py[TM];
 #pragma unroll
@@ -141,9 +151,51 @@
       if (i < PP) buf_lds16(rsrc_a, pbuf + p_piece[i] * 1024, p_voff[i], c * 128);
     }
   };
-  issue_patch(c0 & 1, c0);
-#pragma unroll
-  for (int j = 0; j < NR - 1; ++j) issue_w(j, c0, j);
+  const int nc1 = GNIN ? p.C1 >> 6 : 0;
+  float gsc[GNIN ? 8 : 1], gsh[GNIN ? 8 : 1];
+  u32x4 ring[GNIN ? 2 * PPT : 1];
+  float act_k = 0.f, act_off = 0.f;
+  if constexpr (GNIN) gn_act_consts(p.in_act, act_k, act_off);
+  auto load_scsh = [&](int c) {
+    if constexpr (GNIN) {
+      const float* t = p.in_scsh + ((long long)b * p.chunks + c) * 128 + pslot * 8;
+      const f32x4 s0 = *reinterpret_cast<const f32x4*>(t), s1 = *reinterpret_cast<const f32x4*>(t + 4);
+      const f32x4 h0 = *reinterpret_cast<const f32x4*>(t + 64), h1 = *reinterpret_cast<const f32x4*>(t + 68);
+#pragma unroll
+      for (int j = 0; j < 4; ++j) gsc[j] = s0[j], gsc[4 + j] = s1[j], gsh[j] = h0[j], gsh[4 + j] = h1[j];
+    }
+  };
+  auto load_piece = [&](int i, int c) -> u32x4 {
+    const bool second = c >= nc1;
+    const __amdgpu_buffer_rsrc_t rs = __builtin_amdgcn_make_buffer_rsrc(const_cast<uint16_t*>(second ? p.a2 : p.a), 0,
+                                                                        second ? p.a2_bytes : p.a_bytes, 0x00020000);
+    return __builtin_bit_cast(u32x4, __builtin_amdgcn_raw_buffer_load_b128(rs, second ? p_voff2[i] : p_voff[i], (second ? c - nc1 : c) * 128, 0));
+  };
+  auto store_piece = [&](int buf, int i, const u32x4 v) {
+    const u32x4 on = gn_norm8_sel(v, gsc, gsh, act_k, act_off);
+    const uint32_t keep = ~(uint32_t)((int32_t)p_voff[i] >> 31);
+    u32x4 o;
+#pragma unroll
+    for (int j = 0; j < 4; ++j) o[j] = on[j] & keep;
+    *reinterpret_cast<u32x4*>(patches + buf * G::PATCH_BYTES + p_lds[i]) = o;
+  };
+  if constexpr (GNIN) {
+    load_scsh(c0);
+    u32x4 first[PP];
+#pragma unroll
+    for (int i = 0; i < PP; ++i) first[i] = load_piece(i, c0);
+#pragma unroll
+    for (int i = 0; i < PP; ++i) store_piece(c0 & 1, i, first[i]);
+    asm volatile("s_waitcnt vmcnt(0)" ::: "memory");
+#pragma unroll
+    for (int j = 0; j < NR - 1; ++j) issue_w(j, c0, j);
+    asm volatile("" ::: "memory");
+    load_scsh(c0 + 1 < c1 ? c0 + 1 : c0);
+  } else {
+    issue_patch(c0 & 1, c0);
+#pragma unroll
+    for (int j = 0; j < NR - 1; ++j) issue_w(j, c0, j);
+  }
   int st = 0;
   for (int c = c0; c < c1; ++c) {
     const int cn = (c + 1 < c1) ? c + 1 : c;
@@ -151,8 +203,14 @@
     auto tap_body = [&](auto tap_c) {
       constexpr int tap = decltype(tap_c)::value;
       constexpr auto pcount = [](int t) { const int tt = (t + NT) % NT; return tt < PTAPS ? ((tt + 1) * PPT <= PP ? PPT : PP - tt * PPT) : 0; };
-      wait_vm<pcount(tap - 2) + WP + pcount(tap - 1)>();
+      constexpr auto gcount = [](int t) { const int tt = (t + NT) % NT; return tt < PTAPS ? ((tt + 1) * PPT <= PP ? PPT : PP - tt * PPT) : (tt == NT - 1 ? 4 : 0); };
+      if constexpr (GNIN) wait_vm<WP + gcount(tap - 1)>();
+      else wait_vm<pcount(tap - 2) + WP + pcount(tap - 1)>();
       raw_barrier();
+      if constexpr (GNIN && tap >= 2 && tap - 2 < PTAPS) {
+#pragma unroll
+        for (int j = 0; j < PPT; ++j) asm volatile("" : "+v"(ring[(tap & 1) * PPT + j]));
+      }
       const int dy = PHASE ? tap >> 1 : tap / 3, dx = PHASE ? tap & 1 : tap - dy * 3;
       const char* wbuf = wring + st * G::W_BYTES;
       int arow[TM], aswz[TM];
@@ -183,10 +241,21 @@
             if (ahead < NT) issue_w(s2, c, ahead);
             else issue_w(s2, cn, ahead - NT);
           }
-          if constexpr (tap < PTAPS) {
+          if constexpr (GNIN) {
+            if constexpr (tap < PTAPS) {
+#pragma unroll
+              for (int j = 0; j < PPT; ++j)
+                if (tap * PPT + j < PP) ring[(tap & 1) * PPT + j] = load_piece(tap * PPT + j, cn);
+            }
+            if constexpr (tap == NT - 1) load_scsh(c + 2 < c1 ? c + 2 : c1 - 1);
+          } else if constexpr (tap < PTAPS) {
             if (!UDT_DBG(p.dbg, 1)) issue_patch_part((c + 1) & 1, cn, tap);
           }
         }
+        if constexpr (GNIN && tap >= 2 && tap - 2 < PTAPS) {
+          const int i = (tap - 2) * PPT + ks;
+          if (ks < PPT && i < PP) store_piece((c + 1) & 1, i, ring[(tap & 1) * PPT + ks]);
+        }
         if (UDT_DBG(p.dbg, 2)) {
 #pragma unroll
           for (int tm = 0; tm < TM; ++tm) asm volatile("" ::"v"(fx[ks & 1][tm]));
@@ -200,6 +269,8 @@
         }
       }
       __builtin_amdgcn_sched_group_barrier(0x100, TM + TN, 0);
+      constexpr bool XF = GNIN && tap >= 2 && tap - 2 < PTAPS;
+      constexpr int XV = 24;
 #pragma unroll
       for (int ks = 0; ks < 3; ++ks) {
 #pragma unroll
@@ -207,9 +278,18 @@
           __builtin_amdgcn_sched_group_barrier(0x008, 1, 0);
           __builtin_amdgcn_sched_group_barrier(0x100, 1, 0);
         }
-        __builtin_amdgcn_sched_group_barrier(0x008, TM * TN - (TM + TN), 0);
-      }
-      constexpr int NV = WP + pcount(tap), NVI = NV < TM * TN ? NV : TM * TN;
+        if constexpr (XF) {
+#pragma unroll
+          for (int i = 0; i < TM * TN - (TM + TN); ++i) {
+            __builtin_amdgcn_sched_group_barrier(0x008, 1, 0);
+            __builtin_amdgcn_sched_group_barrier(0x002, XV, 0);
+          }
+          if (ks >= 1) __builtin_amdgcn_sched_group_barrier(0x200, 1, 0);
+        } else {
+          __builtin_amdgcn_sched_group_barrier(0x008, TM * TN - (TM + TN), 0);
+        }
+      }
+      constexpr int NV = WP + (GNIN ? gcount(tap) : pcount(tap)), NVI = NV < TM * TN ? NV : TM * TN;
 #pragma unroll
       for (int i = 0; i < NVI; ++i) {
         __builtin_amdgcn_sched_group_barrier(0x008, 1, 0);
diff --git a/udifftext_amd/lib.py b/udifftext_amd/lib.py
--- a/udifftext_amd/lib.py
+++ b/udifftext_amd/lib.py
@@ -71,6 +71,7 @@
     "udt_gemm_rowstat_parts": (_i32, [C.POINTER(GemmDesc)]),
     "udt_gemm_q8_ok": (_i32, [C.POINTER(GemmDesc)]),
     "udt_gemm_in_scsh_ok": (_i32, [C.POINTER(GemmDesc)]),
+    "udt_gemm_in_scsh_wide_ok": (_i32, [C.POINTER(GemmDesc)]),
     "udt_gemm_up4_ok": (_i32, [C.POINTER(GemmDesc)]),
     "udt_gn_silu_conv3x3_fwd": (C.c_int, [C.POINTER(GemmDesc), _vp, C.c_size_t, _vp]),
     "udt_ln_gemm_fwd": (C.c_int, [C.POINTER(GemmDesc), _vp, C.c_size_t, _vp]),
diff --git a/udifftext_amd/ops.py b/udifftext_amd/ops.py
--- a/udifftext_amd/ops.py
+++ b/udifftext_amd/ops.py
@@ -90,6 +90,10 @@
 
 
 def gemm_desc(**kw) -> L.GemmDesc:
+    return _new_desc(**kw)
+
+
+def _new_desc(**kw) -> L.GemmDesc:
     d = L.GemmDesc()
     d.batch = 1
     d.alpha = 1.0
@@ -333,7 +337,7 @@
            out_hw: Optional[tuple] = None, residual: Optional[torch.Tensor] = None,
            rowvec: Optional[torch.Tensor] = None, flags: int = 0, n_out: Optional[int] = None,
            out: Optional[torch.Tensor] = None, colstats: bool = False, in_scsh: Optional[torch.Tensor] = None,
-           in_act: int = 0, probe_in_scsh: bool = False, w_up4: Optional[torch.Tensor] = None):
+           in_act: int = 0, probe_in_scsh=False, w_up4: Optional[torch.Tensor] = None):
     _bf16(x); _bf16(w)
     assert x.is_contiguous() and w.is_contiguous()
     B, H, W_, C1 = x.shape
@@ -355,13 +359,16 @@
     if out is None and not probe_in_scsh:
         dt = torch.float32 if (flags & L.GEMM_OUT_F32) else torch.bfloat16
         out = torch.empty((B, Ho, Wo, N), dtype=dt, device=x.device)
-    d = gemm_desc(a=_ptr(x), a2=_ptr(x2), w=_ptr(w), bias=_ptr(bias), residual=_ptr(residual), rowvec=_ptr(rowvec),
+    d = (_new_desc if probe_in_scsh else gemm_desc)(
+                  a=_ptr(x), a2=_ptr(x2), w=_ptr(w), bias=_ptr(bias), residual=_ptr(residual), rowvec=_ptr(rowvec),
                   out=_ptr(out), M=M, N=N, K=K, lda=0, ldo=(out.stride(2) if out is not None else N),
                   ldr=(residual.stride(2) if residual is not None else 0),
                   Hin=H, Win=W_, C1=C1, C2=C2, Hout=Ho, Wout=Wo, ksize=ksize, stride=stride, pad_t=pad[0], pad_l=pad[1],
                   upsample=1 if upsample else 0, rows_per_batch=Ho * Wo,
                   ld_rowvec=(rowvec.stride(0) if rowvec is not None else 0), flags=flags | L.GEMM_CONV)
     if probe_in_scsh:
+        if probe_in_scsh == "wide":
+            return bool(L.load().udt_gemm_in_scsh_wide_ok(C.byref(d)))
         return bool(L.load().udt_gemm_in_scsh_ok(C.byref(d)))
     if w_up4 is not None and upsample and ksize == 3 and x2 is None and in_scsh is None:
         _bf16(w_up4)
diff --git a/udifftext_amd/sgm/modules/hipnn.py b/udifftext_amd/sgm/modules/hipnn.py
--- a/udifftext_amd/sgm/modules/hipnn.py
+++ b/udifftext_amd/sgm/modules/hipnn.py
@@ -17,14 +17,15 @@
     ops.count_work(kind, flops)
 
 
-FUSE_GN = os.environ.get("UDT_FUSE_GN", "0") != "0"
+_fuse_gn = os.environ.get("UDT_FUSE_GN", "wide")
+FUSE_GN = False if _fuse_gn == "0" else ("wide" if _fuse_gn == "wide" else True)
 
 GN_EPI = os.environ.get("UDT_GN_EPI", "1") != "0" and os.environ.get("UDT_LEAN", "") != "0"
-EMIT_STATS = FUSE_GN or GN_EPI
+EMIT_STATS = FUSE_GN is True or GN_EPI
 
 
 def want_stats(B: int, HW: int, C: int) -> bool:
-    return FUSE_GN or (GN_EPI and C % 8 == 0)
+    return FUSE_GN is True or (GN_EPI and C % 8 == 0)
 
 
 FP8_LINEARS = os.environ.get("UDT_FP8", "0") != "0"
@@ -221,7 +222,7 @@
         if norm is not None:
             st1, st2 = ops.gn_stats_of(x), ops.gn_stats_of(x2)
             if (FUSE_GN and st1 is not None and (x2 is None or st2 is not None)
-                    and ops.conv2d(x, w, b, x2=x2, probe_in_scsh=True, **kw)):
+                    and ops.conv2d(x, w, b, x2=x2, probe_in_scsh=("wide" if FUSE_GN == "wide" else True), **kw)):
                 B = x.shape[0]
                 in_scsh = ops.gn_finalize(st1, x.shape[-1], st2, x2.shape[-1] if x2 is not None else 0, norm.weight,
                                           norm.bias, B, x.shape[1] * x.shape[2], norm.num_groups, norm.eps)
```

New measurement: 10.75 images/s (median of 3 runs). Within noise of the previous version (+0.1%).
